# pku-lab-1806-llm/lab-1806-vec-db

Measured on AMD Instinct MI355X. Metric: queries/sec at recall@10, Gist1M d=960 (Flat brute force, L2Sqr, k=10), higher is better.
Workload: dtype f32 (int8 lower-bound filter pass); 1 GPU; flat_knn_gist1m; rows=1000000, dim=960, k=10, dist=L2Sqr, parallelism=single GPU, steps_in_flight=1, queries_per_corpus_pass=128

## Files before the change

lab_1806_vec_db_amd/csrc/api.hip:

```cpp
#include <algorithm>
#include <cmath>
#include <cstring>

#include "ctx.hpp"
#include "pq_hnsw.hpp"
#include "remove_plan.hpp"

using namespace vdb;

static thread_local std::string g_last_error;
void vdb::set_last_error(const std::string &m) { g_last_error = m; }
void vdb::require_gpu() {
    int cnt = 0;
    hipError_t e = hipGetDeviceCount(&cnt);
    if (e != hipSuccess || cnt <= 0)
        throw Error(VDB_ERR_NOGPU, std::string("no usable HIP device (libvdbhip has no CPU fallback): ") +
                                       hipGetErrorString(e));
}

static void require_merge_ids_fit(const Index &ix) {
    VDB_REQUIRE(ix.id_offset <= (1ull << 32) && ix.n <= (1ull << 32) - ix.id_offset, "shard merge: global row ids must fit 32 bits");
}

void vdb::merge_topk_dev(Index &ix, const void *d_dists, const void *d_ids, const void *d_counts, uint64_t stride_d,
// ... 616 lines not shown
        throw;
    }
    ix.prof_collect(*ws);
    VDB_API_END
}

int vdb_flat_knn_filtered_device(vdb_index *idx, const void *d_queries, uint64_t nq, uint64_t dim, uint64_t k, const vdb_mask *mask, void *d_out_idx,
                                 void *d_out_dist, void *d_out_count, void *stream) {
    VDB_API_BEGIN
    VDB_REQUIRE(idx, "null index");
    Index &ix = idx->ix;
    check_query_args(ix, d_queries, nq, dim, d_out_idx, d_out_dist);
    VDB_REQUIRE(nq == 0 || d_out_count, "null out_count");
    VDB_REQUIRE(nq <= 32768, "at most 32768 queries per device call");
    filtered_check(ix, mask);
    if (nq == 0) return VDB_OK;
    ix.use_device();
    WsLease ws(ix);
    VDB_SYNC(static_cast<hipStream_t>(stream));
    try {
        ix.flat_knn_masked_device(*ws, static_cast<const float *>(d_queries), nq, k, mask->m, static_cast<uint64_t *>(d_out_idx),
                                  static_cast<float *>(d_out_dist), static_cast<uint64_t *>(d_out_count));
    } catch (...) {
        (void)hipStreamSynchronize(ws->stream);
        ix.prof_collect(*ws);
        throw;
    }
    ix.prof_collect(*ws);
    VDB_API_END
}

static std::vector<const RowMask *> filtered_multi_check(const Index &ix, uint64_t nq, const vdb_mask *const *masks, uint64_t n_masks,
                                                         const uint32_t *mask_of) {
    VDB_REQUIRE(!ix.elem_u8, "filtered k-NN needs f32 rows: a VecSet<u8> index serves the filtered range search only");
    VDB_REQUIRE(n_masks == 0 || masks, "null masks");
    VDB_REQUIRE(nq == 0 || mask_of, "null mask_of");
    VDB_REQUIRE(n_masks < (1ull << 32), "too many masks");
    std::vector<const RowMask *> rm(n_masks);
    for (uint64_t g = 0; g < n_masks; g++) {
        VDB_REQUIRE(masks[g], "null mask");
        ix.check_mask(masks[g]->m);
        rm[g] = &masks[g]->m;
    }
    for (uint64_t q = 0; q < nq; q++)
        VDB_REQUIRE(mask_of[q] < n_masks, "mask_of[" + std::to_string(q) + "] = " + std::to_string(mask_of[q]) + ": the call has " +
                                              std::to_string(n_masks) + " masks");
    return rm;
}

int vdb_flat_knn_filtered_multi(vdb_index *idx, const float *queries, uint64_t nq, uint64_t dim, uint64_t k, const vdb_mask *const *masks,
                                uint64_t n_masks, const uint32_t *mask_of, uint64_t *out_idx, float *out_dist, uint64_t *out_count) {
    VDB_API_BEGIN
    VDB_REQUIRE(idx, "null index");
    Index &ix = idx->ix;
    check_query_args(ix, queries, nq, dim, out_idx, out_dist);
    const std::vector<const RowMask *> rm = filtered_multi_check(ix, nq, masks, n_masks, mask_of);
    ix.filtered_multi_calls++;
    if (nq == 0) return VDB_OK;
    ix.use_device();
    WsLease ws(ix);
    hipStream_t s = ws->stream;
    constexpr uint64_t CHUNK = 16384;
    const uint64_t kk = std::max<uint64_t>(k, 1), ch = std::min(nq, CHUNK);
    const size_t off_d = ch * kk * sizeof(uint64_t), off_c = (off_d + ch * kk * sizeof(float) + 7) & ~size_t(7);
    ws->q.reserve(ch * dim * sizeof(float));
    ws->out_idx.reserve(off_c + ch * sizeof(uint64_t));
    char *d_out = ws->out_idx.as<char>();
    try {
        for (uint64_t q0 = 0; q0 < nq; q0 += CHUNK) {
            const uint64_t nb = std::min<uint64_t>(CHUNK, nq - q0);
            VDB_HIP(hipMemcpyAsync(ws->q.p, queries + q0 * dim, nb * dim * sizeof(float), hipMemcpyHostToDevice, s));
            ix.flat_knn_masked_multi_device(*ws, ws->q.as<float>(), nb, k, rm.data(), n_masks, mask_of + q0, reinterpret_cast<uint64_t *>(d_out),
                                            reinterpret_cast<float *>(d_out + off_d), reinterpret_cast<uint64_t *>(d_out + off_c));
            if (k) {
                VDB_HIP(hipMemcpyAsync(out_idx + q0 * k, d_out, nb * k * sizeof(uint64_t), hipMemcpyDeviceToHost, s));
                VDB_HIP(hipMemcpyAsync(out_dist + q0 * k, d_out + off_d, nb * k * sizeof(float), hipMemcpyDeviceToHost, s));
            }
            if (out_count) VDB_HIP(hipMemcpyAsync(out_count + q0, d_out + off_c, nb * sizeof(uint64_t), hipMemcpyDeviceToHost, s));
            VDB_SYNC(s);
        }
    } catch (...) {
        (void)hipStreamSynchronize(s);
        ix.prof_collect(*ws);
        throw;
    }
    ix.prof_collect(*ws);
    VDB_API_END
}

int vdb_flat_knn_filtered_multi_device(vdb_index *idx, const void *d_queries, uint64_t nq, uint64_t dim, uint64_t k, const vdb_mask *const *masks,
                                       uint64_t n_masks, const uint32_t *mask_of, void *d_out_idx, void *d_out_dist, void *d_out_count, void *stream) {
    VDB_API_BEGIN
    VDB_REQUIRE(idx, "null index");
    Index &ix = idx->ix;
    check_query_args(ix, d_queries, nq, dim, d_out_idx, d_out_dist);
    VDB_REQUIRE(nq == 0 || d_out_count, "null out_count");
    VDB_REQUIRE(nq <= 32768, "at most 32768 queries per device call");
    const std::vector<const RowMask *> rm = filtered_multi_check(ix, nq, masks, n_masks, mask_of);
    ix.filtered_multi_calls++;
    if (nq == 0) return VDB_OK;
    ix.use_device();
    WsLease ws(ix);
    VDB_SYNC(static_cast<hipStream_t>(stream));
    try {
        ix.flat_knn_masked_multi_device(*ws, static_cast<const float *>(d_queries), nq, k, rm.data(), n_masks, mask_of, static_cast<uint64_t *>(d_out_idx),
                                        static_cast<float *>(d_out_dist), static_cast<uint64_t *>(d_out_count));
    } catch (...) {
        (void)hipStreamSynchronize(ws->stream);
        ix.prof_collect(*ws);
        throw;
    }
    ix.prof_collect(*ws);
    VDB_API_END
}

int vdb_flat_range_filtered(vdb_index *idx, const float *queries, uint64_t nq, uint64_t dim, const float *radius, uint64_t limit, const vdb_mask *mask,
                            vdb_range **out) {
    VDB_API_BEGIN
    VDB_REQUIRE(idx, "null index");
    Index &ix = idx->ix;
    range_check(ix, queries, nq, dim, radius, out);
    VDB_REQUIRE(mask, "null mask");
    ix.check_mask(mask->m);
    ix.use_device();
    std::unique_ptr<vdb_range> res(new vdb_range);
    WsLease ws(ix);
    const float *d_q = nullptr, *d_r = nullptr;
    if (nq) {
        const size_t qb = nq * dim * sizeof(float), qb_pad = (qb + 255) & ~size_t(255);
        ws->q.reserve(qb_pad + nq * sizeof(float));
        VDB_HIP(hipMemcpyAsync(ws->q.p, queries, qb, hipMemcpyHostToDevice, ws->stream));
        VDB_HIP(hipMemcpyAsync(ws->q.as<char>() + qb_pad, radius, nq * sizeof(float), hipMemcpyHostToDevice, ws->stream));
        d_q = ws->q.as<float>();
        d_r = reinterpret_cast<const float *>(ws->q.as<char>() + qb_pad);
    }
    try {
        ix.flat_range_device(*ws, d_q, nq, d_r, limit, res->r, &mask->m);
    } catch (...) {
        (void)hipStreamSynchronize(ws->stream);
        ix.prof_collect(*ws);
        throw;
    }
    ix.prof_collect(*ws);
    *out = res.release();
    VDB_API_END
}

int vdb_flat_shortlist_keys(vdb_index *idx, const float *queries, uint64_t nq, uint64_t dim, int tier, float *out_keys,
                            float *out_qsq, float *out_qerr, float *out_dx4) {
    VDB_API_BEGIN
    VDB_REQUIRE(idx && queries && out_keys, "null argument");
    Index &ix = idx->ix;
    VDB_REQUIRE(dim == ix.dim, "query dimension mismatch");
    VDB_REQUIRE(tier >= 0 && tier <= 2, "tier must be 0 (fp16 operands), 1 (split-bf16 operands) or 2 (8-bit operands, lower-bound keys)");
    ix.use_device();
    WsLease ws(ix);
    ws->q.reserve(nq * ix.dim * sizeof(float));
    VDB_HIP(hipMemcpyAsync(ws->q.p, queries, nq * ix.dim * sizeof(float), hipMemcpyHostToDevice, ws->stream));
    ix.flat_debug_keys(*ws, ws->q.as<float>(), nq, tier, out_keys, out_qsq, out_qerr, out_dx4);
    VDB_API_END
}

int vdb_flat_set_mode(vdb_index *idx, int mode) {
    VDB_API_BEGIN
    VDB_REQUIRE(idx, "null index");
    VDB_REQUIRE(mode >= 0 && mode <= 2, "mode must be 0, 1 or 2");
    idx->ix.flat_mode = mode;
    VDB_API_END
}
int vdb_set_param(vdb_index *idx, const char *name, int64_t value) {
    VDB_API_BEGIN
    VDB_REQUIRE(idx && name, "null argument");
    std::string n(name);
    if (n == "mfma_variant")
        mfma_set_variant((int)value);
    else if (n == "flat_share")
        mfma_set_share((int)value);
    else if (n == "flat_gemm")
        idx->ix.flat_gemm_mode = (int)value;
    else if (n == "hnsw_dma")
        hnsw_set_dma((int)value);
    else if (n == "hnsw_half")
        hnsw_set_half((int)value);
    else if (n == "ivf_half")
        ivf_set_half((int)value);
    else if (n == "ivf_q8")
        ivf_set_q8((int)value);
    else if (n == "hnsw_build_gpu")
        hnsw_set_build_gpu((int)value);
    else if (n == "hnsw_pool_cap")
        hnsw_set_pool_cap((int)value);
    else if (n == "pq_adc_fast")
        pq_set_adc_fast((int)value);
    else if (n == "pq_sample16")
        pq_set_adc16_sample((int)value);
    else if (n == "pq_adc16")
        pq_set_adc16((int)value);
    else if (n == "pq_adc8_sliced")
        pq_set_adc8_sliced((int)value);
    else if (n == "flat_sample_thin")
        mfma_set_sample_thin((int)value);
    else if (n == "flat_gemm_tw")
        gemm_set_tw((int)value);
    else if (n == "flat_gemm_nt")
        gemm_set_nt((int)value);
    else if (n == "flat_gemm_zigzag")
        gemm_set_zigzag((int)value);
    else if (n == "flat_gemm_block_rows") {
        VDB_REQUIRE(value >= 0, "flat_gemm_block_rows must be >= 0");
        gemm_set_block_rows((uint64_t)value);
    }
    else if (n == "flat_gemm_stagger")
        gemm_set_stagger((int)value);
    else if (n == "flat_gemm_debug")
        idx->ix.flat_gemm_debug = (int)value;
    else if (n == "flat_tail")
        idx->ix.flat_tail_mode = (int)value;
    else if (n == "flat_tail_lb_nw")
        flat_tail_lb_set_nw((int)value);
    else if (n == "flat_tail_lb_walk")
        flat_tail_lb_set_walk((int)value);
    else if (n == "flat_small")
        idx->ix.flat_small_mode = (int)value;
    else if (n == "flat_small_max_rows")
        idx->ix.flat_small_max_rows = (uint64_t)value;
    else if (n == "flat_half")
        idx->ix.flat_half_mode = (int)value;
    else if (n == "flat_i8")
        idx->ix.flat_i8_mode = (int)value;
    else if (n == "flat_i8_rows") {
        VDB_REQUIRE(value >= 64 && value <= 8192 && value % 64 == 0, "flat_i8_rows must be a multiple of 64 in [64, 8192]");
        idx->ix.flat_i8_kprime = (uint32_t)value;
    }
    else if (n == "flat_range_max_results") {
        VDB_REQUIRE(value >= 0, "flat_range_max_results must be >= 0");
        idx->ix.range_max_results = (uint64_t)value;
    }
    else if (n == "flat_filtered_direct_max") {
        VDB_REQUIRE(value >= 0, "flat_filtered_direct_max must be >= 0");
        idx->ix.flat_filtered_direct_max = (uint64_t)value;
    }
    else if (n == "debug_alloc_fail_over")
        devbuf_fail_over() = (size_t)value;
    else if (n == "flat_i8_unit_min")
        idx->ix.flat_i8_unit_min = (int)value;
    else if (n == "flat_i8_full")
        idx->ix.flat_i8_full = (int)value;
    else if (n == "flat_i8_refine") {
        idx->ix.flat_i8_refine = (int)value;
        idx->ix.i8_refine_on = 0;
        idx->ix.i8_refine_calls = 0;
    }
    else if (n == "flat_i8_second")
        idx->ix.flat_i8_second = (int)value;
    else if (n == "flat_i8_stats") {
        idx->ix.flat_i8_stats = (int)value;
        for (auto &h : idx->ix.i8_rounds_hist) h = 0;
        idx->ix.i8_hits_sum = 0;
        idx->ix.i8_hits_max = 0;
        idx->ix.i8_stat_queries = 0;
    }
    else if (n == "flat_i8_hits") {
        VDB_REQUIRE(value >= 256 && value <= 4096, "flat_i8_hits must be in [256, 4096]");
        idx->ix.flat_i8_hits = (uint32_t)value;
    }
    else if (n == "flat_gemm8_sample_res")
        gemm8_set_sample_res((int)value);
    else if (n == "flat_gemm8_nt")
        gemm8_set_nt((int)value);
    else if (n == "flat_gemm8_kc")
        gemm8_set_kc((int)value);
    else if (n == "flat_gemm8_burst")
        gemm8_set_burst((int)value);
    else if (n == "flat_gemm8_res")
        gemm8_set_res((int)value);
    else if (n == "flat_gemm8_coop")
        gemm8_set_coop((int)value);
    else if (n == "flat_gemm8_grid")
        gemm8_set_grid((int)value);
    else if (n == "flat_gemm8_epi")
        gemm8_set_epi((int)value);
    else if (n == "flat_gemm_coop")
        gemm_set_coop((int)value);
    else if (n == "flat_half_kmul") {
        VDB_REQUIRE(value >= 1 && value <= 64, "flat_half_kmul must be in [1, 64]");
        idx->ix.flat_half_kmul = (uint32_t)value;
    }
    else
        throw Error(VDB_ERR_INVALID, "unknown parameter " + n);
    VDB_API_END
}
int vdb_index_prepare(vdb_index *idx, int all_tiers) {
    VDB_API_BEGIN
    VDB_REQUIRE(idx, "null index");
    require_gpu();
    idx->ix.prepare_flat(all_tiers != 0);
    VDB_API_END
}
int vdb_flat_fallback_count(const vdb_index *idx, uint64_t *out) {
    VDB_API_BEGIN
    VDB_REQUIRE(idx && out, "null argument");
    *out = idx->ix.fallback_count.load();
    VDB_API_END
}

int vdb_get_stat(const vdb_index *idx, const char *name, uint64_t *out) {
    VDB_API_BEGIN
    VDB_REQUIRE(idx && name && out, "null argument");
    std::string n(name);
    if (n == "flat_fallback")
        *out = idx->ix.fallback_count.load();
    else if (n == "flat_half_queries")
        *out = idx->ix.half_queries.load();
    else if (n == "flat_half_redo")
        *out = idx->ix.half_redo.load();
    else if (n == "flat_half_valid")
        *out = idx->ix.half_m.valid ? 1 : 0;
    else if (n == "flat_gemm_coop_sets")
        *out = gemm_last_coop();
    else if (n == "flat_gemm8_coop_sets")
        *out = gemm8_last_coop();
    else if (n == "flat_i8_queries")
        *out = idx->ix.i8_queries.load();
    else if (n == "flat_i8_redo")
        *out = idx->ix.i8_redo.load();
    else if (n == "flat_i8_valid")
        *out = idx->ix.i8_m.valid ? 1 : 0;
    else if (n == "flat_range_queries")
        *out = idx->ix.range_queries.load();
    else if (n == "flat_range_i8_queries")
        *out = idx->ix.range_i8_queries.load();
    else if (n == "flat_range_scan_queries")
        *out = idx->ix.range_scan_queries.load();
    else if (n == "flat_range_hits")
        *out = idx->ix.range_hits.load();
    else if (n == "flat_range_hits_max")
        *out = idx->ix.range_hits_max.load();
    else if (n == "flat_range_results")
        *out = idx->ix.range_results.load();
    else if (n == "flat_filtered_queries")
        *out = idx->ix.filtered_queries.load();
    else if (n == "flat_filtered_direct_queries")
        *out = idx->ix.filtered_direct_queries.load();
    else if (n == "flat_filtered_i8_queries")
        *out = idx->ix.filtered_i8_queries.load();
    else if (n == "flat_filtered_fallback_queries")
        *out = idx->ix.filtered_fallback_queries.load();
    else if (n == "flat_filtered_multi_calls")
        *out = idx->ix.filtered_multi_calls.load();
    else if (n == "flat_filtered_grouped_queries")
        *out = idx->ix.filtered_grouped_queries.load();
    else if (n.rfind("flat_i8_rounds_", 0) == 0 && n.size() == 16 && n[15] >= '0' && n[15] <= '8')
        *out = idx->ix.i8_rounds_hist[n[15] - '0'].load();
    else if (n == "mirror_alloc_failures")
        *out = idx->ix.mirror_alloc_failures.load();
    else if (n == "flat_i8_second_queries")
        *out = idx->ix.i8_second_queries.load();
    else if (n == "flat_i8_second_redo")
        *out = idx->ix.i8_second_redo.load();
    else if (n == "flat_i8_hits_sum")
        *out = idx->ix.i8_hits_sum.load();
    else if (n == "flat_i8_hits_max")
        *out = idx->ix.i8_hits_max.load();
    else if (n == "flat_i8_stat_queries")
        *out = idx->ix.i8_stat_queries.load();
    else if (n == "flat_i8_rows_walked")
        *out = idx->ix.i8_rows_walked.load();
    else if (n == "flat_bf16_mirror")
        *out = idx->ix.tiled_built ? 1 : 0;
    else if (n == "hnsw_heap_walk_queries")
        *out = idx->ix.hnsw.heap_walk_queries.load();
    else if (n == "hnsw_half_dropped")
        *out = idx->ix.hnsw.last_half_dropped.load();
    else if (n == "ivf_last_offers")
        *out = idx->ix.ivf.last_offers.load();
    else if (n == "ivf_last_rows_fetched_q8")
        *out = idx->ix.ivf.last_rows_fetched_q8.load();
    else if (n == "ivf_last_kept_q8")
        *out = idx->ix.ivf.last_kept_q8.load();
    else if (n == "ivf_last_kept")
        *out = idx->ix.ivf.last_kept.load();
    else if (n == "pq_adc16_queries")
        *out = idx->ix.pq.adc16_queries.load();
    else if (n == "pq_adc16_redo")
        *out = idx->ix.pq.adc16_redo.load();
    else if (n == "flat_i8_refine_queries")
        *out = idx->ix.i8_refine_queries.load();
    else if (n == "flat_i8_refine_on")
        *out = (uint64_t)idx->ix.i8_refine_on.load();
    else if (n == "pq_q8_overflow")
        *out = idx->ix.pq.q8_overflow.load();
    else if (n == "pq_q8_short")
        *out = idx->ix.pq.q8_short.load();
    else if (n == "pq_q8_hits_sum")
        *out = idx->ix.pq.q8_hits_sum.load();
    else if (n == "pq_q8_hits_max")
        *out = idx->ix.pq.q8_hits_max.load();
    else if (n == "hbm_bytes_per_row")
        *out = idx->ix.hbm_bytes_per_row();
    else
        throw Error(VDB_ERR_INVALID, "unknown statistic " + n);
    VDB_API_END
}

int vdb_pq_attach(vdb_index *idx, uint64_t n_bits, uint64_t m, const float *centroids, const uint8_t *codes) {
    VDB_API_BEGIN
    VDB_REQUIRE(idx && centroids, "null argument");
    pq_attach(idx->ix, n_bits, m, centroids, codes);
    VDB_API_END
}
int vdb_pq_build(vdb_index *idx, uint64_t n_bits, uint64_t m, uint64_t train_n, uint64_t max_iter, float tol,
                 uint64_t seed) {
    VDB_API_BEGIN
    VDB_REQUIRE(idx, "null index");
    pq_build(idx->ix, n_bits, m, train_n, max_iter, tol, seed);
    VDB_API_END
}
int vdb_pq_clear(vdb_index *idx) {
    VDB_API_BEGIN
    VDB_REQUIRE(idx, "null index");
    pq_clear(idx->ix);
    VDB_API_END
}
int vdb_pq_has(const vdb_index *idx, int *out) {
    VDB_API_BEGIN
    VDB_REQUIRE(idx && out, "null argument");
    *out = idx->ix.pq.present ? 1 : 0;
    VDB_API_END
}
int vdb_pq_info(const vdb_index *idx, uint64_t *n_bits, uint64_t *m, uint64_t *enc_dim) {
    VDB_API_BEGIN
    VDB_REQUIRE(idx, "null index");
    VDB_REQUIRE(idx->ix.pq.present, "no PQ table");
    if (n_bits) *n_bits = idx->ix.pq.n_bits;
    if (m) *m = idx->ix.pq.m;
    if (enc_dim) *enc_dim = idx->ix.pq.enc_dim;
    VDB_API_END
}
int vdb_pq_export(const vdb_index *idx, float *centroids, uint8_t *codes) {
    VDB_API_BEGIN
    VDB_REQUIRE(idx, "null index");
    const Index &ix = idx->ix;
    VDB_REQUIRE(ix.pq.present, "no PQ table");
    if (centroids) std::memcpy(centroids, ix.pq.h_centroids.data(), ix.pq.h_centroids.size() * sizeof(float));
    if (codes && ix.n) {
        ix.use_device();
        VDB_HIP(hipMemcpy(codes, ix.pq.d_codes.p, ix.n * ix.pq.enc_dim, hipMemcpyDeviceToHost));
    }
    VDB_API_END
}

static void flat_pq_dev(Index &ix, Workspace &ws, const float *d_q, uint64_t nq, uint64_t k, uint64_t ef,
                        uint64_t *d_idx, float *d_dist, uint64_t *d_cnt) {
    flat_knn_pq_device(ix, ws, d_q, nq, k, ef, d_idx, d_dist, d_cnt);
}
int vdb_flat_knn_pq(vdb_index *idx, const float *queries, uint64_t nq, uint64_t dim, uint64_t k, uint64_t ef,
                    uint64_t *out_idx, float *out_dist, uint64_t *out_count) {
    VDB_API_BEGIN
    VDB_REQUIRE(idx, "null index");
    check_query_args(idx->ix, queries, nq, dim, out_idx, out_dist);
    VDB_REQUIRE(idx->ix.pq.present, "knn_pq needs a PQ table (vdb_pq_build / vdb_pq_attach)");
    host_search(idx->ix, queries, nq, k, ef, out_idx, out_dist, out_count, flat_pq_dev);
    VDB_API_END
}

int vdb_flat_knn_pq_device(vdb_index *idx, const void *d_queries, uint64_t nq, uint64_t dim, uint64_t k, uint64_t ef,
                           void *d_out_idx, void *d_out_dist, void *d_out_count, void *stream) {
    VDB_API_BEGIN
    VDB_REQUIRE(idx, "null index");
    VDB_REQUIRE(idx->ix.pq.present, "knn_pq needs a PQ table (vdb_pq_build / vdb_pq_attach)");
    device_search(idx->ix, d_queries, nq, dim, k, ef, d_out_idx, d_out_dist, d_out_count, stream, flat_pq_dev);
    VDB_API_END
}

// ... 480 lines not shown
```

lab_1806_vec_db_amd/csrc/index.hip:

```cpp
#include "index.hpp"
#include "multi_plan.hpp"
#include "remove_plan.hpp"

#include <algorithm>
#include <cmath>
#include <cstring>

namespace vdb {

Index::Index(int dev, uint64_t d, int ds, bool u8) : device(dev), dim(d), dist(ds), elem_u8(u8) {
#ifndef VDB_HOST_SANITIZER_BUILD
    use_device();
    hipDeviceProp_t prop;
    VDB_HIP(hipGetDeviceProperties(&prop, dev));
    num_cu = prop.multiProcessorCount > 0 ? prop.multiProcessorCount : 256;
    std::string arch = prop.gcnArchName;
    if (arch.rfind("gfx950", 0) != 0)
        throw Error(4, "libvdbhip is built for gfx950 (MI355X) only; device reports " + arch);
#endif
}

std::unique_ptr<Workspace> Index::acquire_ws() {
    use_device();
    {
// ... 402 lines not shown
            auto &e = prof[p.name];
            e.ms += ms;
            e.launches += 1;
            e.bytes += p.bytes;
        }
    }
    ws.pending.clear();
    ws.ev_used = 0;
}

void Index::scan_rows(uint64_t nrows, uint32_t d, const float *Q, uint32_t nq, int metric, const float *xsq, const float *qsq,
                      float *out, uint64_t ld, bool use_lds, hipStream_t s) const {
    if (elem_u8)
        launch_scan_exact_u8(d_rows.as<uint8_t>(), nrows, d, Q, nq, metric, xsq, qsq, out, ld, s);
    else
        launch_scan_exact(d_rows.as<float>(), nrows, d, Q, nq, metric, xsq, qsq, out, ld, use_lds, s);
}
void Index::rerank_rows(uint32_t d, const float *Q, uint32_t nq, int metric, const float *xsq, const float *qsq, const uint64_t *cand,
                        uint64_t *out, uint32_t ncand, uint32_t ldc, hipStream_t s) const {
    if (elem_u8)
        launch_rerank_u8(d_rows.as<uint8_t>(), d, Q, nq, metric, xsq, qsq, cand, out, ncand, ldc, s);
    else
        launch_rerank(d_rows.as<float>(), d, Q, nq, metric, xsq, qsq, cand, out, ncand, ldc, s);
}

void Index::flat_exact_device(Workspace &ws, const float *d_q, const float *d_qsq, uint64_t nq, uint32_t ksel,
                              uint64_t k, uint64_t *d_idx, float *d_dist, uint64_t *d_cnt) {
    hipStream_t s = ws.stream;
    const int metric = dist == 0 ? MET_L2_DIRECT : MET_COSINE;
    const uint64_t ld = (n + 63) & ~63ull;
    const uint32_t nl = topk_num_lists(n);
    const uint32_t cap = topk_capacity(ksel);
    constexpr uint32_t BQ = 8;
    ws.dense.reserve(size_t(BQ) * ld * sizeof(float));
    ws.lists.reserve(size_t(BQ) * nl * cap * sizeof(uint64_t));
    ws.keys_c.reserve(size_t(BQ) * cap * sizeof(uint64_t));
    if (n <= 8192 && nq >= 32) {
        constexpr uint64_t QCH = 4096;
        const uint64_t qch = std::min<uint64_t>(nq, QCH);
        ws.keys_a.reserve(qch * ld * sizeof(uint64_t));
        ws.keys_b.reserve(qch * ld * sizeof(uint64_t));
        ws.keys_c.reserve(qch * cap * sizeof(uint64_t));
        for (uint64_t q0 = 0; q0 < nq; q0 += qch) {
            const uint32_t nb = (uint32_t)std::min<uint64_t>(qch, nq - q0);
            launch_iota_keys(ws.keys_a.as<uint64_t>(), nb, (uint32_t)n, (uint32_t)ld, s);
            prof_begin(ws, "flat_exact", double(n) * dim * sizeof(float));
            rerank_rows((uint32_t)dim, d_q + q0 * dim, nb, metric, d_sq.as<float>(),
                          d_qsq ? d_qsq + q0 : nullptr, ws.keys_a.as<uint64_t>(), ws.keys_b.as<uint64_t>(), (uint32_t)n,
                          (uint32_t)ld, s);
            prof_end(ws);
            launch_topk_merge(ws.keys_b.as<uint64_t>(), 1, (uint32_t)ld, nb, ksel, ws.keys_c.as<uint64_t>(), s);
            launch_finalize(ws.keys_c.as<uint64_t>(), cap, nb, ksel, (uint32_t)k, id_offset, d_idx + q0 * k, d_dist + q0 * k,
                            d_cnt + q0, s);
        }
        return;
    }
    const bool use_lds = n >= 4096;
    for (uint64_t q0 = 0; q0 < nq; q0 += BQ) {
        uint32_t nb = (uint32_t)std::min<uint64_t>(BQ, nq - q0);
        prof_begin(ws, "flat_exact", double(n) * dim * sizeof(float));
        scan_rows(n, (uint32_t)dim, d_q + q0 * dim, nb, metric, d_sq.as<float>(),
                          d_qsq ? d_qsq + q0 : nullptr, ws.dense.as<float>(), ld, use_lds, s);
        prof_end(ws);
        launch_topk_dense(ws.dense.as<float>(), ld, n, nb, ksel, ws.lists.as<uint64_t>(), s);
        launch_topk_merge(ws.lists.as<uint64_t>(), nl, cap, nb, ksel, ws.keys_c.as<uint64_t>(), s);
        launch_finalize(ws.keys_c.as<uint64_t>(), cap, nb, ksel, (uint32_t)k, id_offset, d_idx + q0 * k, d_dist + q0 * k,
                        d_cnt + q0, s);
    }
}

void Index::flat_sorted_device(Workspace &ws, const float *d_q, uint64_t nq, uint64_t ksel, uint64_t k, uint64_t *d_idx,
                               float *d_dist, uint64_t *d_cnt) {
    hipStream_t s = ws.stream;
    VDB_REQUIRE(k < (1ull << 31), "flat knn: k too large");
    const int metric = dist == 0 ? MET_L2_DIRECT : MET_COSINE;
    const uint64_t ld = (n + 63) & ~63ull;
    constexpr uint32_t BQ = 8;
    size_t tb = sort_pairs_temp_bytes(n);
    ws.qsq.reserve(nq * sizeof(float));
    launch_row_sqnorm(d_q, nq, (uint32_t)dim, ws.qsq.as<float>(), s);
    ws.dense.reserve(size_t(BQ) * ld * sizeof(float));
    ws.keys_a.reserve(n * sizeof(uint64_t));
    ws.keys_b.reserve(n * sizeof(uint64_t));
    ws.lists.reserve(tb + 256);
    if (k > ksel) {
        VDB_HIP(hipMemsetAsync(d_idx, 0, nq * k * sizeof(uint64_t), s));
        VDB_HIP(hipMemsetAsync(d_dist, 0, nq * k * sizeof(float), s));
    }
    for (uint64_t q0 = 0; q0 < nq; q0 += BQ) {
        uint32_t nb = (uint32_t)std::min<uint64_t>(BQ, nq - q0);
        scan_rows(n, (uint32_t)dim, d_q + q0 * dim, nb, metric, d_sq.as<float>(),
                          ws.qsq.as<float>() + q0, ws.dense.as<float>(), ld, n >= 4096, s);
        for (uint32_t b = 0; b < nb; b++) {
            launch_sort_pairs(ws.dense.as<float>() + b * ld, n, ws.keys_a.as<uint64_t>(), ws.keys_b.as<uint64_t>(),
                              ws.lists.p, tb, s);
            launch_finalize(ws.keys_b.as<uint64_t>(), (uint32_t)n, 1, (uint32_t)ksel, (uint32_t)k, id_offset,
                            d_idx + (q0 + b) * k, d_dist + (q0 + b) * k, d_cnt + q0 + b, s);
        }
    }
}

bool Index::flat_small_applies(uint64_t nq, uint64_t k) const {
    if (flat_small_mode == 1 || elem_u8 || n == 0 || !flat_small_supported(n, (uint32_t)dim, nq, k)) return false;
    if (flat_small_mode == 2) return true;
    if (flat_mode != 0) return false;
    if (n <= flat_small_max_rows) return nq < 32;
    return mfma_supported((uint32_t)dim) ? double(n) * (0.9 * double(nq) - 0.3) < 75000.0 : nq < 32 && n <= (1u << 17);
}
void Index::flat_small_device(Workspace &ws, const float *q, uint64_t nq, uint64_t k, uint64_t *o_idx, float *o_dist, uint64_t *o_cnt) {
    hipStream_t s = ws.stream;
    const uint32_t ksel = (uint32_t)std::min<uint64_t>(k, n);
    ws.small_part.reserve(flat_small_part_keys(n, nq, ksel, num_cu) * sizeof(uint64_t));
    if (ws.small_cnt.cap < 64 * sizeof(uint32_t)) {
        ws.small_cnt.reserve(64 * sizeof(uint32_t));
        VDB_HIP(hipMemsetAsync(ws.small_cnt.p, 0, 64 * sizeof(uint32_t), s));
    }
    FlatSmallArgs a{};
    a.X = d_rows.as<float>();
    a.n = n;
    a.dim = (uint32_t)dim;
    a.Q = q;
    a.metric = dist == 0 ? MET_L2_DIRECT : MET_COSINE;
    a.xsq = d_sq.as<float>();
    a.part = ws.small_part.as<uint64_t>();
    a.counter = ws.small_cnt.as<uint32_t>();
    a.ksel = ksel;
    a.kstride = (uint32_t)k;
    a.id_offset = id_offset;
    a.out_idx = o_idx;
    a.out_dist = o_dist;
    a.out_count = o_cnt;
    prof_begin(ws, "flat_small", double(nq) * double(n) * dim * sizeof(float));
    launch_flat_small(a, (uint32_t)nq, num_cu, s);
    prof_end(ws);
}

constexpr uint64_t QCH = 1024;

template <class F>
void Index::corpus_pass(Workspace &ws, const char *name, double bytes, F launch) {
    {
        std::lock_guard<std::mutex> g(pass_mu);
        if (pass_ev_valid) VDB_HIP(hipStreamWaitEvent(ws.stream, pass_ev, 0));
    }
    prof_begin(ws, name, bytes);
    launch();
    prof_end(ws);
    std::lock_guard<std::mutex> g(pass_mu);
    if (!pass_ev) VDB_HIP(hipEventCreateWithFlags(&pass_ev, hipEventDisableTiming));
    VDB_HIP(hipEventRecord(pass_ev, ws.stream));
    pass_ev_valid = true;
}

I8Queries Index::i8_query_prep(Workspace &ws, const float *Q, uint64_t nb) {
    I8Queries qp;
    const uint64_t gq = gemm_group();
    qp.ngroups = (nb + gq - 1) / gq;
    qp.nq_pad = qp.ngroups * gq;
    const size_t sync_words = std::max<size_t>(128, mfma_sync_words(uint32_t(qp.nq_pad / mfma_batch((uint32_t)dim)), num_cu));
    ws.qsq.reserve(qp.nq_pad * sizeof(float));
    ws.qfrag_g.reserve(qp.nq_pad * size_t(mfma_dim_pad((uint32_t)dim)) * sizeof(float));
    ws.qaux.reserve(3 * qp.nq_pad * sizeof(float));
    ws.misc.reserve(qp.nq_pad * (sizeof(float) + sizeof(uint32_t)) + sync_words * sizeof(uint32_t));
    qp.d_tau = ws.misc.as<float>();
    qp.d_hits = reinterpret_cast<uint32_t *>(qp.d_tau + qp.nq_pad);
    qp.d_qscale = ws.qaux.as<float>();
    qp.d_qoff = qp.d_qscale + qp.nq_pad;
    launch_query_prep_i8(Q, (uint32_t)nb, (uint32_t)qp.nq_pad, (uint32_t)dim, d_mu_i8.as<float>(), i8_l1, i8_l2, ws.qsq.as<float>(), qp.d_qscale,
                         qp.d_qoff, qp.d_hits, ws.qfrag_g.p, ws.stream, dist == 1 ? 1 : 0);
    return qp;
}

TauSample Index::i8_sample_plan() const {
    TauSample sp;
    sp.s_rank = 64;
    mfma_sample_plan(n, 64u, &sp.s_step, &sp.s_rank, flat_i8_hits);
    const uint64_t units = gemm8_sample_units(n, sp.s_step);
    sp.unit_min = flat_i8_unit_min != 1 && units >= (flat_i8_unit_min == 2 ? 2ull : 16ull) * sp.s_rank;
    sp.set_keys(sp.unit_min ? units : gemm8_sample_rows(n, sp.s_step));
    return sp;
}

void Index::i8_sample(Workspace &ws, const I8Queries &qp, const float *rowc, const TauSample &sp) {
    launch_flat_gemm8_sample(d_tiled_i8.p, n, (uint32_t)dim, ws.qfrag_g.p, qp.d_qscale, (uint32_t)qp.ngroups, rowc, sp.s_step, ws.dense.as<float>(),
                             sp.ld_s, num_cu, ws.stream, sp.unit_min ? 1 : 0);
}

void Index::select_tau(Workspace &ws, const TauSample &sp, uint64_t nq_pad, uint64_t nq, float *d_tau) {
    hipStream_t s = ws.stream;
    if (sp.n_s <= select_tau_max_n()) {
        launch_select_tau(ws.dense.as<float>(), sp.ld_s, (uint32_t)sp.n_s, (uint32_t)nq_pad, (uint32_t)nq, sp.s_rank, d_tau, s);
        return;
    }
    launch_topk_dense(ws.dense.as<float>(), sp.ld_s, sp.n_s, (uint32_t)nq_pad, sp.s_rank, ws.lists.as<uint64_t>(), s);
    launch_topk_merge(ws.lists.as<uint64_t>(), sp.nl_s, sp.cap_s, (uint32_t)nq_pad, sp.s_rank, ws.keys_a.as<uint64_t>(), s);
    launch_extract_tau(ws.keys_a.as<uint64_t>(), sp.cap_s, (uint32_t)nq_pad, sp.s_rank, d_tau, s);
    if (nq_pad > nq) VDB_HIP(hipMemsetD32Async(reinterpret_cast<hipDeviceptr_t>(d_tau + nq), (int)0xFF800000u, nq_pad - nq, s));
}

void Index::i8_filter(Workspace &ws, const I8Queries &qp, const float *rowc, const char *name, uint32_t hits_expected) {
    corpus_pass(ws, name, double(qp.ngroups) * double(n) * dim, [&] {
        launch_flat_gemm8_filter(d_tiled_i8.p, n, (uint32_t)dim, ws.qfrag_g.p, qp.d_qscale, (uint32_t)qp.ngroups, rowc, qp.d_tau, ws.lists.as<uint64_t>(),
                                 qp.d_hits, FLAT_CAND_CAP, flat_gemm_debug, num_cu, ws.stream, hits_expected);
    });
}

FlatTailArgs Index::flat_tail_args(const Workspace &ws, const uint32_t *d_hits, const float *d_tau, const SplitErr &se) const {
    FlatTailArgs t{};
    t.cand = ws.lists.as<uint64_t>();
    t.cap = FLAT_CAND_CAP;
    t.cnt = d_hits;
    t.X = d_rows.as<float>();
    t.dim = (uint32_t)dim;
    t.cosine = dist == 1 ? 1 : 0;
    t.metric = t.cosine ? MET_COSINE : MET_L2_DIRECT;
    t.xsq = d_sq.as<float>();
    t.qsq = ws.qsq.as<float>();
    t.n_rows = n;
    t.xsq_max = xsq_max;
    t.xsq_min_pos = xsq_min_pos;
    t.se = se;
    t.id_offset = id_offset;
    t.tau = d_tau;
    return t;
}

bool Index::i8_side_tier(Workspace &ws) {
    return flat_mode != 1 && (flat_mode == 2 || n >= 16384) && flat_gemm_mode != 1 && i8_mirror_applicable() && ensure_i8(ws);
}

struct RedoSet {
    const uint64_t nr, k;
    DevBuf rx, rq, ri, rd, rc;
    RedoSet(const std::vector<uint64_t> &rows, const float *d_q, uint64_t dim, uint64_t k_, hipStream_t s) : nr(rows.size()), k(k_) {
        rx.reserve(nr * sizeof(uint64_t));
        rq.reserve(nr * dim * sizeof(float));
        ri.reserve(nr * k * sizeof(uint64_t));
        rd.reserve(nr * k * sizeof(float));
        rc.reserve(nr * sizeof(uint64_t));
        VDB_HIP(hipMemcpyAsync(rx.p, rows.data(), nr * sizeof(uint64_t), hipMemcpyHostToDevice, s));
        launch_gather_rows_f32(d_q, rx.as<uint64_t>(), nr, (uint32_t)dim, rq.as<float>(), s);
        VDB_HIP(hipMemsetAsync(ri.p, 0, nr * k * sizeof(uint64_t), s));
        VDB_HIP(hipMemsetAsync(rd.p, 0, nr * k * sizeof(float), s));
    }
    void scatter(uint64_t *d_idx, float *d_dist, uint64_t *d_cnt, hipStream_t s) {
        launch_scatter_results(ri.as<uint64_t>(), rd.as<float>(), rc.as<uint64_t>(), rx.as<uint64_t>(), nr, (uint32_t)k, d_idx, d_dist, d_cnt, s);
        VDB_SYNC(s);
    }
};

uint64_t Index::flat_knn_device(Workspace &ws, const float *d_q, uint64_t nq, uint64_t k, uint64_t *d_idx,
                                float *d_dist, uint64_t *d_cnt, bool allow_half, uint32_t kprime_min, bool allow_i8, const float *d_dk_hint) {
    FlatPending p;
    flat_knn_enqueue(ws, d_q, nq, k, d_idx, d_dist, d_cnt, allow_half, kprime_min, p, allow_i8, d_dk_hint);
    return flat_knn_finish(ws, p);
}

void Index::flat_knn_enqueue(Workspace &ws, const float *d_q, uint64_t nq, uint64_t k, uint64_t *d_idx, float *d_dist,
                             uint64_t *d_cnt, bool allow_half, uint32_t kprime_min, FlatPending &p, bool allow_i8, const float *d_dk_hint) {
    hipStream_t s = ws.stream;
    p = FlatPending{};
    if (nq == 0) return;
    if (k == 0 || n == 0) {
        VDB_HIP(hipMemsetAsync(d_cnt, 0, nq * sizeof(uint64_t), s));
        return;
    }
    if (flat_small_applies(nq, k)) {
        flat_small_device(ws, d_q, nq, k, d_idx, d_dist, d_cnt);
        return;
    }
    const uint64_t ksel64 = std::min<uint64_t>(k, n);
    if (ksel64 > 1024) {
        flat_sorted_device(ws, d_q, nq, ksel64, k, d_idx, d_dist, d_cnt);
        return;
    }
    const uint32_t ksel = (uint32_t)ksel64;
    if (k > ksel) {
        VDB_HIP(hipMemsetAsync(d_idx, 0, nq * k * sizeof(uint64_t), s));
        VDB_HIP(hipMemsetAsync(d_dist, 0, nq * k * sizeof(float), s));
    }
    ws.qsq.reserve(nq * sizeof(float));

    uint32_t kprime = std::max<uint32_t>(32, 2 * ksel);
    if (kprime_min > kprime && kprime_min <= 1024 && n > kprime_min) kprime = kprime_min;
    const int cosine = dist == 1 ? 1 : 0;
    bool mfma = mfma_supported((uint32_t)dim) && kprime <= 1024 && n > kprime &&
                (flat_mode == 2 || (flat_mode == 0 && n >= 16384));
    if (flat_mode == 1) mfma = false;
    if (!mfma) {
        launch_row_sqnorm(d_q, nq, (uint32_t)dim, ws.qsq.as<float>(), s);
        flat_exact_device(ws, d_q, ws.qsq.as<float>(), nq, ksel, k, d_idx, d_dist, d_cnt);
        return;
    }

    const uint64_t bq = mfma_batch((uint32_t)dim);
    const uint32_t kprime_h = std::max<uint32_t>(64, flat_half_kmul * ksel);
    const uint64_t hq = half_queries.load(), hr = half_redo.load();
    const bool i8_first = allow_i8 && allow_half && kprime_min == 0 && flat_gemm_mode != 1 && (d_dk_hint ? i8_m.valid.load() : i8_applicable(ksel));
    const bool i8 = i8_first && ensure_i8(ws);
    const bool half_wanted = !i8 && allow_half && flat_half_mode != 1 && kprime_h <= 1024 && n > kprime_h &&
                             (flat_half_mode == 2 || hq < 1024 || hr * 8 <= hq);
    const bool half_ok = half_wanted && ensure_half(ws);
    const bool gemm = i8 || flat_gemm_mode == 2 || (flat_gemm_mode == 0 && (nq > 64 || half_ok));
    const bool half = !i8 && half_ok && gemm;
    if (half) kprime = kprime_h;
    const bool i8_second = i8 && d_dk_hint != nullptr;
    if (i8) kprime = i8_second ? FLAT_CAND_CAP : flat_i8_kprime;
    if (!half && !i8) launch_row_sqnorm(d_q, nq, (uint32_t)dim, ws.qsq.as<float>(), s);
    if (!half && !i8 && !ensure_tiled(ws)) {
        flat_exact_device(ws, d_q, ws.qsq.as<float>(), nq, ksel, k, d_idx, d_dist, d_cnt);
        return;
    }
    const uint32_t capp = topk_capacity(i8 ? 64u : kprime);
    const uint32_t capk = topk_capacity(ksel);
    const uint64_t gq = gemm_group();
    const uint64_t ngroups = gemm ? (nq + gq - 1) / gq : 0;
    const uint64_t nq_pad = gemm ? ngroups * gq : (nq + bq - 1) / bq * bq;
    const uint64_t nbatch = nq_pad / bq;
    TauSample sp;
    if (i8) {
        sp = i8_sample_plan();
    } else {
        sp.s_rank = kprime;
        mfma_sample_plan(n, kprime, &sp.s_step, &sp.s_rank);
        sp.set_keys(gemm ? gemm_sample_rows(n, sp.s_step) : mfma_sample_rows(n, sp.s_step));
    }
    const size_t qf = mfma_qfrag_floats((uint32_t)dim);
    ws.qfrag.reserve(nbatch * qf * sizeof(float));
    ws.dense.reserve(nq_pad * sp.ld_s * sizeof(float));
    ws.lists.reserve(std::max<size_t>(nq_pad * sp.nl_s * capp, nq_pad * size_t(FLAT_CAND_CAP)) * sizeof(uint64_t));
    ws.keys_a.reserve(nq_pad * capp * sizeof(uint64_t));
    ws.keys_b.reserve(nq_pad * capp * sizeof(uint64_t));
    ws.keys_c.reserve(nq_pad * capk * sizeof(uint64_t));
    const size_t sync_words = mfma_sync_words((uint32_t)nbatch, num_cu);
    I8Queries qp;
    if (i8) {
        qp = i8_query_prep(ws, d_q, nq);
    } else {
        ws.misc.reserve(nq_pad * (sizeof(float) + sizeof(uint32_t)) + sync_words * sizeof(uint32_t));
        qp.d_tau = ws.misc.as<float>();
        qp.d_hits = reinterpret_cast<uint32_t *>(qp.d_tau + nq_pad);
    }
    float *const d_tau = qp.d_tau;
    uint32_t *const d_hits = qp.d_hits;
    if (!gemm) launch_mfma_pack_queries(d_q, (uint32_t)nq, (uint32_t)nq_pad, (uint32_t)dim, ws.qfrag.as<float>(), s);
    const float *xt = half ? d_tiled_h.as<float>() : d_tiled.as<float>();
    float *d_qmul = nullptr, *d_qerr = nullptr;
    if (gemm && !i8) {
        ws.qfrag_g.reserve(nq_pad * size_t(mfma_dim_pad((uint32_t)dim)) * sizeof(float));
        if (half) {
            ws.qaux.reserve(3 * nq_pad * sizeof(float));
            float *d_qscale = ws.qaux.as<float>();
            d_qmul = d_qscale + nq_pad;
            d_qerr = d_qmul + nq_pad;
            launch_query_prep_h(d_q, (uint32_t)nq, (uint32_t)nq_pad, (uint32_t)dim, half_sx(), ws.qsq.as<float>(), d_qscale, d_qmul,
                                d_qerr, d_hits, ws.qfrag_g.p, s);
        } else {
            launch_mfma_pack_queries_nh(d_q, (uint32_t)nq, (uint32_t)nq_pad, (uint32_t)dim, 8, ws.qfrag_g.as<float>(), s);
        }
    }
    if (i8_second) {
        launch_i8_tau_from_dk(d_dk_hint, (uint32_t)nq, (uint32_t)nq_pad, qp.d_qoff, ws.qsq.as<float>(), xsq_max, i8_mu_norm, (uint32_t)dim, cosine,
                              d_tau, s);
    } else {
        if (i8)
            i8_sample(ws, qp, d_rowc_i8.as<float>(), sp);
        else if (gemm)
            launch_flat_gemm_sample(xt, n, (uint32_t)dim, ws.qfrag_g.as<float>(), d_qmul, (uint32_t)ngroups,
                                    d_sq.as<float>(), cosine, sp.s_step, ws.dense.as<float>(), sp.ld_s, num_cu, s);
        else
            launch_flat_mfma_sample(d_tiled.as<float>(), n, (uint32_t)dim, ws.qfrag.as<float>(), (uint32_t)nbatch,
                                    d_sq.as<float>(), cosine, sp.s_step, ws.dense.as<float>(), sp.ld_s, num_cu, s);
        select_tau(ws, sp, nq_pad, nq, d_tau);
    }
    uint64_t *d_cand = ws.lists.as<uint64_t>();
    if (i8) {
        i8_filter(ws, qp, d_rowc_i8.as<float>(), "flat_i8", i8_second ? FLAT_CAND_CAP : std::max<uint32_t>(64u, sp.s_step * sp.s_rank));
    } else {
        if (!half) VDB_HIP(hipMemsetAsync(d_hits, 0, (nq_pad + sync_words) * sizeof(uint32_t), s));
        const uint64_t hbm_passes = gemm ? ngroups : (nbatch + mfma_share() - 1) / mfma_share();
        corpus_pass(ws, half ? "flat_half" : "flat_mfma", double(hbm_passes) * double(n) * dim * (half ? sizeof(uint16_t) : sizeof(float)), [&] {
            if (gemm)
                launch_flat_gemm_filter(xt, n, (uint32_t)dim, ws.qfrag_g.as<float>(), d_qmul, (uint32_t)ngroups,
                                        d_sq.as<float>(), cosine, d_tau, d_cand, d_hits, FLAT_CAND_CAP, flat_gemm_debug, num_cu, s);
            else
                launch_flat_mfma_filter(d_tiled.as<float>(), n, (uint32_t)dim, ws.qfrag.as<float>(), (uint32_t)nbatch,
                                        d_sq.as<float>(), cosine, d_tau, d_cand, d_hits, FLAT_CAND_CAP, d_hits + nq_pad, num_cu, s);
        });
    }
    SplitErr se;
    if (half) {
        se.qerr = d_qerr;
        se.dx_abs = half_dx_abs;
        se.dx_rel = half_dx_rel;
    }
    if (i8) {
        se.qoff = qp.d_qoff;
        se.mu_norm = i8_mu_norm;
    }
    if (i8 || (flat_tail_mode != 1 && !elem_u8 && flat_tail64_supported((uint32_t)dim, kprime, ksel))) {
        FlatTailArgs t = flat_tail_args(ws, d_hits, d_tau, se);
        t.kprime = kprime;
        t.ksel = ksel;
        t.kstride = (uint32_t)k;
        t.Q = d_q;
        bool refine = false;
        if (i8 && !i8_second && nq >= 64 && flat_i8_refine != 1) {
            bool on = flat_i8_refine == 2;
            if (flat_i8_refine == 0 && i8_refine_on.load() != 0) on = (i8_refine_calls.fetch_add(1) % 32u) != 31u;
            refine = on && ensure_rows_h(ws);
        }
        const size_t st_off = (nq + 15) & ~size_t(15);
        const bool want_stats = i8 && flat_i8_stats;
        t.flags = static_cast<uint8_t *>(ws.pinned(want_stats ? st_off + nq * sizeof(uint32_t) : nq));
        if (want_stats) t.qstat = reinterpret_cast<uint32_t *>(t.flags + st_off);
        p.stats = want_stats;
        p.refined = refine;
        if (refine) {
            launch_flat_refine_half(d_rows_h.as<uint16_t>(), (uint32_t)dim, half_sx(), half_dx_abs, half_dx_rel, cosine, d_q, d_sq.as<float>(),
                                    ws.qsq.as<float>(), qp.d_qoff, d_cand, FLAT_CAND_CAP, d_hits, (uint32_t)nq, FLAT_CAND_CAP, s);
            i8_refine_queries += nq;
        }
        t.out_idx = d_idx;
        t.out_dist = d_dist;
        t.out_count = d_cnt;
        if (i8 && i8_second && nq <= 96 && flat_i8_full != 1) {
            ws.keys_b.reserve(nq * size_t(FLAT_CAND_CAP) * sizeof(uint64_t));
            launch_flat_full_lb(t, (uint32_t)nq, ws.keys_b.as<uint64_t>(), ws.keys_c.as<uint64_t>(), s);
        } else if (i8)
            launch_flat_tail_lb(t, (uint32_t)nq, s);
        else
            launch_flat_tail64(t, (uint32_t)nq, s);
    } else {
        launch_topk_merge_counted(d_cand, FLAT_CAND_CAP, d_hits, (uint32_t)nq, kprime, ws.keys_a.as<uint64_t>(), s);
        rerank_rows((uint32_t)dim, d_q, (uint32_t)nq, cosine ? MET_COSINE : MET_L2_DIRECT, d_sq.as<float>(),
                      ws.qsq.as<float>(), ws.keys_a.as<uint64_t>(), ws.keys_b.as<uint64_t>(), kprime, capp, s);
        launch_topk_merge(ws.keys_b.as<uint64_t>(), 1, capp, (uint32_t)nq, ksel, ws.keys_c.as<uint64_t>(), s);
        launch_flat_finish(ws.keys_c.as<uint64_t>(), capk, ws.keys_a.as<uint64_t>(), capp, (uint32_t)nq, ksel, (uint32_t)k, kprime,
                           n, ws.qsq.as<float>(), xsq_max, xsq_min_pos, cosine, (uint32_t)dim, se, d_hits, FLAT_CAND_CAP, id_offset,
                           static_cast<uint8_t *>(ws.pinned(nq)), d_idx, d_dist, d_cnt, s);
    }
    p.active = true;
    p.half = half;
    p.i8 = i8;
    p.i8_second = i8_second;
    p.kprime = kprime;
    p.ksel = ksel;
    p.nq = nq;
    p.k = k;
    p.d_q = d_q;
    p.d_idx = d_idx;
    p.d_dist = d_dist;
    p.d_cnt = d_cnt;
}

uint64_t Index::flat_knn_finish(Workspace &ws, FlatPending &p) {
    hipStream_t s = ws.stream;
    if (!p.active) return 0;
    p.active = false;
    const uint64_t nq = p.nq, k = p.k;
    const uint8_t *flags = static_cast<const uint8_t *>(ws.pinned(nq));
    VDB_SYNC(s);
    std::vector<uint64_t> redo;
    for (uint64_t q = 0; q < nq; q++)
        if (flags[q] & 1u) redo.push_back(q);
    if (p.half) {
        half_queries += nq;
        half_redo += redo.size();
    }
    if (p.i8 && p.i8_second) {
        i8_second_queries += nq;
        i8_second_redo += redo.size();
    }
    const bool try_second = p.i8 && !p.i8_second && flat_i8_second != 1 && !redo.empty();
    if (p.i8 && !p.i8_second) {
        i8_queries += nq;
        if (!try_second) i8_redo += redo.size();
        if (flat_i8_refine == 0 && nq >= 64) {
            uint64_t rs = 0;
            for (uint64_t q = 0; q < nq; q++) rs += std::min<uint32_t>(flags[q] >> 1, 32u);
            const double mean_rounds = double(rs) / double(nq);
            if (!p.refined) {
                const int was = i8_refine_on.load();
                const int now = was ? (mean_rounds >= 4.0 ? 1 : 0) : (mean_rounds >= 6.0 ? 1 : 0);
                if (now != was) {
                    i8_refine_on = now;
                    i8_refine_calls = 0;
                }
            }
        }
        if (p.stats) {
            const uint32_t *qs = reinterpret_cast<const uint32_t *>(flags + ((nq + 15) & ~size_t(15)));
            uint64_t hs = 0, hm = 0;
            for (uint64_t q = 0; q < nq; q++) {
                const uint32_t r = qs[q] & 0xFFu, h = qs[q] >> 8;
                i8_rounds_hist[r < 8 ? r : 8] += 1;
                hs += h;
                hm = std::max<uint64_t>(hm, h);
            }
            i8_hits_sum += hs;
            i8_stat_queries += nq;
            uint64_t cur = i8_hits_max.load();
            while (hm > cur && !i8_hits_max.compare_exchange_weak(cur, hm)) {
            }
        }
    }
    if (redo.empty()) return 0;
    if (!p.half && !p.i8) fallback_count += redo.size();
    const uint64_t nr = redo.size();
    RedoSet r(redo, p.d_q, dim, k, s);
    DevBuf rqs, rdk;
    rqs.reserve(nr * sizeof(float));
    launch_gather_rows_f32(ws.qsq.as<float>(), r.rx.as<uint64_t>(), nr, 1, rqs.as<float>(), s);
    if (try_second) {
        rdk.reserve(nr * sizeof(float));
        launch_gather_dk(p.d_dist, p.d_cnt, r.rx.as<uint64_t>(), nr, (uint32_t)k, p.ksel, rdk.as<float>(), s);
    }
    VDB_SYNC(s);
    uint64_t *ri = r.ri.as<uint64_t>(), *rc = r.rc.as<uint64_t>();
// ... 125 lines not shown
            launch_range_scan_select(ws.dense.as<float>(), ld, n, R, nb, blk.as<uint32_t>(), p_cnt, s);
            VDB_SYNC(s);
            uint64_t add = 0, max_tot = 0, max_take = 0;
            for (uint32_t j = 0; j < nb; j++) {
                const uint64_t q = scan[g0 + j], t = limit ? std::min<uint64_t>(p_cnt[j], limit) : p_cnt[j];
                h_cnt[q] = t;
                h_off[q] = pool_used + add;
                p_off[j] = pool_used + add;
                p_take[j] = (uint32_t)t;
                add += t;
                max_tot = std::max<uint64_t>(max_tot, p_cnt[j]);
                max_take = std::max(max_take, t);
            }
            if (add == 0) continue;
            pool_room(add);
            const uint64_t ldo = (max_tot + 63) & ~63ull;
            const size_t tb = sort_rows_temp_bytes(nb, ldo);
            ws.keys_a.reserve(size_t(nb) * ldo * sizeof(uint64_t));
            ws.keys_b.reserve(size_t(nb) * ldo * sizeof(uint64_t));
            ws.lists.reserve(tb);
            VDB_HIP(hipMemsetAsync(ws.keys_a.p, 0xFF, size_t(nb) * ldo * sizeof(uint64_t), s));
            launch_range_compact(ws.dense.as<float>(), ld, n, R, nb, blk.as<uint32_t>(), ws.keys_a.as<uint64_t>(), ldo, s);
            launch_sort_rows(ws.keys_a.as<uint64_t>(), ws.keys_b.as<uint64_t>(), nb, ldo, ws.lists.p, tb, s);
            launch_range_append(ws.keys_b.as<uint64_t>(), ldo, p_off, p_take, nb, max_take, pool.as<uint64_t>(), s);
            pool_used += add;
            VDB_SYNC(s);
        }
        VDB_SYNC(s);
    }
    uint64_t total = 0, max_take = 0;
    for (uint64_t q = 0; q < nq; q++) {
        out.lims[q] = total;
        total += h_cnt[q];
        max_take = std::max(max_take, h_cnt[q]);
    }
    out.lims[nq] = total;
    range_results += total;
    if (total == 0) return;
    out.idx.reserve(total * sizeof(uint64_t));
    out.dist.reserve(total * sizeof(float));
    DevBuf meta;
    meta.reserve((2 * nq + 1) * sizeof(uint64_t));
    VDB_HIP(hipMemcpyAsync(meta.p, h_off.data(), nq * sizeof(uint64_t), hipMemcpyHostToDevice, s));
    VDB_HIP(hipMemcpyAsync(meta.as<uint64_t>() + nq, out.lims.data(), (nq + 1) * sizeof(uint64_t), hipMemcpyHostToDevice, s));
    launch_range_gather(pool.as<uint64_t>(), meta.as<uint64_t>(), meta.as<uint64_t>() + nq, nq, max_take, id_offset, out.idx.as<uint64_t>(),
                        out.dist.as<float>(), s);
    VDB_SYNC(s);
}

void Index::check_mask(const RowMask &mask) const {
    if (mask.owner != this) throw Error(1, "mask: made for another index");
    if (mask.gen != write_gen.load() || mask.n_rows != n)
        throw Error(3, "mask: stale -- rows were added to or removed from the index after the mask was made; make a new one");
}

const float *Index::masked_rowc(Workspace &ws, const RowMask &mask) {
    std::lock_guard<std::mutex> g(mask.mu);
    if (mask.rowc_of == d_rowc_i8.p && mask.d_rowc.p) return mask.d_rowc.as<float>();
    const uint64_t rows_pad = mirror_tiles(n) * 16;
    mask.d_rowc.reserve(rows_pad * 2 * sizeof(float));
    launch_mask_rowc(d_rowc_i8.as<float>(), mask.d_bits.as<uint64_t>(), n, rows_pad, mask.d_rowc.as<float>(), ws.stream);
    VDB_SYNC(ws.stream);
    mask.rowc_of = d_rowc_i8.p;
    return mask.d_rowc.as<float>();
}

void Index::flat_masked_direct(Workspace &ws, const float *d_q, uint64_t nq, uint64_t k, const RowMask &mask, uint64_t *d_idx, float *d_dist,
                               uint64_t *d_cnt) {
    hipStream_t s = ws.stream;
    const uint64_t m = mask.m;
    if (nq == 0 || k == 0 || m == 0) return;
    VDB_REQUIRE(k < (1ull << 31), "flat knn: k too large");
    const int metric = dist == 0 ? MET_L2_DIRECT : MET_COSINE;
    const uint64_t ksel = std::min<uint64_t>(k, m), ld = (m + 63) & ~63ull;
    const uint32_t *ids = mask.d_ids.as<uint32_t>();
    const bool use_lds = m >= 4096;
    constexpr uint64_t BUDGET = 256ull << 20;
    auto chunk_of = [&](uint64_t row_bytes) { return std::max<uint64_t>(8, std::min<uint64_t>(BUDGET / row_bytes, 32768) & ~7ull); };
    ws.qsq.reserve(nq * sizeof(float));
    launch_row_sqnorm(d_q, nq, (uint32_t)dim, ws.qsq.as<float>(), s);
    if (ksel <= 1024) {
        const uint32_t nl = topk_num_lists(m), cap = topk_capacity((uint32_t)ksel);
        const uint64_t qch = std::min(nq, std::min(chunk_of(ld * sizeof(float)), chunk_of(uint64_t(nl) * cap * sizeof(uint64_t))));
        ws.dense.reserve(qch * ld * sizeof(float));
        ws.lists.reserve(qch * nl * cap * sizeof(uint64_t));
        ws.keys_c.reserve(qch * cap * sizeof(uint64_t));
        for (uint64_t q0 = 0; q0 < nq; q0 += qch) {
            const uint32_t nb = (uint32_t)std::min<uint64_t>(qch, nq - q0);
            prof_begin(ws, "flat_filtered_scan", double((nb + 7) / 8) * double(m) * dim * sizeof(float));
            launch_scan_gather(d_rows.as<float>(), ids, m, (uint32_t)dim, d_q + q0 * dim, nb, metric, d_sq.as<float>(), ws.qsq.as<float>() + q0,
                               ws.dense.as<float>(), ld, use_lds, s);
            prof_end(ws);
            launch_topk_dense(ws.dense.as<float>(), ld, m, nb, (uint32_t)ksel, ws.lists.as<uint64_t>(), s);
            launch_topk_merge(ws.lists.as<uint64_t>(), nl, cap, nb, (uint32_t)ksel, ws.keys_c.as<uint64_t>(), s);
            launch_filter_finalize(ws.keys_c.as<uint64_t>(), cap, nb, (uint32_t)ksel, (uint32_t)k, ids, m, id_offset, d_idx + q0 * k, d_dist + q0 * k,
                                   d_cnt + q0, s);
        }
        return;
    }
    const uint64_t qch = std::min(nq, chunk_of(ld * sizeof(uint64_t)));
    const size_t tb = sort_rows_temp_bytes(qch, ld);
    ws.dense.reserve(qch * ld * sizeof(float));
    ws.keys_a.reserve(qch * ld * sizeof(uint64_t));
    ws.keys_b.reserve(qch * ld * sizeof(uint64_t));
    ws.keys_c.reserve(qch * ksel * sizeof(uint64_t));
    ws.lists.reserve(tb);
    for (uint64_t q0 = 0; q0 < nq; q0 += qch) {
        const uint32_t nb = (uint32_t)std::min<uint64_t>(qch, nq - q0);
        prof_begin(ws, "flat_filtered_scan", double((nb + 7) / 8) * double(m) * dim * sizeof(float));
        launch_scan_gather(d_rows.as<float>(), ids, m, (uint32_t)dim, d_q + q0 * dim, nb, metric, d_sq.as<float>(), ws.qsq.as<float>() + q0,
                           ws.dense.as<float>(), ld, use_lds, s);
        prof_end(ws);
        launch_pair_keys_rows(ws.dense.as<float>(), ld, m, nb, ws.keys_a.as<uint64_t>(), ld, s);
        launch_sort_rows(ws.keys_a.as<uint64_t>(), ws.keys_b.as<uint64_t>(), nb, ld, ws.lists.p, tb, s);
        launch_copy_prefix(ws.keys_b.as<uint64_t>(), ld, ws.keys_c.as<uint64_t>(), ksel, ksel, nb, s);
        launch_filter_finalize(ws.keys_c.as<uint64_t>(), ksel, nb, (uint32_t)ksel, (uint32_t)k, ids, m, id_offset, d_idx + q0 * k, d_dist + q0 * k,
                               d_cnt + q0, s);
    }
}

void Index::flat_knn_masked_device(Workspace &ws, const float *d_q, uint64_t nq, uint64_t k, const RowMask &mask, uint64_t *d_idx, float *d_dist,
                                   uint64_t *d_cnt) {
    hipStream_t s = ws.stream;
    check_mask(mask);
    VDB_REQUIRE(!elem_u8, "filtered k-NN needs f32 rows: a VecSet<u8> index serves the filtered range search only");
    filtered_queries += nq;
    if (nq == 0) return;
    const uint64_t m = mask.m;
    const uint64_t ksel64 = std::min<uint64_t>(k, m);
    VDB_HIP(hipMemsetAsync(d_cnt, 0, nq * sizeof(uint64_t), s));
    if (k > ksel64) {
        VDB_HIP(hipMemsetAsync(d_idx, 0, nq * k * sizeof(uint64_t), s));
        VDB_HIP(hipMemsetAsync(d_dist, 0, nq * k * sizeof(float), s));
    }
    if (ksel64 == 0) {
        filtered_direct_queries += nq;
        VDB_SYNC(s);
        return;
    }
    const bool tier = m > flat_filtered_direct_max && ksel64 <= 64 && flat_tail_lb_supported((uint32_t)dim, flat_i8_kprime, (uint32_t)ksel64) &&
                      i8_side_tier(ws);
    if (!tier) {
        filtered_direct_queries += nq;
        flat_masked_direct(ws, d_q, nq, k, mask, d_idx, d_dist, d_cnt);
        VDB_SYNC(s);
        return;
    }
    const float *rowc = masked_rowc(ws, mask);
    const TauSample sp = i8_sample_plan();
    std::vector<uint64_t> redo;
    for (uint64_t q0 = 0; q0 < nq; q0 += QCH) {
        const uint64_t nb = std::min<uint64_t>(QCH, nq - q0);
        const float *Q = d_q + q0 * dim;
        const I8Queries qp = i8_query_prep(ws, Q, nb);
        ws.dense.reserve(qp.nq_pad * sp.ld_s * sizeof(float));
        ws.lists.reserve(std::max<size_t>(qp.nq_pad * size_t(sp.nl_s) * sp.cap_s, qp.nq_pad * size_t(FLAT_CAND_CAP)) * sizeof(uint64_t));
        ws.keys_a.reserve(qp.nq_pad * size_t(sp.cap_s) * sizeof(uint64_t));
        i8_sample(ws, qp, rowc, sp);
        select_tau(ws, sp, qp.nq_pad, nb, qp.d_tau);
        launch_tau_clamp(qp.d_tau, (uint32_t)qp.nq_pad, s);
        i8_filter(ws, qp, rowc, "flat_filtered_i8", std::max<uint32_t>(64u, sp.s_step * sp.s_rank));
        SplitErr se;
        se.qoff = qp.d_qoff;
        se.mu_norm = i8_mu_norm;
        FlatTailArgs t = flat_tail_args(ws, qp.d_hits, qp.d_tau, se);
        t.kprime = flat_i8_kprime;
        t.ksel = (uint32_t)ksel64;
        t.kstride = (uint32_t)k;
        t.Q = Q;
        t.flags = static_cast<uint8_t *>(ws.pinned(nb));
        t.out_idx = d_idx + q0 * k;
        t.out_dist = d_dist + q0 * k;
        t.out_count = d_cnt + q0;
        launch_flat_tail_lb(t, (uint32_t)nb, s);
        VDB_SYNC(s);
        for (uint64_t q = 0; q < nb; q++)
            if (t.flags[q] & 1u) redo.push_back(q0 + q);
    }
    filtered_i8_queries += nq;
    filtered_fallback_queries += redo.size();
    if (redo.empty()) return;
    RedoSet r(redo, d_q, dim, k, s);
    VDB_HIP(hipMemsetAsync(r.rc.p, 0, r.nr * sizeof(uint64_t), s));
    flat_masked_direct(ws, r.rq.as<float>(), r.nr, k, mask, r.ri.as<uint64_t>(), r.rd.as<float>(), r.rc.as<uint64_t>());
    r.scatter(d_idx, d_dist, d_cnt, s);
}

void Index::flat_knn_masked_multi_device(Workspace &ws, const float *d_q, uint64_t nq, uint64_t k, const RowMask *const *masks, uint64_t n_masks,
                                         const uint32_t *mask_of, uint64_t *d_idx, float *d_dist, uint64_t *d_cnt) {
    hipStream_t s = ws.stream;
    VDB_REQUIRE(!elem_u8, "filtered k-NN needs f32 rows: a VecSet<u8> index serves the filtered range search only");
    if (nq == 0) return;
    VDB_REQUIRE(nq < (1ull << 32) && k < (1ull << 31), "flat knn: too many queries or k too large");
    if (k == 0) {
        filtered_queries += nq;
        filtered_direct_queries += nq;
        VDB_HIP(hipMemsetAsync(d_cnt, 0, nq * sizeof(uint64_t), s));
        VDB_SYNC(s);
        return;
    }
    std::vector<uint64_t> m_of(n_masks);
    std::vector<uint8_t> grouped(n_masks);
    for (uint64_t g = 0; g < n_masks; g++) {
        m_of[g] = masks[g]->m;
        grouped[g] = k <= 1024 && m_of[g] <= flat_filtered_direct_max;
    }
    {
        std::vector<std::vector<uint64_t>> bucket(n_masks);
        for (uint64_t q = 0; q < nq; q++)
            if (!grouped[mask_of[q]]) bucket[mask_of[q]].push_back(q);
        for (uint64_t g = 0; g < n_masks; g++) {
            if (bucket[g].empty()) continue;
            RedoSet r(bucket[g], d_q, dim, k, s);
            VDB_HIP(hipMemsetAsync(r.rc.p, 0, r.nr * sizeof(uint64_t), s));
            flat_knn_masked_device(ws, r.rq.as<float>(), r.nr, k, *masks[g], r.ri.as<uint64_t>(), r.rd.as<float>(), r.rc.as<uint64_t>());
            r.scatter(d_idx, d_dist, d_cnt, s);
        }
    }
    const uint64_t max_m = multi_plan_max_m(m_of.data(), grouped.data(), n_masks, mask_of, nq);
    const uint64_t ksel_all = std::min<uint64_t>(k, max_m);
    const uint64_t list_bytes = ksel_all ? uint64_t(topk_num_lists(max_m)) * topk_capacity((uint32_t)ksel_all) * sizeof(uint64_t) : 64;
    constexpr uint64_t BUDGET = 256ull << 20;
    MultiPlan plan;
    multi_plan(m_of.data(), grouped.data(), n_masks, mask_of, nq, BUDGET, list_bytes, plan);
    const uint64_t ns = plan.slot_query.size();
    if (ns == 0) return;
    filtered_queries += ns;
    filtered_direct_queries += ns;
    filtered_grouped_queries += ns;
    const int metric = dist == 0 ? MET_L2_DIRECT : MET_COSINE;
    std::vector<GroupedItem> h_items(plan.items.size());
    for (size_t i = 0; i < h_items.size(); i++) {
        const MultiItem &it = plan.items[i];
        h_items[i] = GroupedItem{masks[it.mask]->d_ids.as<uint32_t>(), (uint32_t)m_of[it.mask], it.tile, it.slot, it.nb};
    }
    std::vector<const uint32_t *> h_ids(ns);
    std::vector<uint32_t> h_m(ns);
    for (uint64_t i = 0; i < ns; i++) {
        h_ids[i] = masks[plan.slot_mask[i]]->d_ids.as<uint32_t>();
        h_m[i] = (uint32_t)m_of[plan.slot_mask[i]];
    }
    static_assert(sizeof(GroupedItem) % 8 == 0, "the items follow the pointer array");
    const size_t off_items = ns * sizeof(uint32_t *), off_q = off_items + h_items.size() * sizeof(GroupedItem), off_m = off_q + ns * sizeof(uint32_t);
    ws.misc.reserve(off_m + ns * sizeof(uint32_t));
    ws.qsq.reserve(nq * sizeof(float));
    const uint64_t ld_all = (max_m + 63) & ~63ull;
    const uint64_t qch = std::min(plan.qch, ns);
    if (ksel_all) {
        ws.dense.reserve(qch * ld_all * sizeof(float));
        ws.lists.reserve(qch * list_bytes);
        ws.keys_c.reserve(qch * topk_capacity((uint32_t)ksel_all) * sizeof(uint64_t));
    }
    char *d_plan = ws.misc.as<char>();
    VDB_HIP(hipMemcpyAsync(d_plan, h_ids.data(), ns * sizeof(uint32_t *), hipMemcpyHostToDevice, s));
    if (!h_items.empty()) VDB_HIP(hipMemcpyAsync(d_plan + off_items, h_items.data(), h_items.size() * sizeof(GroupedItem), hipMemcpyHostToDevice, s));
    VDB_HIP(hipMemcpyAsync(d_plan + off_q, plan.slot_query.data(), ns * sizeof(uint32_t), hipMemcpyHostToDevice, s));
    VDB_HIP(hipMemcpyAsync(d_plan + off_m, h_m.data(), ns * sizeof(uint32_t), hipMemcpyHostToDevice, s));
    const uint32_t *const *d_slot_ids = reinterpret_cast<const uint32_t *const *>(d_plan);
    const GroupedItem *d_items = reinterpret_cast<const GroupedItem *>(d_plan + off_items);
    const uint32_t *d_slot_q = reinterpret_cast<const uint32_t *>(d_plan + off_q), *d_slot_m = reinterpret_cast<const uint32_t *>(d_plan + off_m);
    launch_row_sqnorm(d_q, nq, (uint32_t)dim, ws.qsq.as<float>(), s);
    for (const MultiChunk &c : plan.chunks) {
        const uint32_t nb = (uint32_t)c.nslots;
        const uint64_t ksel = std::min<uint64_t>(k, c.max_m);
        uint32_t cap = 0;
        if (ksel) {
            const uint32_t nl = topk_num_lists(c.max_m);
            cap = topk_capacity((uint32_t)ksel);
            VDB_HIP(hipMemsetAsync(ws.dense.p, 0xFF, uint64_t(nb) * c.ld * sizeof(float), s));
            prof_begin(ws, "flat_filtered_scan_grouped", double(c.rows) * dim * sizeof(float));
            launch_scan_gather_grouped(d_rows.as<float>(), (uint32_t)dim, d_items + c.item0, c.nitems, d_slot_q + c.slot0, d_q, metric, d_sq.as<float>(),
                                       ws.qsq.as<float>(), ws.dense.as<float>(), c.ld, s);
            prof_end(ws);
            launch_topk_dense(ws.dense.as<float>(), c.ld, c.max_m, nb, (uint32_t)ksel, ws.lists.as<uint64_t>(), s);
            launch_topk_merge(ws.lists.as<uint64_t>(), nl, cap, nb, (uint32_t)ksel, ws.keys_c.as<uint64_t>(), s);
        }
        launch_filter_finalize_grouped(ws.keys_c.as<uint64_t>(), cap, nb, (uint32_t)ksel, (uint32_t)k, d_slot_ids + c.slot0, d_slot_m + c.slot0,
                                       d_slot_q + c.slot0, id_offset, d_idx, d_dist, d_cnt, s);
    }
    VDB_SYNC(s);
}

void Index::flat_debug_keys(Workspace &ws, const float *d_q, uint64_t nq, int tier, float *h_keys, float *h_qsq, float *h_qerr,
                            float *h_dx) {
    hipStream_t s = ws.stream;
    VDB_REQUIRE(nq >= 1 && nq <= 1024 && n >= 1, "debug keys: 1..1024 queries on a non-empty index");
    VDB_REQUIRE(mfma_supported((uint32_t)dim), "debug keys: the dimension has no MFMA shortlist path");
    const int cosine = dist == 1 ? 1 : 0;
    const uint64_t gq = gemm_group(), ngroups = (nq + gq - 1) / gq, nq_pad = ngroups * gq;
    if (tier == 2) {
        VDB_REQUIRE(!elem_u8 && (dim & 3) == 0 && gemm8_supported((uint32_t)dim), "debug keys: the index has no 8-bit pass");
        VDB_REQUIRE(ensure_i8(ws), "debug keys: the 8-bit mirror could not be allocated");
        TauSample sp;
        sp.set_keys(gemm8_sample_rows(n, 1));
        const I8Queries qp = i8_query_prep(ws, d_q, nq);
        ws.dense.reserve(qp.nq_pad * sp.ld_s * sizeof(float));
        i8_sample(ws, qp, d_rowc_i8.as<float>(), sp);
        VDB_HIP(hipMemcpy2DAsync(h_keys, n * sizeof(float), ws.dense.p, sp.ld_s * sizeof(float), n * sizeof(float), nq, hipMemcpyDeviceToHost, s));
        if (h_qsq) VDB_HIP(hipMemcpyAsync(h_qsq, ws.qsq.p, nq * sizeof(float), hipMemcpyDeviceToHost, s));
        if (h_qerr) VDB_HIP(hipMemcpyAsync(h_qerr, qp.d_qoff, nq * sizeof(float), hipMemcpyDeviceToHost, s));
        VDB_SYNC(s);
        if (h_dx) {
            h_dx[0] = i8_l1;
            h_dx[1] = i8_l2;
            h_dx[2] = i8_mu_norm;
            h_dx[3] = 0.0f;
        }
        return;
    }
    const bool half = tier == 0;
    VDB_REQUIRE(!half || ensure_half(ws), "debug keys: the index holds no fp16 mirror");
    if (!half) VDB_REQUIRE(ensure_tiled(ws), "debug keys: the split-bf16 mirror could not be allocated");
    const uint64_t n_s = gemm_sample_rows(n, 1), ld = (n_s + 63) & ~63ull;
    ws.qsq.reserve(nq_pad * sizeof(float));
    ws.qfrag_g.reserve(nq_pad * size_t(mfma_dim_pad((uint32_t)dim)) * sizeof(float));
    ws.dense.reserve(nq_pad * ld * sizeof(float));
    ws.qaux.reserve(3 * nq_pad * sizeof(float));
    ws.misc.reserve((nq_pad + 128) * sizeof(uint32_t));
    float *d_qscale = ws.qaux.as<float>(), *d_qmul = d_qscale + nq_pad, *d_qerr = d_qmul + nq_pad;
    if (half) {
        launch_query_prep_h(d_q, (uint32_t)nq, (uint32_t)nq_pad, (uint32_t)dim, half_sx(), ws.qsq.as<float>(), d_qscale, d_qmul, d_qerr,
                            ws.misc.as<uint32_t>(), nullptr, s);
        launch_pack_queries_h(d_q, (uint32_t)nq, (uint32_t)nq_pad, (uint32_t)dim, 8, d_qscale, ws.qfrag_g.p, s);
    } else {
        launch_row_sqnorm(d_q, nq, (uint32_t)dim, ws.qsq.as<float>(), s);
        launch_mfma_pack_queries_nh(d_q, (uint32_t)nq, (uint32_t)nq_pad, (uint32_t)dim, 8, ws.qfrag_g.as<float>(), s);
    }
    launch_flat_gemm_sample(half ? d_tiled_h.as<float>() : d_tiled.as<float>(), n, (uint32_t)dim, ws.qfrag_g.as<float>(),
                            half ? d_qmul : nullptr, (uint32_t)ngroups, d_sq.as<float>(), cosine, 1, ws.dense.as<float>(), ld, num_cu, s);
    VDB_HIP(hipMemcpy2DAsync(h_keys, n * sizeof(float), ws.dense.p, ld * sizeof(float), n * sizeof(float), nq, hipMemcpyDeviceToHost, s));
    if (h_qsq) VDB_HIP(hipMemcpyAsync(h_qsq, ws.qsq.p, nq * sizeof(float), hipMemcpyDeviceToHost, s));
    if (h_qerr) {
        if (half)
            VDB_HIP(hipMemcpyAsync(h_qerr, d_qerr, nq * sizeof(float), hipMemcpyDeviceToHost, s));
        else
            std::memset(h_qerr, 0, nq * sizeof(float));
    }
    VDB_SYNC(s);
    if (h_dx) {
        h_dx[0] = half ? half_dx_abs : 0.0f;
        h_dx[1] = half ? half_dx_rel : 0.0f;
        h_dx[2] = xsq_max;
        h_dx[3] = xsq_min_pos;
    }
}

}
```

lab_1806_vec_db_amd/csrc/index.hpp:

```cpp
#pragma once
#include <algorithm>
#include <atomic>
#include <cmath>
#include <cstdlib>
#include <functional>
#include <map>
#include <memory>
#include <mutex>
#include <string>
#include <vector>

#include "common.hpp"
#include "kernels.hpp"

namespace vdb {

inline bool devbuf_efence() {
    static const bool on = [] {
        const char *e = std::getenv("VDB_EFENCE");
        return e && e[0] == '1';
    }();
    return on;
}
inline std::atomic<size_t> &devbuf_fail_over() {
// ... 152 lines not shown
    std::atomic<uint64_t> heap_walk_queries{0};
};

struct FlatPending {
    bool active = false;
    bool half = false;
    bool i8 = false;
    bool i8_second = false;
    bool stats = false;
    bool refined = false;
    uint32_t kprime = 0, ksel = 0;
    uint64_t nq = 0, k = 0;
    const float *d_q = nullptr;
    uint64_t *d_idx = nullptr;
    float *d_dist = nullptr;
    uint64_t *d_cnt = nullptr;
};

struct I8Queries {
    uint64_t ngroups = 0, nq_pad = 0;
    float *d_tau = nullptr, *d_qscale = nullptr, *d_qoff = nullptr;
    uint32_t *d_hits = nullptr;
};

struct TauSample {
    uint32_t s_step = 1, s_rank = 0;
    bool unit_min = false;
    uint64_t n_s = 0, ld_s = 0;
    uint32_t nl_s = 0, cap_s = 0;
    void set_keys(uint64_t keys) {
        n_s = keys;
        ld_s = (keys + 63) & ~63ull;
        nl_s = topk_num_lists(keys);
        cap_s = topk_capacity(s_rank);
    }
};

struct RangeResult {
    int device = 0;
    uint64_t nq = 0;
    std::vector<uint64_t> lims;
    DevBuf idx, dist;
};

inline uint64_t mirror_tiles(uint64_t rows) { return ((rows + 15) / 16 + 11) / 12 * 12; }

struct RowMirror {
    std::mutex mu;
    std::atomic<bool> valid{false};
    std::atomic<uint64_t> rows{0};
    uint64_t failed_n = ~0ull;
    std::atomic<uint64_t> &failures;
    std::vector<DevBuf *> bufs;
    RowMirror(std::atomic<uint64_t> &f, std::initializer_list<DevBuf *> b) : failures(f), bufs(b) {}
    bool covers(uint64_t n) const { return valid && rows == n; }
    void set(uint64_t n) {
        rows = n;
        valid = true;
    }
    void invalidate() {
        valid = false;
        rows = 0;
    }
    bool attempt(const std::function<void()> &build);
    bool ensure(uint64_t n, const std::function<bool()> &current, const std::function<void()> &build);
};

struct Index;
struct RowMask {
    const Index *owner = nullptr;
    int device = 0;
    uint64_t gen = 0;
    uint64_t n_rows = 0;
    uint64_t m = 0;
    DevBuf d_bits;
    DevBuf d_ids;
    mutable std::mutex mu;
    mutable DevBuf d_rowc;
    mutable const void *rowc_of = nullptr;
};
struct IVFState {
    bool present = false;
    uint64_t k = 0, default_n_probes = 4;
    std::shared_ptr<Index> cent;
    std::vector<uint64_t> assign;
    std::vector<uint32_t> offsets;
    std::vector<uint32_t> sizes_desc;
    DevBuf d_offsets, d_members;
    std::atomic<uint64_t> last_rows_fetched_q8{0};
    std::atomic<uint64_t> last_kept_q8{0};
    std::atomic<uint32_t> q8_overflows{0};
    std::atomic<uint64_t> last_offers{0}, last_kept{0};
    std::atomic<uint32_t> half_overflows{0};
};

struct Index {
    int device = 0;
    int num_cu = 256;
    uint64_t dim = 0;
    int dist = 0;
    uint64_t n = 0;
    uint64_t id_offset = 0;
    bool elem_u8 = false;
    size_t elem_size() const { return elem_u8 ? 1 : sizeof(float); }
    const float *rows_f32_view(DevBuf &scratch, uint64_t r0, uint64_t r1, hipStream_t s) const;
    static constexpr uint64_t TILE_CHUNK = 12 * 64;
    size_t tile_chunk_bytes() const { return TILE_CHUNK * 16 * dim * sizeof(float); }
    template <class F>
    void for_tile_chunks(Workspace &ws, uint64_t t_begin, uint64_t t_end, uint64_t n_rows, F fn) const {
        if (!elem_u8) {
            fn(d_rows.as<float>(), t_begin, t_end, std::min(t_begin * 16, n_rows), n_rows);
            return;
        }
        constexpr uint64_t CH = TILE_CHUNK;
        ws.dense.reserve(tile_chunk_bytes());
        for (uint64_t t = t_begin; t < t_end; t += CH) {
            const uint64_t tb = std::min(t_end, t + CH), ra = std::min(t * 16, n_rows), rb = std::min(tb * 16, n_rows);
            fn(rows_f32_view(ws.dense, ra, rb, ws.stream), t, tb, ra, rb);
        }
    }
    DevBuf d_rows, d_sq;
    std::atomic<uint64_t> mirror_alloc_failures{0};
    DevBuf d_tiled;
    RowMirror tiled_m{mirror_alloc_failures, {&d_tiled}};
    const std::atomic<bool> &tiled_built = tiled_m.valid;
    bool ensure_tiled(Workspace &ws);
    void prepare_flat(bool all_tiers);
    uint64_t hbm_bytes_per_row() const;
    DevBuf d_tiled_h, d_half_err;
    int half_exp = 0;
    float half_dx_abs = 0.0f, half_dx_rel = 0.0f;
    int flat_half_mode = 0;
    uint32_t flat_half_kmul = 4;
    std::atomic<uint64_t> half_queries{0}, half_redo{0};
    void half_refresh(Workspace &ws, uint64_t n_old, uint64_t n_new);
    RowMirror half_m{mirror_alloc_failures, {&d_tiled_h}};
    bool i8_defers_half() const;
    bool ensure_half(Workspace &ws);
    float half_sx() const { return std::ldexp(1.0f, 13 - half_exp); }
    DevBuf d_tiled_i8, d_rowc_i8, d_mu_i8;
    RowMirror i8_m{mirror_alloc_failures, {&d_tiled_i8, &d_rowc_i8}};
    uint64_t i8_mu_rows = 0;
    float i8_l1 = 0.0f, i8_l2 = 0.0f, i8_mu_norm = 0.0f;
    int flat_i8_mode = 0;
    uint32_t flat_i8_kprime = 2048;
    int flat_i8_full = 0;
    int flat_i8_refine = 0;
    std::atomic<int> i8_refine_on{0};
    std::atomic<uint32_t> i8_refine_calls{0};
    std::atomic<uint64_t> i8_refine_queries{0};
    int flat_i8_unit_min = 0;
    int flat_i8_second = 0;
    std::atomic<uint64_t> i8_second_queries{0}, i8_second_redo{0};
    uint32_t flat_i8_hits = 1024;
    std::atomic<uint64_t> i8_queries{0}, i8_redo{0};
    int flat_i8_stats = 0;
    std::atomic<uint64_t> i8_rounds_hist[9] = {};
    std::atomic<uint64_t> i8_hits_sum{0}, i8_hits_max{0}, i8_stat_queries{0};
    std::atomic<uint64_t> i8_rows_walked{0};
    bool i8_applicable(uint32_t ksel) const;
    bool i8_mirror_applicable() const;
    bool ensure_i8(Workspace &ws);
    void build_i8(Workspace &ws);
    DevBuf d_rows_h;
    RowMirror rows_h_m{mirror_alloc_failures, {&d_rows_h}};
    int rows_h_exp = 0;
    bool ensure_rows_h(Workspace &ws);
    DevBuf d_rows_q8, d_q8_scale, d_q8_err;
    RowMirror rows_q8_m{mirror_alloc_failures, {&d_rows_q8, &d_q8_scale, &d_q8_err}};
    bool ensure_rows_q8(Workspace &ws);
    std::vector<float> h_sq;
    float xsq_max = 0.0f;
    float xsq_min_pos = 3.4e38f;
    mutable std::vector<float> h_rows;
    mutable bool host_valid = true;
    mutable std::mutex host_mu;
    int flat_mode = 0;
    int flat_gemm_mode = 0;
    int flat_gemm_debug = 0;
    int flat_tail_mode = 0;
    int flat_small_mode = 0;
    uint64_t flat_small_max_rows = 16384;
    bool flat_small_applies(uint64_t nq, uint64_t k) const;
    void flat_small_device(Workspace &ws, const float *q, uint64_t nq, uint64_t k, uint64_t *o_idx, float *o_dist, uint64_t *o_cnt);
    std::atomic<uint64_t> fallback_count{0};
    PQState pq;
    HNSWState hnsw;
    IVFState ivf;

    std::mutex ws_mu;
    std::vector<std::unique_ptr<Workspace>> ws_free;
    std::mutex pass_mu;
    hipEvent_t pass_ev = nullptr;
    bool pass_ev_valid = false;
    bool prof_on = false;
    std::mutex prof_mu;
    std::map<std::string, ProfEntry> prof;

    Index(int dev, uint64_t d, int ds, bool u8 = false);
    ~Index() {
        if (pass_ev) (void)hipEventDestroy(pass_ev);
    }
    void use_device() const {
#ifndef VDB_HOST_SANITIZER_BUILD
        VDB_HIP(hipSetDevice(device));
#endif
    }
    std::unique_ptr<Workspace> acquire_ws();
    void release_ws(std::unique_ptr<Workspace> ws);
    const float *host_rows() const;

    void add_rows(const void *rows, uint64_t count, bool on_device);
    void swap_remove(uint64_t i);
    void remove_rows(const uint64_t *rows, uint64_t m, std::vector<uint64_t> &dst, std::vector<uint64_t> &src);

    void prof_begin(Workspace &ws, const char *name, double bytes);
    void prof_end(Workspace &ws);
    void prof_collect(Workspace &ws);

    uint64_t flat_knn_device(Workspace &ws, const float *d_q, uint64_t nq, uint64_t k, uint64_t *d_idx, float *d_dist,
                         uint64_t *d_cnt, bool allow_half = true, uint32_t kprime_min = 0, bool allow_i8 = true,
                         const float *d_dk_hint = nullptr);
    void flat_knn_enqueue(Workspace &ws, const float *d_q, uint64_t nq, uint64_t k, uint64_t *d_idx, float *d_dist, uint64_t *d_cnt,
                          bool allow_half, uint32_t kprime_min, FlatPending &p, bool allow_i8 = true, const float *d_dk_hint = nullptr);
    uint64_t flat_knn_finish(Workspace &ws, FlatPending &p);
    template <class F>
    void corpus_pass(Workspace &ws, const char *name, double bytes, F launch);
    I8Queries i8_query_prep(Workspace &ws, const float *Q, uint64_t nb);
    TauSample i8_sample_plan() const;
    void i8_sample(Workspace &ws, const I8Queries &qp, const float *rowc, const TauSample &sp);
    void select_tau(Workspace &ws, const TauSample &sp, uint64_t nq_pad, uint64_t nq, float *d_tau);
    void i8_filter(Workspace &ws, const I8Queries &qp, const float *rowc, const char *name, uint32_t hits_expected);
    FlatTailArgs flat_tail_args(const Workspace &ws, const uint32_t *d_hits, const float *d_tau, const SplitErr &se) const;
    bool i8_side_tier(Workspace &ws);
    void flat_sorted_device(Workspace &ws, const float *d_q, uint64_t nq, uint64_t ksel, uint64_t k, uint64_t *d_idx,
                            float *d_dist, uint64_t *d_cnt);
    void scan_rows(uint64_t nrows, uint32_t d, const float *Q, uint32_t nq, int metric, const float *xsq, const float *qsq, float *out,
                   uint64_t ld, bool use_lds, hipStream_t s) const;
    void rerank_rows(uint32_t d, const float *Q, uint32_t nq, int metric, const float *xsq, const float *qsq, const uint64_t *cand,
                     uint64_t *out, uint32_t ncand, uint32_t ldc, hipStream_t s) const;
    void flat_debug_keys(Workspace &ws, const float *d_q, uint64_t nq, int tier, float *h_keys, float *h_qsq, float *h_qerr,
                         float *h_dx );
    void flat_exact_device(Workspace &ws, const float *d_q, const float *d_qsq, uint64_t nq, uint32_t ksel,
                           uint64_t k, uint64_t *d_idx, float *d_dist, uint64_t *d_cnt);
    void flat_range_device(Workspace &ws, const float *d_q, uint64_t nq, const float *d_radius, uint64_t limit, RangeResult &out,
                           const RowMask *mask = nullptr);
    void flat_knn_masked_device(Workspace &ws, const float *d_q, uint64_t nq, uint64_t k, const RowMask &mask, uint64_t *d_idx, float *d_dist,
                                uint64_t *d_cnt);
    void flat_masked_direct(Workspace &ws, const float *d_q, uint64_t nq, uint64_t k, const RowMask &mask, uint64_t *d_idx, float *d_dist,
                            uint64_t *d_cnt);
    void flat_knn_masked_multi_device(Workspace &ws, const float *d_q, uint64_t nq, uint64_t k, const RowMask *const *masks, uint64_t n_masks,
                                      const uint32_t *mask_of, uint64_t *d_idx, float *d_dist, uint64_t *d_cnt);
    void check_mask(const RowMask &mask) const;
    const float *masked_rowc(Workspace &ws, const RowMask &mask);
    std::atomic<uint64_t> write_gen{0};
    uint64_t flat_filtered_direct_max = 8192;
    std::atomic<uint64_t> filtered_queries{0}, filtered_direct_queries{0}, filtered_i8_queries{0}, filtered_fallback_queries{0};
    std::atomic<uint64_t> filtered_multi_calls{0}, filtered_grouped_queries{0};
    uint64_t range_max_results = 0;
    std::atomic<uint64_t> range_queries{0}, range_i8_queries{0}, range_scan_queries{0}, range_hits{0}, range_results{0};
    std::atomic<uint64_t> range_hits_max{0};
};

struct WsLease {
    Index &ix;
    std::unique_ptr<Workspace> ws;
    explicit WsLease(Index &i) : ix(i), ws(i.acquire_ws()) {}
    ~WsLease() { ix.release_ws(std::move(ws)); }
    Workspace &operator*() { return *ws; }
    Workspace *operator->() { return ws.get(); }
};

}
```

lab_1806_vec_db_amd/csrc/k_gemm8.hip:

```cpp
#include <atomic>
#include <type_traits>

#include "common.hpp"
#include "kernels.hpp"

namespace vdb {

typedef int i32x4 __attribute__((ext_vector_type(4)));
typedef float f32x2 __attribute__((ext_vector_type(2)));

constexpr uint32_t G8_NH = 8;
constexpr uint32_t G8_BQ = 16 * G8_NH;
constexpr uint32_t G8_WGBUF = 3072;
constexpr uint32_t G8_WGBUF_RES = 1536;
constexpr uint32_t G8_STAGE = 64;
constexpr uint32_t G8_TW = 3;

struct Gemm8Args {
    const uint4 *XT;
    const uint4 *qfrag;
    const float *qscale;
    const float2 *rowc;
    uint64_t n;
    uint32_t KB, n_units, ngroups;
    uint32_t unit_step;
    float *out;
    uint32_t unit_min;
    uint64_t ld;
    const float *tau;
    uint64_t *cand;
    uint32_t *cnt;
    uint32_t cap;
    uint32_t nt;
    uint32_t debug;
    uint32_t coop;
    uint32_t coop_block;
    uint32_t hits_expected;
    uint32_t *sync;
};

enum { G8_FILTER = 0, G8_SAMPLE = 1 };
#ifndef G8_ABLATE
#define G8_ABLATE 0
#endif

template <int KC, int MODE, bool XNT, bool BURST, bool RES, int EPI>
__global__ __launch_bounds__(512, 1) void k_flat_gemm8(Gemm8Args a) {
    constexpr int TW = G8_TW, NT = 512, NW = 8, NH = G8_NH, R = KC;
    constexpr uint32_t CHUNK = KC * NH * 64;
    constexpr int QST = CHUNK / NT;
    static_assert(CHUNK % NT == 0 && QST == KC, "one staged uint4 per thread and k-block");
    static_assert(!(RES && BURST), "the resident form stages nothing");
    constexpr uint32_t WGBUF = RES ? G8_WGBUF_RES : G8_WGBUF;
    extern __shared__ __attribute__((aligned(16))) uint4 smem8[];
    uint64_t *hit_key = reinterpret_cast<uint64_t *>(smem8 + (RES ? (a.KB / KC) * CHUNK : 2 * CHUNK));
    uint32_t *hit_q = reinterpret_cast<uint32_t *>(hit_key + WGBUF);
    uint32_t *hit_n = hit_q + WGBUF;
    float *tau_s = reinterpret_cast<float *>(hit_n + 4 + 2 * G8_BQ);
    float *qs_s = tau_s + G8_BQ;
    float *c_s = qs_s + G8_BQ;
    float *m_s = c_s + 8 * 64;
    float *stage_s = m_s + 8 * 64;

    const uint32_t lane = threadIdx.x & 63, wave = __builtin_amdgcn_readfirstlane(threadIdx.x >> 6);
    const uint32_t nwaves = gridDim.x * NW, gw = blockIdx.x * NW + wave;
    const uint32_t KB = a.KB, nchunk = KB / KC;
    const uint64_t n = a.n;

    const uint32_t S0 = a.n_units / nwaves, rem = a.n_units - S0 * nwaves;
    const uint32_t rem_wg = (rem + NW - 1) / NW;
    const uint32_t rw = S0 == 0 ? 0u : rem_wg;
    const uint32_t coopS = (RES && MODE == G8_FILTER) ? a.coop : 0u;
    const bool coop = coopS > 1;
    const uint32_t c_li = blockIdx.x >> 3, c_member = coop ? c_li % coopS : 0u, c_slices = coop ? (gridDim.x >> 3) / coopS : 1u;
    const uint32_t c_stride = c_slices * 64u, c_base0 = ((coop ? c_li / coopS : 0u) * 8u) * 8u + (blockIdx.x & 7u), c_base = c_base0 + wave * 8u;
    const uint32_t c_steps = c_base < a.n_units ? (a.n_units - c_base + c_stride - 1) / c_stride : 0u;
    const uint32_t c_steps_max = c_base0 < a.n_units ? (a.n_units - c_base0 + c_stride - 1) / c_stride : 0u;
    auto adv = [&](uint32_t slot) -> uint32_t {
        if (coop) return slot;
        return slot >= rw ? slot - rw : slot + gridDim.x - rw;
    };
    auto steps_of = [&](uint32_t slot) -> uint32_t {
        if (coop) return c_steps;
        if (rem == 0) return S0;
        if (S0 == 0) return 1;
        return S0 + (slot < rem_wg ? 1u : 0u);
    };
    auto unit_of = [&](uint32_t slot, uint32_t st) -> uint32_t {
        if (coop) return c_base + st * c_stride;
        return st < S0 ? st * nwaves + gw : S0 * nwaves + slot * NW + wave;
    };
    auto unit_ptr = [&](uint32_t u) -> const char * {
        if (u >= a.n_units) u = a.n_units - 1;
        return reinterpret_cast<const char *>(a.XT) + uint64_t(u) * a.unit_step * TW * KB * 1024;
    };
    if (coop && a.sync) {
        if (threadIdx.x == 0) {
            uint32_t *ctr = a.sync + (blockIdx.x & 7u) * 16u + c_li / coopS;
            __hip_atomic_fetch_add(ctr, 1u, __ATOMIC_RELAXED, __HIP_MEMORY_SCOPE_AGENT);
            const unsigned long long t0 = __builtin_readcyclecounter();
            while (__hip_atomic_load(ctr, __ATOMIC_RELAXED, __HIP_MEMORY_SCOPE_AGENT) < coopS && __builtin_readcyclecounter() - t0 < 250000ull)
                __builtin_amdgcn_s_sleep(16);
        }
        __syncthreads();
    }
    uint32_t slot_cur = blockIdx.x, slot_nxt = adv(slot_cur);
    const char *cp_cur = unit_ptr(unit_of(slot_cur, 0)),
               *cp_nxt = unit_ptr(1 < steps_of(slot_cur) ? unit_of(slot_cur, 1) : unit_of(slot_nxt, 0));
    uint32_t voff[TW];
#pragma unroll
    for (int t = 0; t < TW; t++) voff[t] = lane * 16 + t * KB * 1024;
    uint4 ring[R][TW];
    auto fetch_at = [&](uint4(&dst)[TW], const char *base, uint32_t kb) {
        const char *sb = base + kb * 1024;
#pragma unroll
        for (int t = 0; t < TW; t++) {
            if constexpr (XNT) {
                typedef uint32_t u32x4 __attribute__((ext_vector_type(4)));
                dst[t] = __builtin_bit_cast(uint4, __builtin_nontemporal_load(reinterpret_cast<const u32x4 *>(sb + voff[t])));
            } else {
                dst[t] = *reinterpret_cast<const uint4 *>(sb + voff[t]);
            }
        }
    };
#pragma unroll
    for (int p = 0; p < R; p++) {
        fetch_at(ring[p], cp_cur, p);
        __builtin_amdgcn_sched_barrier(0);
    }

    if constexpr (!RES) {
        const uint4 *src = a.qfrag + (MODE == G8_SAMPLE ? uint64_t(blockIdx.y) * nchunk * CHUNK : 0);
#pragma unroll
        for (int j = 0; j < QST; j++) smem8[j * NT + threadIdx.x] = src[j * NT + threadIdx.x];
    }
    uint32_t buf = 0;
    if constexpr (!RES) __syncthreads();

    const uint32_t g_begin = MODE == G8_SAMPLE ? blockIdx.y : 0, g_end = MODE == G8_SAMPLE ? blockIdx.y + 1 : a.ngroups;
    uint32_t stage_n = 0;
    for (uint32_t grp = g_begin + c_member; grp < g_end; grp += coop ? coopS : 1u) {
        const uint4 *qgrp = a.qfrag + uint64_t(grp) * nchunk * CHUNK;
        if constexpr (RES) {
            for (uint32_t c = 0; c < nchunk; c++) {
                uint4 t[QST];
#pragma unroll
                for (int j = 0; j < QST; j++) t[j] = qgrp[(c * QST + j) * NT + threadIdx.x];
#pragma unroll
                for (int j = 0; j < QST; j++) smem8[(c * QST + j) * NT + threadIdx.x] = t[j];
            }
        }
        if (MODE == G8_FILTER && threadIdx.x < 1 + 2 * G8_BQ) hit_n[threadIdx.x] = 0;
        if (MODE == G8_FILTER && threadIdx.x < G8_BQ) tau_s[threadIdx.x] = (a.debug & 1) ? -INFINITY : a.tau[grp * G8_BQ + threadIdx.x];
        if (threadIdx.x < G8_BQ) qs_s[threadIdx.x] = a.qscale[grp * G8_BQ + threadIdx.x];
        if constexpr (RES) __syncthreads();
        i32x4 qr0 = {0, 0, 0, 0}, qr1 = qr0, qr2 = qr0, qr3 = qr0;
        if constexpr (RES) {
            const uint4 *q0p = smem8 + lane;
            qr0 = __builtin_bit_cast(i32x4, q0p[0]);
            qr1 = __builtin_bit_cast(i32x4, q0p[64]);
            qr2 = __builtin_bit_cast(i32x4, q0p[128]);
        }
        auto drain = [&](const uint32_t lane) {
            float4 *stage_k = reinterpret_cast<float4 *>(stage_s) + wave * G8_STAGE;
            uint32_t *stage_r = reinterpret_cast<uint32_t *>(reinterpret_cast<float4 *>(stage_s) + 8 * G8_STAGE) + wave * G8_STAGE;
            uint32_t *stage_q = stage_r + 8 * G8_STAGE;
            const uint32_t cnt = stage_n < G8_STAGE ? stage_n : G8_STAGE;
            for (uint32_t i = lane; i < cnt; i += 64) {
                const float4 kv = stage_k[i];
                const uint2 mt = make_uint2(stage_r[i], stage_q[i]);
                const float tq = tau_s[mt.y];
                const bool p0 = kv.x <= tq && mt.x + 0 < n, p1 = kv.y <= tq && mt.x + 1 < n;
                const bool p2 = kv.z <= tq && mt.x + 2 < n, p3 = kv.w <= tq && mt.x + 3 < n;
                const uint32_t mine = uint32_t(p0) + uint32_t(p1) + uint32_t(p2) + uint32_t(p3);
                if (mine) {
                    uint32_t pos = atomicAdd(hit_n, mine);
#ifdef G8_NOSPILL
#define G8_SPILL(KEY, E) atomicAdd(&a.cnt[grp * G8_BQ + mt.y], a.cap + 1);
#else
#define G8_SPILL(KEY, E)                                                                  \
    const uint32_t gslot = atomicAdd(&a.cnt[grp * G8_BQ + mt.y], 1u);                     \
    if (gslot < a.cap) a.cand[(uint64_t(grp) * G8_BQ + mt.y) * a.cap + gslot] = pair_key(KEY, mt.x + E);
#endif
#define VDB_PARK8(P, KEY, E)                                                                          \
    if (P) {                                                                                          \
        if (pos < WGBUF) {                                                                            \
            hit_key[pos] = pair_key(KEY, mt.x + E);                                                   \
            hit_q[pos] = mt.y;                                                                        \
        } else {                                                                                      \
            G8_SPILL(KEY, E)                                                                          \
        }                                                                                             \
        pos++;                                                                                        \
    }
                    if constexpr (EPI == 0) {
#pragma clang loop unroll(disable)
                        for (uint32_t e = 0; e < 4; e++) {
                            const bool pe = e == 0 ? p0 : (e == 1 ? p1 : (e == 2 ? p2 : p3));
                            const float ke = e == 0 ? kv.x : (e == 1 ? kv.y : (e == 2 ? kv.z : kv.w));
                            VDB_PARK8(pe, ke, e)
                        }
                    } else {
                        VDB_PARK8(p0, kv.x, 0)
                        VDB_PARK8(p1, kv.y, 1)
                        VDB_PARK8(p2, kv.z, 2)
                        VDB_PARK8(p3, kv.w, 3)
                    }
#undef VDB_PARK8
#undef G8_SPILL
                }
            }
            stage_n = 0;
        };
        const uint32_t steps = steps_of(slot_cur);
        const uint32_t steps_all = coop ? c_steps_max : steps;
        const uint32_t blk = RES && a.coop_block ? a.coop_block : 0xFFFFFFFFu;
        for (uint32_t b0 = 0;;) {
        const uint32_t b1 = blk >= steps_all - b0 ? steps_all : b0 + blk;
        const uint32_t st_end = b1 < steps ? b1 : steps;
        for (uint32_t st = b0; st < st_end; st++) {
            const uint32_t u_raw = unit_of(slot_cur, st);
            const uint32_t u = u_raw < a.n_units ? u_raw : a.n_units - 1;
            i32x4 acc[TW][NH];
#pragma unroll
            for (int t = 0; t < TW; t++)
#pragma unroll
                for (int h = 0; h < NH; h++) acc[t][h] = (i32x4){0, 0, 0, 0};
            const char *rc_base = reinterpret_cast<const char *>(a.rowc + uint64_t(__builtin_amdgcn_readfirstlane(u)) * a.unit_step * (16 * TW));
            uint32_t rc_off = (lane < 16 * TW ? lane : 0) * 8;
            asm volatile("" : "+v"(rc_off));
            for (uint32_t c = 0; c < nchunk; c++) {
                const uint4 *nxt = (c + 1 < nchunk ? qgrp + uint64_t(c + 1) * CHUNK
                                    : (st + 1 < steps ? qgrp : (grp + 1 < a.ngroups ? qgrp + uint64_t(nchunk) * CHUNK : a.qfrag)));
                const uint32_t tid16 = threadIdx.x * 16;
                uint4 *qdst = smem8 + (buf ^ 1) * CHUNK + threadIdx.x;
                const uint4 *qcur = smem8 + (RES ? c : buf) * CHUNK + lane;
                const bool last_c = c + 1 == nchunk;
                i32x4 q_n = {0, 0, 0, 0};
                if constexpr (!RES) q_n = __builtin_bit_cast(i32x4, qcur[0]);
                const uint4 *qnx = smem8 + (last_c ? 0u : (c + 1) * CHUNK) + lane;
                float2 rc_stage = make_float2(0.0f, 0.0f);
                uint4 qs0, qs1, qs2, qs3, qs4;
                auto stage_ref = [&](auto P) -> uint4 & {
                    constexpr int p = decltype(P)::value;
                    if constexpr (p == 0) return qs0;
                    else if constexpr (p == 1) return qs1;
                    else if constexpr (p == 2) return qs2;
                    else if constexpr (p == 3) return qs3;
                    else return qs4;
                };
                auto stage_load = [&](auto P) {
                    constexpr int p = decltype(P)::value;
                    stage_ref(P) = *reinterpret_cast<const uint4 *>(reinterpret_cast<const char *>(nxt + p * NT) + tid16);
                };
                auto kblock = [&](auto P) {
                    constexpr int p = decltype(P)::value;
                    if constexpr (!BURST && !RES) {
                        stage_load(P);
                        if (p == 0) rc_stage = *reinterpret_cast<const float2 *>(rc_base + rc_off);
                    }
                    if constexpr (RES) {
                        if (p == 0) rc_stage = *reinterpret_cast<const float2 *>(rc_base + rc_off);
                    }
                    __builtin_amdgcn_sched_barrier(0);
                    i32x4 xv[TW];
#pragma unroll
                    for (int t = 0; t < TW; t++) xv[t] = __builtin_bit_cast(i32x4, ring[p][t]);
#pragma unroll
                    for (int h = 0; h < NH; h++) {
                        i32x4 qv;
                        if constexpr (RES) {
                            const int sidx = p * NH + h, f = sidx + 3;
                            qv = (sidx & 3) == 0 ? qr0 : ((sidx & 3) == 1 ? qr1 : ((sidx & 3) == 2 ? qr2 : qr3));
                            const i32x4 ld = __builtin_bit_cast(i32x4, f < KC * NH ? qcur[f * 64] : qnx[(f - KC * NH) * 64]);
                            if ((f & 3) == 0) qr0 = ld;
                            else if ((f & 3) == 1) qr1 = ld;
                            else if ((f & 3) == 2) qr2 = ld;
                            else qr3 = ld;
                        } else {
                            qv = q_n;
                            if (!(p == KC - 1 && h == NH - 1)) {
                                const int pn = h + 1 < NH ? p : p + 1, hn = h + 1 < NH ? h + 1 : 0;
                                q_n = __builtin_bit_cast(i32x4, qcur[(pn * NH + hn) * 64]);
                            }
                        }
                        __builtin_amdgcn_sched_barrier(0);
                        if ((G8_ABLATE & 2) && h > 0) {
                            acc[0][h][0] += qv[0];
                        } else {
#pragma unroll
                            for (int t = 0; t < TW; t++) acc[t][h] = __builtin_amdgcn_mfma_i32_16x16x64_i8(xv[t], qv, acc[t][h], 0, 0, 0);
                        }
                        __builtin_amdgcn_sched_barrier(0);
                    }
                    fetch_at(ring[p], last_c ? cp_nxt : cp_cur, last_c ? uint32_t(p) : (c + 1) * KC + p);
                    __builtin_amdgcn_sched_barrier(0);
                    if constexpr (!BURST && !RES) {
                        qdst[p * NT] = stage_ref(P);
                        if (p == 0) {
                            c_s[wave * 64 + lane] = rc_stage.x;
                            m_s[wave * 64 + lane] = rc_stage.y;
                        }
                        __builtin_amdgcn_sched_barrier(0);
                    }
                };
                using I0 = std::integral_constant<int, 0>;
                using I1 = std::integral_constant<int, 1>;
                using I2 = std::integral_constant<int, 2>;
// ... 39 lines not shown
                else
                    un = 1 < steps_of(slot_nxt) ? unit_of(slot_nxt, 1) : unit_of(adv(slot_nxt), 0);
                cp_nxt = unit_ptr(un);
            }
            const uint64_t row0 = uint64_t(u_raw) * a.unit_step * (16 * TW);
            if constexpr (EPI == 1) stage_n = 0;
            uint32_t lane_e = __builtin_amdgcn_mbcnt_hi(~0u, __builtin_amdgcn_mbcnt_lo(~0u, 0u));
            asm volatile("" : "+v"(lane_e));
            const uint32_t r = lane_e & 15, g4 = lane_e >> 4, lane = lane_e;
            float4 *stage_k = reinterpret_cast<float4 *>(stage_s) + wave * G8_STAGE;
            uint32_t *stage_r = reinterpret_cast<uint32_t *>(reinterpret_cast<float4 *>(stage_s) + 8 * G8_STAGE) + wave * G8_STAGE;
            uint32_t *stage_q = stage_r + 8 * G8_STAGE;
            float tauv[NH], qsv[NH];
#pragma unroll
            for (int h = 0; h < NH; h++) {
                tauv[h] = MODE == G8_FILTER ? tau_s[h * 16 + r] : 0.0f;
                qsv[h] = qs_s[h * 16 + r];
            }
            float umin[NH];
#pragma unroll
            for (int h = 0; h < NH; h++) umin[h] = INFINITY;
#pragma unroll
            for (int t = 0; t < TW; t++) {
                const float4 c4 = *reinterpret_cast<const float4 *>(&c_s[wave * 64 + t * 16 + 4 * g4]);
                const float4 m4 = *reinterpret_cast<const float4 *>(&m_s[wave * 64 + t * 16 + 4 * g4]);
                const uint32_t rb32 = uint32_t(row0) + t * 16 + 4 * g4;
#pragma unroll
                for (int h = 0; h < NH; h++) {
                    if ((G8_ABLATE & 1) && (t > 0 || h > 0)) {
                        if (acc[t][h][0] + acc[t][h][1] + acc[t][h][2] + acc[t][h][3] == 12345) atomicAdd(hit_n, 1u);
                        continue;
                    }
                    const float tau_h = tauv[h], sq = qsv[h];
                    float k0, k1, k2, k3;
                    if constexpr (EPI == 1) {
                        const f32x2 c01 = {c4.x, c4.y}, c23 = {c4.z, c4.w}, m01 = {m4.x, m4.y}, m23 = {m4.z, m4.w};
                        const f32x2 sq2 = {sq, sq};
                        f32x2 p01 = {float(acc[t][h][0]), float(acc[t][h][1])}, p23 = {float(acc[t][h][2]), float(acc[t][h][3])};
                        p01 *= sq2;
                        p23 *= sq2;
                        const f32x2 k01 = __builtin_elementwise_fma(p01, m01, c01), k23 = __builtin_elementwise_fma(p23, m23, c23);
                        k0 = k01.x, k1 = k01.y, k2 = k23.x, k3 = k23.y;
                    } else {
                        float p0 = float(acc[t][h][0]) * sq, p1 = float(acc[t][h][1]) * sq, p2 = float(acc[t][h][2]) * sq, p3 = float(acc[t][h][3]) * sq;
                        asm volatile("" : "+v"(p0), "+v"(p1), "+v"(p2), "+v"(p3));
                        k0 = __builtin_fmaf(p0, m4.x, c4.x), k1 = __builtin_fmaf(p1, m4.y, c4.y);
                        k2 = __builtin_fmaf(p2, m4.z, c4.z), k3 = __builtin_fmaf(p3, m4.w, c4.w);
                        asm volatile("" : "+v"(k0), "+v"(k1), "+v"(k2), "+v"(k3));
                    }
                    if (MODE == G8_SAMPLE && a.unit_min) {
                        float mn;
                        asm("v_min3_f32 %0, %1, %2, %3" : "=v"(mn) : "v"(rb32 + 0 < n ? k0 : INFINITY), "v"(rb32 + 1 < n ? k1 : INFINITY),
                            "v"(rb32 + 2 < n ? k2 : INFINITY));
                        asm("v_min3_f32 %0, %1, %2, %3" : "=v"(umin[h]) : "v"(mn), "v"(rb32 + 3 < n ? k3 : INFINITY), "v"(umin[h]));
                        continue;
                    }
                    if (MODE == G8_SAMPLE) {
                        if (u_raw < a.n_units) {
                            float4 kv;
                            kv.x = rb32 + 0 < n ? k0 : INFINITY;
                            kv.y = rb32 + 1 < n ? k1 : INFINITY;
                            kv.z = rb32 + 2 < n ? k2 : INFINITY;
                            kv.w = rb32 + 3 < n ? k3 : INFINITY;
                            const uint64_t col = uint64_t(u_raw) * (16 * TW) + t * 16 + 4 * g4;
                            *reinterpret_cast<float4 *>(a.out + (uint64_t(grp) * G8_BQ + h * 16 + r) * a.ld + col) = kv;
                        }
                        continue;
                    }
                    float kmin3, kmin;
                    asm("v_min3_f32 %0, %1, %2, %3" : "=v"(kmin3) : "v"(k0), "v"(k1), "v"(k2));
                    asm("v_min_f32 %0, %1, %2" : "=v"(kmin) : "v"(kmin3), "v"(k3));
                    const bool pass = kmin <= tau_h;
                    const uint64_t pm = __ballot(pass);
                    if (pm) {
                        const uint32_t np = __builtin_popcountll(pm);
                        if (stage_n + np > G8_STAGE) drain(lane);
                        if (pass) {
                            const uint32_t slot = stage_n + __builtin_amdgcn_mbcnt_hi(uint32_t(pm >> 32), __builtin_amdgcn_mbcnt_lo(uint32_t(pm), 0u));
                            stage_k[slot] = make_float4(k0, k1, k2, k3);
                            stage_r[slot] = rb32;
                            stage_q[slot] = h * 16 + r;
                        }
                        stage_n += np;
                    }
                }
            }
            if (MODE == G8_SAMPLE && a.unit_min && u_raw < a.n_units) {
#pragma unroll
                for (int h = 0; h < NH; h++) {
                    float m = umin[h];
                    m = fminf(m, __shfl_xor(m, 16));
                    m = fminf(m, __shfl_xor(m, 32));
                    if (g4 == 0) a.out[(uint64_t(grp) * G8_BQ + h * 16 + r) * a.ld + u_raw] = m;
                }
            }
            if (EPI == 1 && MODE == G8_FILTER && stage_n) drain(lane);
        }
        if (EPI == 0 && MODE == G8_FILTER && stage_n) drain(__builtin_amdgcn_mbcnt_hi(~0u, __builtin_amdgcn_mbcnt_lo(~0u, 0u)));
        __syncthreads();
        if (MODE == G8_FILTER) {
            uint32_t total = hit_n[0];
            if (total > WGBUF) total = WGBUF;
            constexpr uint32_t NJ = (WGBUF + NT - 1) / NT;
            uint32_t rank[NJ];
#pragma unroll
            for (uint32_t j = 0; j < NJ; j++) {
                uint32_t i = j * NT + threadIdx.x;
                rank[j] = i < total ? atomicAdd(&hit_n[1 + hit_q[i]], 1u) : 0u;
            }
            __syncthreads();
            if (threadIdx.x < G8_BQ && hit_n[1 + threadIdx.x] > 0)
                hit_n[1 + G8_BQ + threadIdx.x] = atomicAdd(&a.cnt[grp * G8_BQ + threadIdx.x], hit_n[1 + threadIdx.x]);
            __syncthreads();
#pragma unroll
            for (uint32_t j = 0; j < NJ; j++) {
                uint32_t i = j * NT + threadIdx.x;
                if (i < total) {
                    uint32_t q = hit_q[i];
                    uint32_t slot = hit_n[1 + G8_BQ + q] + rank[j];
                    if (slot < a.cap) a.cand[(uint64_t(grp) * G8_BQ + q) * a.cap + slot] = hit_key[i];
                }
            }
            __syncthreads();
            if (blk != 0xFFFFFFFFu) {
                if (threadIdx.x < 1 + 2 * G8_BQ) hit_n[threadIdx.x] = 0;
                __syncthreads();
            }
        }
        b0 = b1;
        if (b0 >= steps_all) break;
        }
        slot_cur = slot_nxt;
        slot_nxt = adv(slot_nxt);
    }
}

static std::atomic<int> g_gemm8_nt{0};
void gemm8_set_nt(int v) { g_gemm8_nt = v; }

bool gemm8_supported(uint32_t dim) {
    const uint32_t pad = mfma_dim_pad(dim);
    const uint32_t kb = pad / 64;
    return kb >= 2 && pad <= 2048 && (kb % 5 == 0 || kb % 3 == 0 || kb % 2 == 0);
}

static size_t gemm8_res_lds(uint32_t KB) {
    return size_t(KB) * G8_NH * 64 * sizeof(uint4) + size_t(G8_WGBUF_RES) * 12 + (4 + 4 * G8_BQ + 2 * 8 * 64) * 4 + size_t(8) * G8_STAGE * 24 + 16;
}
static std::atomic<int> g_gemm8_epi{0};
void gemm8_set_epi(int v) {
    VDB_REQUIRE(v == 0 || v == 1, "flat_gemm8_epi: 0 (scalar arithmetic, carried stage) or 1 (packed arithmetic, one drain per unit)");
    g_gemm8_epi = v;
}
template <int KC, int MODE, bool XNT, bool BURST, bool RES, int EPI>
static void flat_gemm8_launch2(const Gemm8Args &a0, int num_cu, hipStream_t s) {
    Gemm8Args a = a0;
    const uint64_t n_tiles = (a.n + 15) / 16;
    const uint32_t units_all = (uint32_t)((n_tiles + G8_TW - 1) / G8_TW);
    uint32_t grid;
    if (MODE == G8_SAMPLE) {
        a.n_units = (units_all + a.unit_step - 1) / a.unit_step;
        grid = (a.n_units + 7) / 8;
    } else {
        a.unit_step = 1;
        a.n_units = units_all;
        grid = (uint32_t)num_cu;
        const uint32_t need = (a.n_units + 7) / 8;
        if (need < grid) grid = need;
    }
    if (grid == 0 || a.ngroups == 0) return;
    const size_t lds = RES ? gemm8_res_lds(a.KB)
                           : size_t(2) * KC * G8_NH * 64 * sizeof(uint4) + size_t(G8_WGBUF) * 12 + (4 + 4 * G8_BQ + 2 * 8 * 64) * 4 +
                                 size_t(8) * G8_STAGE * 24 + 16;
    func_max_lds(reinterpret_cast<const void *>(&k_flat_gemm8<KC, MODE, XNT, BURST, RES, EPI>), int(160 * 1024));
    hipLaunchKernelGGL((k_flat_gemm8<KC, MODE, XNT, BURST, RES, EPI>), dim3(grid, MODE == G8_SAMPLE ? a.ngroups : 1), dim3(512), lds, s, a);
    VDB_HIP(hipGetLastError());
}
template <int KC, int MODE, bool XNT, bool BURST, bool RES>
static void flat_gemm8_launch1(const Gemm8Args &a, int num_cu, hipStream_t s) {
    if (g_gemm8_epi == 1)
        flat_gemm8_launch2<KC, MODE, XNT, BURST, RES, 1>(a, num_cu, s);
    else
        flat_gemm8_launch2<KC, MODE, XNT, BURST, RES, 0>(a, num_cu, s);
}
static std::atomic<int> g_gemm8_kc{0};
void gemm8_set_kc(int v) { g_gemm8_kc = v; }
static std::atomic<int> g_gemm8_burst{0};
void gemm8_set_burst(int v) { g_gemm8_burst = v; }
static std::atomic<int> g_gemm8_res{0};
void gemm8_set_res(int v) { g_gemm8_res = v; }

static std::atomic<int> g_gemm8_sample_res{0};
void gemm8_set_sample_res(int v) { g_gemm8_sample_res = v; }

static std::atomic<int> g_gemm8_coop{0};
void gemm8_set_coop(int v) { g_gemm8_coop = v; }
static std::atomic<int> g_gemm8_grid{0};
void gemm8_set_grid(int v) {
    VDB_REQUIRE(v == 0 || (v >= 32 && v <= 256 && v % 32 == 0), "flat_gemm8_grid: 0, or a multiple of 32 up to 256");
    g_gemm8_grid = v;
}
static std::atomic<uint32_t> g_gemm8_last_coop{0};
uint32_t gemm8_last_coop() { return g_gemm8_last_coop; }

template <int KC, int MODE>
static void flat_gemm8_launch(const Gemm8Args &a0, int num_cu, hipStream_t s) {
    Gemm8Args a = a0;
    const bool nt = MODE == G8_FILTER && a.nt;
    if (g_gemm8_res != 1 && !(MODE == G8_SAMPLE && g_gemm8_sample_res == 1) && gemm8_res_lds(a.KB) <= size_t(160) * 1024) {
        if (MODE == G8_FILTER && g_gemm8_coop != 1 && num_cu == 256) {
            const uint32_t S = a.ngroups % 8 == 0 ? 8u : (a.ngroups % 4 == 0 ? 4u : (a.ngroups % 2 == 0 ? 2u : 1u));
            const uint64_t units = ((a.n + 15) / 16 + G8_TW - 1) / G8_TW;
            if (S > 1 && units >= 2048) {
                a.coop = S;
                g_gemm8_last_coop = S;
                const double per_unit = 8.0 * 48.0 * 128.0 * double(a.hits_expected ? a.hits_expected : 1024u) / double(a.n);
                const double b = double(G8_WGBUF_RES) * 0.8 / per_unit;
                a.coop_block = b < 1.0 ? 1u : (b > 4096.0 ? 4096u : uint32_t(b));
                const int grid = g_gemm8_grid ? (int)g_gemm8_grid : num_cu;
                VDB_REQUIRE((grid / 8) % S == 0, "flat_gemm8_grid: the sets do not divide the workgroups of an XCD (sets of 8 need a multiple of 64)");
                flat_gemm8_launch1<KC, MODE, false, false, true>(a, grid, s);
                return;
            }
        }
        if (MODE == G8_FILTER) g_gemm8_last_coop = 0;
        if (MODE == G8_FILTER && a.hits_expected > 2048) {
            const double per_unit = 8.0 * 48.0 * 128.0 * double(a.hits_expected) / double(a.n);
            const double b = double(G8_WGBUF_RES) * 0.55 / per_unit;
            a.coop_block = b < 1.0 ? 1u : (b > 4096.0 ? 4096u : uint32_t(b));
        }
        if (nt)
            flat_gemm8_launch1<KC, MODE, true, false, true>(a, num_cu, s);
        else
            flat_gemm8_launch1<KC, MODE, false, false, true>(a, num_cu, s);
        return;
    }
    const int bm = g_gemm8_burst;
    const bool burst = KC <= 3 && bm != 1;
    if (nt) {
        if (burst) {
            if constexpr (KC <= 3) flat_gemm8_launch1<KC, MODE, true, true, false>(a, num_cu, s);
        } else {
            flat_gemm8_launch1<KC, MODE, true, false, false>(a, num_cu, s);
        }
    } else {
        if (burst) {
            if constexpr (KC <= 3) flat_gemm8_launch1<KC, MODE, false, true, false>(a, num_cu, s);
        } else {
            flat_gemm8_launch1<KC, MODE, false, false, false>(a, num_cu, s);
        }
    }
}
template <int MODE>
static void flat_gemm8_dispatch(const Gemm8Args &a, int num_cu, hipStream_t s) {
    const int want = g_gemm8_kc;
    int kc = 0;
    if (want == 5 || want == 3 || want == 2)
        if (a.KB % uint32_t(want) == 0) kc = want;
    const bool res = g_gemm8_res != 1 && !(MODE == G8_SAMPLE && g_gemm8_sample_res == 1) && gemm8_res_lds(a.KB) <= size_t(160) * 1024;
    if (kc == 0) kc = res ? (a.KB % 5 == 0 ? 5 : (a.KB % 3 == 0 ? 3 : 2)) : (a.KB % 3 == 0 ? 3 : (a.KB % 5 == 0 ? 5 : 2));
    VDB_REQUIRE(a.KB % uint32_t(kc) == 0, "flat_gemm8: k-block count must be divisible by 5, 3 or 2");
    if (kc == 5)
        flat_gemm8_launch<5, MODE>(a, num_cu, s);
    else if (kc == 3)
        flat_gemm8_launch<3, MODE>(a, num_cu, s);
    else
        flat_gemm8_launch<2, MODE>(a, num_cu, s);
}

static Gemm8Args gemm8_args(const void *XT, uint64_t n, uint32_t dim, const void *qfrag, const float *qscale, uint32_t ngroups,
                            const float *rowc) {
    VDB_REQUIRE(n < (1ull << 32), "flat_gemm8: too many rows for one shard");
    VDB_REQUIRE(gemm8_supported(dim), "flat_gemm8: unsupported dimension");
    Gemm8Args a{};
    a.XT = reinterpret_cast<const uint4 *>(XT);
    a.qfrag = reinterpret_cast<const uint4 *>(qfrag);
    a.qscale = qscale;
    a.rowc = reinterpret_cast<const float2 *>(rowc);
    a.n = n;
    a.KB = mfma_dim_pad(dim) / 64;
    a.ngroups = ngroups;
    a.unit_step = 1;
    return a;
}

void launch_flat_gemm8_filter(const void *XT, uint64_t n, uint32_t dim, const void *qfrag, const float *qscale, uint32_t ngroups,
                              const float *rowc, const float *tau, uint64_t *cand, uint32_t *cnt, uint32_t cap, int debug, int num_cu,
                              hipStream_t s, uint32_t hits_expected) {
    if (n == 0 || ngroups == 0) return;
    Gemm8Args a = gemm8_args(XT, n, dim, qfrag, qscale, ngroups, rowc);
    a.debug = (uint32_t)debug;
    a.tau = tau;
    a.cand = cand;
    a.cnt = cnt;
    a.sync = cnt + uint64_t(ngroups) * G8_BQ;
    a.cap = cap;
    a.hits_expected = hits_expected;
    const double mirror_bytes = double((n + 15) / 16 * 16) * mfma_dim_pad(dim);
    a.nt = g_gemm8_nt == 2 || (g_gemm8_nt == 0 && mirror_bytes > 384.0 * 1024 * 1024) ? 1u : 0u;
    flat_gemm8_dispatch<G8_FILTER>(a, num_cu, s);
}

uint64_t gemm8_sample_rows(uint64_t n, uint32_t unit_step) {
    const uint64_t units = ((n + 15) / 16 + G8_TW - 1) / G8_TW;
    return (units + unit_step - 1) / unit_step * (16 * G8_TW);
}
uint64_t gemm8_sample_units(uint64_t n, uint32_t unit_step) {
    const uint64_t units = ((n + 15) / 16 + G8_TW - 1) / G8_TW;
    return (units + unit_step - 1) / unit_step;
}
void launch_flat_gemm8_sample(const void *XT, uint64_t n, uint32_t dim, const void *qfrag, const float *qscale, uint32_t ngroups,
                              const float *rowc, uint32_t unit_step, float *out, uint64_t ld, int num_cu, hipStream_t s, int unit_min) {
    if (n == 0 || ngroups == 0) return;
    VDB_REQUIRE(unit_step >= 1 && (ld & 3) == 0 && ld >= (unit_min ? gemm8_sample_units(n, unit_step) : gemm8_sample_rows(n, unit_step)),
                "flat_gemm8: ld must cover the sample");
    VDB_REQUIRE(ngroups <= 65535, "flat_gemm8: too many query groups");
    Gemm8Args a = gemm8_args(XT, n, dim, qfrag, qscale, ngroups, rowc);
    a.unit_step = unit_step;
    a.out = out;
    a.ld = ld;
    a.unit_min = unit_min ? 1u : 0u;
    flat_gemm8_dispatch<G8_SAMPLE>(a, num_cu, s);
}

}
```

lab_1806_vec_db_amd/csrc/k_i8.hip:

```cpp
#include "common.hpp"
#include "kernels.hpp"

namespace vdb {

constexpr float I8_U = 5.9604645e-8f;

__global__ __launch_bounds__(256) void k_col_sum(const float *__restrict__ X, uint64_t n, uint32_t dim, uint64_t stride,
                                                 uint64_t n_s, float *__restrict__ part, const float *__restrict__ xsq) {
    const uint32_t col = blockIdx.x * 64 + (threadIdx.x & 63), sub = threadIdx.x >> 6;
    const uint64_t per = (n_s + gridDim.y - 1) / gridDim.y;
    const uint64_t a = uint64_t(blockIdx.y) * per, b = a + per < n_s ? a + per : n_s;
    float acc = 0.0f;
    if (col < dim)
        for (uint64_t i = a + sub; i < b; i += 4) {
            float v = X[(i * stride) * dim + col];
            if (xsq) {
                const float ns = xsq[i * stride];
                v = (ns >= 1e-30f && ns <= 1e30f) ? v / sqrtf(ns) : 0.0f;
            }
            acc += (v - v == 0.0f) ? v : 0.0f;
        }
    __shared__ float sh[256];
    sh[threadIdx.x] = acc;
    __syncthreads();
    if (sub == 0 && col < dim) part[uint64_t(blockIdx.y) * dim + col] = (sh[threadIdx.x] + sh[threadIdx.x + 64]) + (sh[threadIdx.x + 128] + sh[threadIdx.x + 192]);
}
__global__ void k_col_mean(const float *__restrict__ part, uint32_t chunks, uint32_t dim, float inv_rows, float *__restrict__ mu) {
    const uint32_t col = blockIdx.x * blockDim.x + threadIdx.x;
    if (col >= dim) return;
    float acc = 0.0f;
    for (uint32_t c = 0; c < chunks; c++) acc += part[uint64_t(c) * dim + col];
    mu[col] = acc * inv_rows;
}
void launch_i8_col_mean(const float *X, uint64_t n, uint32_t dim, float *part, float *mu, hipStream_t s, const float *xsq_cos) {
    const uint64_t n_s = n < 16384 ? n : 16384, stride = n / n_s;
    hipLaunchKernelGGL(k_col_sum, dim3((dim + 63) / 64, I8_MEAN_CHUNKS), dim3(256), 0, s, X, n, dim, stride, n_s, part, xsq_cos);
    hipLaunchKernelGGL(k_col_mean, dim3((dim + 63) / 64), dim3(64), 0, s, part, I8_MEAN_CHUNKS, dim, 1.0f / float(n_s), mu);
}

struct I8Row {
    float s;
    float xs;
    float e2;
    float i2;
    bool bad;
};
template <bool COS>
__device__ __forceinline__ float i8_centre(float a, float m, double inv) {
    if constexpr (COS)
        return float(double(a) * inv - double(m));
    else
        return a - m;
}
__device__ __forceinline__ double i8_sumsq64(const float *__restrict__ v, uint32_t dim, uint32_t sub) {
    double acc = 0.0;
    const float4 *v4 = reinterpret_cast<const float4 *>(v);
    for (uint32_t j = sub; j < dim / 4; j += 16) {
        const float4 a = v4[j];
        acc += double(a.x) * double(a.x) + double(a.y) * double(a.y);
        acc += double(a.z) * double(a.z) + double(a.w) * double(a.w);
    }
#pragma unroll
    for (int o = 8; o > 0; o >>= 1) acc += __shfl_xor(acc, o);
    return acc;
}
template <bool COS>
__device__ __forceinline__ void i8_pass1(const float *__restrict__ v, const float *__restrict__ mu, uint32_t dim, uint32_t sub, double inv,
                                         float &mx, float &xs, bool &bad) {
    mx = 0.0f;
    xs = 0.0f;
    bad = false;
    const float4 *v4 = reinterpret_cast<const float4 *>(v), *m4 = reinterpret_cast<const float4 *>(mu);
    for (uint32_t j = sub; j < dim / 4; j += 16) {
        const float4 a = v4[j], m = m4[j];
        const float c[4] = {i8_centre<COS>(a.x, m.x, inv), i8_centre<COS>(a.y, m.y, inv), i8_centre<COS>(a.z, m.z, inv), i8_centre<COS>(a.w, m.w, inv)};
#pragma unroll
        for (int e = 0; e < 4; e++) {
            mx = fmaxf(mx, fabsf(c[e]));
            xs += c[e] * c[e];
            bad |= !(c[e] - c[e] == 0.0f);
        }
    }
#pragma unroll
    for (int o = 8; o > 0; o >>= 1) {
        mx = fmaxf(mx, __shfl_xor(mx, o));
        xs += __shfl_xor(xs, o);
        bad |= __shfl_xor((int)bad, o) != 0;
    }
}
template <bool COS>
__device__ __forceinline__ uint4 i8_piece(const float *__restrict__ v, const float *__restrict__ mu, uint32_t dim, uint32_t c0, float s,
                                          float inv, double inv_n, bool zero, float &e2, float &i2) {
    uint32_t w[4] = {0u, 0u, 0u, 0u};
    if (zero || c0 >= dim) return make_uint4(0u, 0u, 0u, 0u);
#pragma unroll
    for (int k = 0; k < 4; k++) {
        if (c0 + 4 * k >= dim) break;
        const float4 a = *reinterpret_cast<const float4 *>(v + c0 + 4 * k), m = *reinterpret_cast<const float4 *>(mu + c0 + 4 * k);
        const float c[4] = {i8_centre<COS>(a.x, m.x, inv_n), i8_centre<COS>(a.y, m.y, inv_n), i8_centre<COS>(a.z, m.z, inv_n),
                            i8_centre<COS>(a.w, m.w, inv_n)};
#pragma unroll
        for (int e = 0; e < 4; e++) {
            float q = rintf(c[e] * inv);
            q = fminf(fmaxf(q, -127.0f), 127.0f);
            const float d = c[e] - q * s;
            e2 += d * d;
            i2 += q * q;
            w[k] |= (uint32_t(int(q)) & 0xffu) << (8 * e);
        }
    }
    return make_uint4(w[0], w[1], w[2], w[3]);
}
__device__ __forceinline__ float i8_scale(float mx, bool bad) { return (mx >= 1e-30f && mx <= 1e30f && !bad) ? mx / 127.0f : 1.0f; }

template <bool COS>
__global__ __launch_bounds__(256) void k_tile_rows_i8(const float *__restrict__ X, uint64_t n, uint32_t dim, uint64_t tile0,
                                                      const float *__restrict__ mu, float il1, float il2, uint4 *__restrict__ T,
                                                      float2 *__restrict__ rowc, float *__restrict__ stats, uint64_t stride,
                                                      const float *__restrict__ xsq, const uint32_t *__restrict__ tiles) {
    const uint32_t KB = ((dim + 63) & ~63u) / 64;
    const uint32_t grp = threadIdx.x >> 4, sub = threadIdx.x & 15;
    const uint64_t tile = tiles ? uint64_t(tiles[blockIdx.x]) : tile0 + blockIdx.x;
    const uint64_t row = stats ? (uint64_t(blockIdx.x) * 16 + grp) * stride : tile * 16 + grp;
    const bool live = row < n;
    const float *v = X + (live ? row : 0) * dim;
    double inv_n = 0.0;
    bool odd = false;
    if constexpr (COS) {
        const double s64 = i8_sumsq64(v, dim, sub);
        const float ns = xsq[live ? row : 0];
        inv_n = (s64 > 0.0 && s64 < 1e300) ? 1.0 / sqrt(s64) : 0.0;
        odd = !(s64 == 0.0 && ns == 0.0) && !(ns >= 1e-30f && ns <= 1e30f);
    }
    float mx, xs;
    bool bad;
    i8_pass1<COS>(v, mu, dim, sub, inv_n, mx, xs, bad);
    const float s = i8_scale(mx, bad), inv = 1.0f / s;
    const bool zero = !live || bad || odd || !(mx >= 1e-30f && mx <= 1e30f);
    float e2 = 0.0f, i2 = 0.0f;
    for (uint32_t pp = sub; pp < KB * 4; pp += 16) {
        const uint4 w = i8_piece<COS>(v, mu, dim, pp * 16, s, inv, inv_n, zero, e2, i2);
        if (T) T[(tile * KB + (pp >> 2)) * 64 + 16 * (pp & 3) + grp] = w;
    }
#pragma unroll
    for (int o = 8; o > 0; o >>= 1) {
        e2 += __shfl_xor(e2, o);
        i2 += __shfl_xor(i2, o);
    }
    if (zero && live && !bad) e2 = xs;
    if (sub != 0) return;
    if (stats) {
        stats[2 * (uint64_t(blockIdx.x) * 16 + grp)] = (live && !bad && !odd) ? e2 : 0.0f;
        stats[2 * (uint64_t(blockIdx.x) * 16 + grp) + 1] = (live && !bad && !odd) ? xs : 0.0f;
        return;
    }
    float2 out;
    if (!live) {
        out = make_float2(INFINITY, 0.0f);
    } else if (bad) {
        out = make_float2(__uint_as_float(0x7fc00000u), 0.0f);
    } else if (odd) {
        out = make_float2(-3.4028234664e38f, 0.0f);
    } else {
        const float du = 2.0f * float(dim + 8) * I8_U;
        const float xs_lo = xs * (1.0f - du);
        const float dxn = sqrtf(e2) * 1.001f + 4.0f * I8_U * sqrtf(xs) + (COS ? 1e-12f : 0.0f);
        const float xt2 = (s * s) * i2 * 1.001f;
        float c = xs_lo - dxn * dxn * il1 - xt2 * il2;
        c -= 8.0f * I8_U * (xs + dxn * dxn * il1 + xt2 * il2);
        out = make_float2(c, zero ? 0.0f : -2.0f * s);
    }
    rowc[row] = out;
}
void launch_tile_rows_i8(const float *X, uint64_t n, uint32_t dim, uint64_t tile0, uint64_t tile1, const float *mu, float l1, float l2,
                         void *T, float *rowc, hipStream_t s, const float *xsq_cos) {
    if (tile1 <= tile0) return;
    if (xsq_cos)
        hipLaunchKernelGGL(k_tile_rows_i8<true>, dim3((unsigned)(tile1 - tile0)), dim3(256), 0, s, X, n, dim, tile0, mu, 1.0f / l1, 1.0f / l2,
                           reinterpret_cast<uint4 *>(T), reinterpret_cast<float2 *>(rowc), (float *)nullptr, uint64_t(1), xsq_cos, (const uint32_t *)nullptr);
    else
        hipLaunchKernelGGL(k_tile_rows_i8<false>, dim3((unsigned)(tile1 - tile0)), dim3(256), 0, s, X, n, dim, tile0, mu, 1.0f / l1, 1.0f / l2,
                           reinterpret_cast<uint4 *>(T), reinterpret_cast<float2 *>(rowc), (float *)nullptr, uint64_t(1), (const float *)nullptr, (const uint32_t *)nullptr);
}
void launch_tile_rows_i8_list(const float *X, uint64_t n, uint32_t dim, const uint32_t *tiles, uint64_t n_tiles, const float *mu, float l1,
                              float l2, void *T, float *rowc, hipStream_t s, const float *xsq_cos) {
    if (n_tiles == 0) return;
    if (xsq_cos)
        hipLaunchKernelGGL(k_tile_rows_i8<true>, dim3((unsigned)n_tiles), dim3(256), 0, s, X, n, dim, uint64_t(0), mu, 1.0f / l1, 1.0f / l2,
                           reinterpret_cast<uint4 *>(T), reinterpret_cast<float2 *>(rowc), (float *)nullptr, uint64_t(1), xsq_cos, tiles);
    else
        hipLaunchKernelGGL(k_tile_rows_i8<false>, dim3((unsigned)n_tiles), dim3(256), 0, s, X, n, dim, uint64_t(0), mu, 1.0f / l1, 1.0f / l2,
                           reinterpret_cast<uint4 *>(T), reinterpret_cast<float2 *>(rowc), (float *)nullptr, uint64_t(1), (const float *)nullptr,
                           tiles);
}
void launch_i8_row_stats(const float *X, uint64_t n, uint32_t dim, const float *mu, uint64_t n_s, uint64_t stride, float *stats,
                         hipStream_t s, const float *xsq_cos) {
    if (n_s == 0) return;
    if (xsq_cos)
        hipLaunchKernelGGL(k_tile_rows_i8<true>, dim3((unsigned)((n_s + 15) / 16)), dim3(256), 0, s, X, n, dim, uint64_t(0), mu, 1.0f, 1.0f,
                           (uint4 *)nullptr, (float2 *)nullptr, stats, stride, xsq_cos, (const uint32_t *)nullptr);
    else
        hipLaunchKernelGGL(k_tile_rows_i8<false>, dim3((unsigned)((n_s + 15) / 16)), dim3(256), 0, s, X, n, dim, uint64_t(0), mu, 1.0f, 1.0f,
                           (uint4 *)nullptr, (float2 *)nullptr, stats, stride, (const float *)nullptr, (const uint32_t *)nullptr);
}

template <bool COS>
__global__ __launch_bounds__(512) void k_query_prep_i8(const float *__restrict__ Q, uint32_t nq, uint32_t nq_pad, uint32_t dim,
                                                       const float *__restrict__ mu, float l1, float l2, float *__restrict__ qsq,
                                                       float *__restrict__ qscale, float *__restrict__ qoff,
                                                       uint32_t *__restrict__ hits, uint4 *__restrict__ qfrag) {
    extern __shared__ float qp8_smem[];
    const uint32_t lane = threadIdx.x & 63, wave = threadIdx.x >> 6;
    if (blockIdx.x == 0 && threadIdx.x < 128) hits[nq_pad + threadIdx.x] = 0;
    const uint32_t q = blockIdx.x * 4 + (wave & 3);
    if (q >= nq_pad) return;
    constexpr uint32_t NH = 8;
    const uint32_t KB = ((dim + 63) & ~63u) / 64;
    uint4 *dst = qfrag + uint64_t(q / (16 * NH)) * KB * NH * 64;
    const uint32_t h = (q % (16 * NH)) / 16, r = q & 15;
    if (q >= nq) {
        if (wave >= 4) return;
        for (uint32_t pp = lane; pp < KB * 4; pp += 64) dst[((pp >> 2) * NH + h) * 64 + 16 * (pp & 3) + r] = make_uint4(0u, 0u, 0u, 0u);
        if (lane == 0) {
            qscale[q] = 0.0f;
            qoff[q] = 0.0f;
            hits[q] = 0;
        }
        return;
    }
    const float *qv = Q + size_t(q) * dim;
    float *sq = qp8_smem + size_t(wave) * dim;
    for (uint32_t j = lane; j < dim; j += 64) sq[j] = qv[j];
    if (wave >= 4) {
        if (lane != 0) return;
        float qs = 0.0f;
        const float4 *s4 = reinterpret_cast<const float4 *>(sq);
        const uint32_t nv = dim / 4;
        uint32_t i = 0;
        for (; i + 8 <= nv; i += 8) {
            float4 t[8];
#pragma unroll
            for (int u = 0; u < 8; u++) t[u] = s4[i + u];
#pragma unroll
            for (int u = 0; u < 8; u++) {
                const float p0 = t[u].x * t[u].x, p1 = t[u].y * t[u].y, p2 = t[u].z * t[u].z, p3 = t[u].w * t[u].w;
                qs = qs + p0;
                qs = qs + p1;
                qs = qs + p2;
                qs = qs + p3;
            }
        }
        for (uint32_t j = i * 4; j < dim; j++) qs = qs + sq[j] * sq[j];
        qsq[q] = qs;
        return;
    }
    float mx, xs;
    bool bad;
    double inv_n = 0.0;
    bool odd = false;
    if constexpr (COS) {
        const double s64 = i8_sumsq64(sq, dim, lane & 15);
        odd = !(s64 >= 1e-29 && s64 <= 1e29);
        inv_n = odd ? 0.0 : 1.0 / sqrt(s64);
    }
    i8_pass1<COS>(sq, mu, dim, lane & 15, inv_n, mx, xs, bad);
    bad |= odd;
    const float s = i8_scale(mx, bad), inv = 1.0f / s;
    const bool zero = bad || !(mx >= 1e-30f && mx <= 1e30f);
    float e2 = 0.0f, i2 = 0.0f;
    for (uint32_t pp = lane; pp < KB * 4; pp += 64)
        dst[((pp >> 2) * NH + h) * 64 + 16 * (pp & 3) + r] = i8_piece<COS>(sq, mu, dim, pp * 16, s, inv, inv_n, zero, e2, i2);
#pragma unroll
    for (int o = 32; o > 0; o >>= 1) e2 += __shfl_xor(e2, o);
    if (zero && !bad) e2 = xs;
    if (lane == 0) {
        float off;
        if (bad) {
            off = __uint_as_float(0x7fc00000u);
        } else {
            const float du = 2.0f * float(dim + 8) * I8_U;
            const float dqn = sqrtf(e2) * 1.001f + 4.0f * I8_U * sqrtf(xs) + (COS ? 1e-12f : 0.0f);
            const float w1 = 1.0f - l1;
            off = (w1 >= 0.0f ? xs * (1.0f - du) : xs * (1.0f + du)) * w1 - l2 * dqn * dqn;
            off -= 8.0f * I8_U * (xs * fabsf(w1) + l2 * dqn * dqn);
        }
        qscale[q] = (zero || bad) ? 0.0f : s;
        qoff[q] = off;
        hits[q] = 0;
    }
}
void launch_query_prep_i8(const float *Q, uint32_t nq, uint32_t nq_pad, uint32_t dim, const float *mu, float l1, float l2, float *qsq,
                          float *qscale, float *qoff, uint32_t *hits, void *qfrag, hipStream_t s, int cosine) {
    if (nq_pad == 0) return;
    if (size_t(8) * dim * sizeof(float) > size_t(48) * 1024) {
        func_max_lds(reinterpret_cast<const void *>(&k_query_prep_i8<true>), int(64 * 1024));
        func_max_lds(reinterpret_cast<const void *>(&k_query_prep_i8<false>), int(64 * 1024));
    }
    if (cosine)
        hipLaunchKernelGGL(k_query_prep_i8<true>, dim3((nq_pad + 3) / 4), dim3(512), size_t(8) * dim * sizeof(float), s, Q, nq, nq_pad, dim, mu,
                           l1, l2, qsq, qscale, qoff, hits, reinterpret_cast<uint4 *>(qfrag));
    else
        hipLaunchKernelGGL(k_query_prep_i8<false>, dim3((nq_pad + 3) / 4), dim3(512), size_t(8) * dim * sizeof(float), s, Q, nq, nq_pad, dim, mu,
                           l1, l2, qsq, qscale, qoff, hits, reinterpret_cast<uint4 *>(qfrag));
}

}
```

lab_1806_vec_db_amd/csrc/kernels.hpp:

```cpp
#pragma once
#include <hip/hip_runtime.h>

#include <cstdint>

namespace vdb {

enum Metric : int {
    MET_L2_DIRECT = 0,
    MET_COSINE = 1,
    MET_L2_CACHED = 2,
};

void launch_row_sqnorm(const float *X, uint64_t n, uint32_t dim, float *sq, hipStream_t s);
void launch_scan_exact(const float *X, uint64_t n, uint32_t dim, const float *Q, uint32_t nq, int metric,
                       const float *xsq, const float *qsq, float *out, uint64_t ld, bool use_lds, hipStream_t s);
void launch_rerank(const float *X, uint32_t dim, const float *Q, uint32_t nq, int metric, const float *xsq,
                   const float *qsq, const uint64_t *cand, uint64_t *out, uint32_t ncand, uint32_t ldc,
                   hipStream_t s, const uint32_t *cnt = nullptr);
void launch_finalize(const uint64_t *keys, uint32_t ldk, uint32_t nq, uint32_t ksel, uint32_t kstride,
                     uint64_t id_offset, uint64_t *out_idx, float *out_dist, uint64_t *out_count, hipStream_t s);
void launch_iota_keys(uint64_t *rows, uint32_t nq, uint32_t n, uint32_t ld, hipStream_t s);
struct SplitErr {
    const float *qerr = nullptr;
    float dx_abs = 0.0f, dx_rel = 0.0f;
// ... 17 lines not shown
    int metric;
    const float *xsq, *qsq;
    uint64_t n_rows;
    float xsq_max, xsq_min_pos;
    int cosine;
    SplitErr se;
    uint64_t id_offset;
    uint8_t *flags;
    uint64_t *out_idx;
    float *out_dist;
    uint64_t *out_count;
    unsigned long long *stamps = nullptr;
    const float *tau = nullptr;
    uint32_t *qstat = nullptr;
};
bool flat_tail_lb_supported(uint32_t dim, uint32_t kprime, uint32_t ksel);
void launch_flat_tail_lb(const FlatTailArgs &a, uint32_t nq, hipStream_t s);
void launch_flat_full_lb(const FlatTailArgs &a, uint32_t nq, uint64_t *exact_keys, uint64_t *topk, hipStream_t s);
void flat_tail_lb_set_nw(int v);
void flat_tail_lb_set_walk(int v);
bool flat_tail64_supported(uint32_t dim, uint32_t kprime, uint32_t ksel);
void launch_flat_tail64(const FlatTailArgs &a, uint32_t nq, hipStream_t s);
struct FlatSmallArgs {
    const float *X;
    uint64_t n;
    uint32_t dim;
    const float *Q;
    int metric;
    const float *xsq;
    uint64_t *part;
    uint32_t *counter;
    uint32_t ksel, kstride;
    uint64_t id_offset;
    uint64_t *out_idx;
    float *out_dist;
    uint64_t *out_count;
};
bool flat_small_supported(uint64_t n, uint32_t dim, uint64_t nq, uint64_t k);
uint32_t flat_small_rows_per_wg(uint64_t n, int num_cu);
size_t flat_small_part_keys(uint64_t n, uint64_t nq, uint32_t ksel, int num_cu);
void launch_flat_small(const FlatSmallArgs &a, uint32_t nq, int num_cu, hipStream_t s);
void launch_certify(const uint64_t *exact_sorted, uint32_t lde, const uint64_t *approx_sorted, uint32_t lda,
                    uint32_t nq, uint32_t k, uint32_t kprime, uint64_t n_rows, const float *qsq, float xsq_max,
                    float xsq_min_pos, int cosine, uint32_t dim, uint8_t *flags, hipStream_t s);

void launch_extract_tau(const uint64_t *sorted, uint32_t ld, uint32_t nq, uint32_t kprime, float *tau, hipStream_t s);
void launch_flag_overflow(const uint32_t *cnt, uint32_t cap, uint32_t min_hits, uint32_t nq, uint8_t *flags,
                          hipStream_t s);

uint32_t topk_chunk(uint64_t n);
uint32_t topk_num_lists(uint64_t n);
void launch_select_tau(const float *keys, uint64_t ld, uint32_t n, uint32_t nq, uint32_t nq_real, uint32_t kth, float *tau,
                       hipStream_t s);
uint32_t select_tau_max_n();
uint32_t topk_capacity(uint32_t k);
void launch_topk_dense(const float *keys, uint64_t ld, uint64_t n, uint32_t nq, uint32_t k, uint64_t *lists,
                       hipStream_t s);
void launch_topk_merge(const uint64_t *lists, uint32_t nlists, uint32_t cap_in, uint32_t nq, uint32_t k,
                       uint64_t *out, hipStream_t s);

void launch_topk_merge_counted(const uint64_t *lists, uint32_t cap_in, const uint32_t *cnt, uint32_t nq, uint32_t k,
                               uint64_t *out, hipStream_t s);
void launch_merge_shards64(const float *dists, const uint64_t *ids, const uint64_t *counts, uint64_t stride_d,
                           uint64_t stride_i, uint64_t stride_c, uint32_t S, uint32_t nq, uint32_t k, uint64_t *out_idx,
                           float *out_dist, uint64_t *out_count, hipStream_t s);
void launch_pack_pairs(const float *dists, const uint64_t *ids, const uint64_t *counts, uint64_t stride_d,
                       uint64_t stride_i, uint64_t stride_c , uint32_t S, uint32_t nq, uint32_t k,
                       uint32_t cap_in, uint64_t *lists, hipStream_t s);

void launch_widen_u8(const uint8_t *in, uint64_t count, float *out, hipStream_t s);
void launch_scan_exact_u8(const uint8_t *X, uint64_t n, uint32_t dim, const float *Q, uint32_t nq, int metric, const float *xsq,
                          const float *qsq, float *out, uint64_t ld, hipStream_t s);
void launch_rerank_u8(const uint8_t *X, uint32_t dim, const float *Q, uint32_t nq, int metric, const float *xsq, const float *qsq,
                      const uint64_t *cand, uint64_t *out, uint32_t ncand, uint32_t ldc, hipStream_t s);

double stream_probe(int device, uint64_t bytes, int iters);
double stream_probe_pattern(int device, uint64_t bytes, int iters, int pattern, uint32_t row_bytes);
void mfma_probe(int device, int waves_per_simd, int iters, double *tflops, double *clock_ghz, int i8 = 0);
double latency_probe(int device, uint64_t bytes, uint32_t hops);
double fold_probe(int device, uint32_t adds);

size_t sort_pairs_temp_bytes(uint64_t n);
void launch_sort_pairs(const float *dist, uint64_t n, uint64_t *tmp_keys, uint64_t *out, void *temp, size_t temp_bytes,
                       hipStream_t s);

size_t sort_rows_temp_bytes(uint64_t nq, uint64_t ld);
void launch_sort_rows(const uint64_t *in, uint64_t *out, uint64_t nq, uint64_t ld, void *temp, size_t temp_bytes, hipStream_t s);
void launch_pair_keys_rows(const float *dist, uint64_t ldd, uint64_t n, uint32_t nq, uint64_t *keys, uint64_t ldk, hipStream_t s);
void launch_copy_prefix(const uint64_t *in, uint64_t ld_in, uint64_t *out, uint64_t ld_out, uint64_t count, uint32_t nq, hipStream_t s);
void launch_resort_big(const uint64_t *offers, uint32_t ncand, uint32_t ldc, uint32_t nq, uint32_t k, uint64_t *out, uint32_t ldo,
                       hipStream_t s);

uint32_t mfma_batch(uint32_t dim);
void launch_mfma_pack_queries(const float *Q, uint32_t nq, uint32_t nq_cover, uint32_t dim, float *qfrag, hipStream_t s);
void launch_tile_rows(const float *X, uint64_t n, uint32_t dim, uint64_t tile0, uint64_t tile1, float *T,
                      hipStream_t s);
void launch_tile_rows_list(const float *X, uint64_t n, uint32_t dim, const uint32_t *tiles, uint64_t n_tiles, float *T, hipStream_t s);
void launch_flat_mfma_sample(const float *XT, uint64_t n, uint32_t dim, const float *qfrag, uint32_t nbatch,
                             const float *xsq, int cosine, uint32_t step, float *out, uint64_t ld, int num_cu,
                             hipStream_t s);
void launch_flat_mfma_filter(const float *XT, uint64_t n, uint32_t dim, const float *qfrag, uint32_t nbatch,
                             const float *xsq, int cosine, const float *tau, uint64_t *cand, uint32_t *cnt,
                             uint32_t cap, uint32_t *sync , int num_cu, hipStream_t s);
size_t mfma_sync_words(uint32_t nbatch, int num_cu);
void launch_flat_gemm_filter(const float *XT, uint64_t n, uint32_t dim, const float *qfrag, const float *qmul, uint32_t ngroups,
                             const float *xsq, int cosine, const float *tau, uint64_t *cand, uint32_t *cnt,
                             uint32_t cap, int debug, int num_cu, hipStream_t s);
uint32_t gemm_group();
uint64_t gemm_sample_rows(uint64_t n, uint32_t unit_step);
void launch_flat_gemm_sample(const float *XT, uint64_t n, uint32_t dim, const float *qfrag, const float *qmul, uint32_t ngroups,
                             const float *xsq, int cosine, uint32_t unit_step, float *out, uint64_t ld, int num_cu,
                             hipStream_t s);
void gemm_set_tw(int v);
void gemm_set_zigzag(int v);
void gemm_set_nt(int v);
void gemm_set_block_rows(uint64_t v);
void gemm_set_stagger(int v);
bool gemm_f16_supported(uint32_t dim);
void launch_tile_rows_h(const float *X, uint64_t n, uint32_t dim, uint64_t tile0, uint64_t tile1, float sx, void *T,
                        hipStream_t s);
void launch_tile_rows_h_list(const float *X, uint64_t n, uint32_t dim, const uint32_t *tiles, uint64_t n_tiles, float sx, void *T,
                             hipStream_t s);
void launch_row_split_err(const float *X, const float *xsq, uint64_t row0, uint64_t row1, uint32_t dim, float sx,
                          uint32_t *out2 , hipStream_t s);
void launch_rows_to_half(const float *X, uint64_t count, float sx, uint16_t *H, hipStream_t s);
void launch_rows_to_q8(const float *X, uint64_t n, uint32_t dim, int8_t *Q8, float *scale, float *err, hipStream_t s);
void launch_query_prep_h(const float *Q, uint32_t nq, uint32_t nq_pad, uint32_t dim, float sx, float *qsq ,
                         float *qscale, float *qmul, float *qerr, uint32_t *hits ,
                         void *qfrag , hipStream_t s);
void launch_pack_queries_h(const float *Q, uint32_t nq, uint32_t nq_cover, uint32_t dim, uint32_t NH, const float *qscale,
                           void *qfrag, hipStream_t s);
void launch_mfma_pack_queries_nh(const float *Q, uint32_t nq, uint32_t nq_cover, uint32_t dim, uint32_t NH, float *qfrag,
                                 hipStream_t s);
constexpr uint32_t I8_MEAN_CHUNKS = 64;
bool gemm8_supported(uint32_t dim);
void gemm8_set_nt(int v);
void gemm8_set_kc(int v);
void gemm8_set_burst(int v);
uint32_t gemm8_last_coop();
uint32_t gemm_last_coop();
void gemm_set_coop(int v);
void gemm8_set_grid(int v);
void gemm8_set_epi(int v);
void gemm8_set_coop(int v);
void gemm8_set_res(int v);
void gemm8_set_sample_res(int v);
uint64_t gemm8_sample_rows(uint64_t n, uint32_t unit_step);
void launch_flat_gemm8_filter(const void *XT, uint64_t n, uint32_t dim, const void *qfrag, const float *qscale, uint32_t ngroups,
                              const float *rowc, const float *tau, uint64_t *cand, uint32_t *cnt, uint32_t cap, int debug, int num_cu,
                              hipStream_t s, uint32_t hits_expected = 0);
void launch_flat_gemm8_sample(const void *XT, uint64_t n, uint32_t dim, const void *qfrag, const float *qscale, uint32_t ngroups,
                              const float *rowc, uint32_t unit_step, float *out, uint64_t ld, int num_cu, hipStream_t s, int unit_min = 0);
uint64_t gemm8_sample_units(uint64_t n, uint32_t unit_step);
void launch_i8_col_mean(const float *X, uint64_t n, uint32_t dim, float *part , float *mu, hipStream_t s,
                        const float *xsq_cos = nullptr);
void launch_i8_row_stats(const float *X, uint64_t n, uint32_t dim, const float *mu, uint64_t n_s, uint64_t stride,
                         float *stats , hipStream_t s, const float *xsq_cos = nullptr);
void launch_tile_rows_i8(const float *X, uint64_t n, uint32_t dim, uint64_t tile0, uint64_t tile1, const float *mu, float l1, float l2,
                         void *T, float *rowc, hipStream_t s, const float *xsq_cos = nullptr);
void launch_tile_rows_i8_list(const float *X, uint64_t n, uint32_t dim, const uint32_t *tiles, uint64_t n_tiles, const float *mu, float l1,
                              float l2, void *T, float *rowc, hipStream_t s, const float *xsq_cos = nullptr);
void launch_rows_move(void *rows, uint64_t row_bytes, float *sq, const uint32_t *moves, uint64_t n_moves, int num_cu, hipStream_t s);
void launch_query_prep_i8(const float *Q, uint32_t nq, uint32_t nq_pad, uint32_t dim, const float *mu, float l1, float l2, float *qsq,
                          float *qscale, float *qoff, uint32_t *hits, void *qfrag, hipStream_t s, int cosine = 0);
void launch_gather_rows_f32(const float *src, const uint64_t *rows, uint64_t nr, uint32_t width, float *dst, hipStream_t s);
void launch_scatter_results(const uint64_t *ri, const float *rd, const uint64_t *rc, const uint64_t *rows, uint64_t nr, uint32_t k,
                            uint64_t *o_idx, float *o_dist, uint64_t *o_cnt, hipStream_t s);
void launch_gather_dk(const float *o_dist, const uint64_t *o_cnt, const uint64_t *rows, uint64_t nr, uint32_t k, uint32_t ksel, float *dk,
                      hipStream_t s);
void launch_flat_refine_half(const uint16_t *rows_h, uint32_t dim, float sx, float dx_abs, float dx_rel, int cosine, const float *Q, const float *xsq,
                             const float *qsq, const float *qoff, uint64_t *cand, uint32_t cap, const uint32_t *cnt, uint32_t nq, uint32_t max_hits,
                             hipStream_t s);
void launch_i8_tau_from_dk(const float *dk, uint32_t nq, uint32_t nq_pad, const float *qoff, const float *qsq, float xsq_max, float mu_norm,
                           uint32_t dim, int cosine, float *tau, hipStream_t s);
constexpr uint32_t RANGE_LEFT = 0xFFFFFFFFu;
void launch_range_admit(const float *radius, uint32_t nq, const float *qoff, const float *qsq, float xsq_max, float xsq_min_pos, float mu_norm,
                        uint32_t dim, int cosine, float *tau, hipStream_t s);
void launch_range_cut(uint64_t *keys, uint32_t cap, const uint32_t *cnt, const float *radius, const float *tau, uint32_t nq, uint32_t *o_cnt,
                      uint32_t *o_hits, hipStream_t s);
uint32_t range_scan_blocks(uint64_t n);
void launch_range_scan_select(const float *dist, uint64_t ld, uint64_t n, const float *radius, uint32_t nq, uint32_t *blk, uint32_t *total,
                              hipStream_t s);
void launch_range_compact(const float *dist, uint64_t ld, uint64_t n, const float *radius, uint32_t nq, const uint32_t *blk_off, uint64_t *out,
                          uint64_t ldo, hipStream_t s);
void launch_range_append(const uint64_t *keys, uint64_t ld, const uint64_t *off, const uint32_t *take, uint32_t nq, uint64_t max_take, uint64_t *pool,
                         hipStream_t s);
void launch_range_gather(const uint64_t *pool, const uint64_t *off, const uint64_t *lims, uint64_t nq, uint64_t max_take, uint64_t id_offset,
                         uint64_t *out_idx, float *out_dist, hipStream_t s);
void launch_scan_gather(const float *X, const uint32_t *ids, uint64_t m, uint32_t dim, const float *Q, uint32_t nq, int metric, const float *xsq,
                        const float *qsq, float *out, uint64_t ld, bool use_lds, hipStream_t s);
void launch_filter_finalize(const uint64_t *keys, uint64_t ldk, uint32_t nq, uint32_t ksel, uint32_t kstride, const uint32_t *ids, uint64_t m,
                            uint64_t id_offset, uint64_t *out_idx, float *out_dist, uint64_t *out_count, hipStream_t s);
struct GroupedItem {
    const uint32_t *ids;
    uint32_t m;
    uint32_t tile;
    uint32_t slot;
    uint32_t nb;
};
void launch_scan_gather_grouped(const float *X, uint32_t dim, const GroupedItem *items, uint64_t nitems, const uint32_t *slot_q, const float *Q,
                                int metric, const float *xsq, const float *qsq, float *out, uint64_t ld, hipStream_t s);
void launch_filter_finalize_grouped(const uint64_t *keys, uint64_t ldk, uint32_t nslots, uint32_t ksel, uint32_t kstride, const uint32_t *const *slot_ids,
                                    const uint32_t *slot_m, const uint32_t *slot_q, uint64_t id_offset, uint64_t *out_idx, float *out_dist,
                                    uint64_t *out_count, hipStream_t s);
void launch_mask_rowc(const float *rowc, const uint64_t *bits, uint64_t n, uint64_t rows_pad, float *out, hipStream_t s);
void launch_tau_clamp(float *tau, uint32_t nq, hipStream_t s);
void launch_mask_dense_nan(float *dist, uint64_t ld, uint64_t n, uint32_t nq, const uint64_t *bits, hipStream_t s);
void mfma_set_sample_thin(int v);
void mfma_sample_plan(uint64_t n, uint32_t kprime, uint32_t *step, uint32_t *rank, uint32_t target_floor = 1024);
uint64_t mfma_sample_rows(uint64_t n, uint32_t step);
size_t mfma_qfrag_floats(uint32_t dim);
uint32_t mfma_dim_pad(uint32_t dim);
void mfma_set_variant(int v);
void mfma_set_share(int v);
uint32_t mfma_share();
uint64_t mfma_row_pad();
bool mfma_supported(uint32_t dim);

}
```

Baseline: 1.083 million queries/s.

## Fuse int8 query preparation into the resident gemm8 threshold-sample kernel

Result: no change. 1.085 million queries/s (median of 3 runs) (+0.1%).

```diff
diff --git a/lab_1806_vec_db_amd/csrc/api.hip b/lab_1806_vec_db_amd/csrc/api.hip
--- a/lab_1806_vec_db_amd/csrc/api.hip
+++ b/lab_1806_vec_db_amd/csrc/api.hip
@@ -792,7 +792,9 @@
     VDB_REQUIRE(idx && queries && out_keys, "null argument");
     Index &ix = idx->ix;
     VDB_REQUIRE(dim == ix.dim, "query dimension mismatch");
-    VDB_REQUIRE(tier >= 0 && tier <= 2, "tier must be 0 (fp16 operands), 1 (split-bf16 operands) or 2 (8-bit operands, lower-bound keys)");
+    VDB_REQUIRE(tier >= 0 && tier <= 4,
+                "tier must be 0 (fp16 operands), 1 (split-bf16 operands), 2 (8-bit operands, lower-bound keys), 3 (the same with the query scales) or 4 "
+                "(the 8-bit pass's threshold sample)");
     ix.use_device();
     WsLease ws(ix);
     ws->q.reserve(nq * ix.dim * sizeof(float));
@@ -920,6 +922,8 @@
         gemm8_set_grid((int)value);
     else if (n == "flat_gemm8_epi")
         gemm8_set_epi((int)value);
+    else if (n == "flat_i8_prep_fused")
+        gemm8_set_prep_fused((int)value);
     else if (n == "flat_gemm_coop")
         gemm_set_coop((int)value);
     else if (n == "flat_half_kmul") {
@@ -960,6 +964,8 @@
         *out = gemm_last_coop();
     else if (n == "flat_gemm8_coop_sets")
         *out = gemm8_last_coop();
+    else if (n == "flat_i8_prep_fused_launches")
+        *out = idx->ix.i8_prep_fused_launches.load();
     else if (n == "flat_i8_queries")
         *out = idx->ix.i8_queries.load();
     else if (n == "flat_i8_redo")
diff --git a/lab_1806_vec_db_amd/csrc/i8_quant.hpp b/lab_1806_vec_db_amd/csrc/i8_quant.hpp
--- /dev/null
+++ b/lab_1806_vec_db_amd/csrc/i8_quant.hpp
@@ -0,0 +1,171 @@
+#pragma once
+#include "common.hpp"
+
+namespace vdb {
+
+constexpr float I8_U = 5.9604645e-8f;
+
+struct I8Row {
+    float s;
+    float xs;
+    float e2;
+    float i2;
+    bool bad;
+};
+template <bool COS>
+__device__ __forceinline__ float i8_centre(float a, float m, double inv) {
+    if constexpr (COS)
+        return float(double(a) * inv - double(m));
+    else
+        return a - m;
+}
+template <bool COS>
+__device__ __forceinline__ float4 i8_centre4(const float4 a, const float4 m, double inv) {
+    return make_float4(i8_centre<COS>(a.x, m.x, inv), i8_centre<COS>(a.y, m.y, inv), i8_centre<COS>(a.z, m.z, inv), i8_centre<COS>(a.w, m.w, inv));
+}
+__device__ __forceinline__ double i8_sumsq64(const float *__restrict__ v, uint32_t dim, uint32_t sub) {
+    double acc = 0.0;
+    const float4 *v4 = reinterpret_cast<const float4 *>(v);
+    for (uint32_t j = sub; j < dim / 4; j += 16) {
+        const float4 a = v4[j];
+        acc += double(a.x) * double(a.x) + double(a.y) * double(a.y);
+        acc += double(a.z) * double(a.z) + double(a.w) * double(a.w);
+    }
+#pragma unroll
+    for (int o = 8; o > 0; o >>= 1) acc += __shfl_xor(acc, o);
+    return acc;
+}
+template <class F>
+__device__ __forceinline__ void i8_pass1_c(F centred, uint32_t dim, uint32_t sub, float &mx, float &xs, bool &bad) {
+    mx = 0.0f;
+    xs = 0.0f;
+    float nf = 0.0f;
+    for (uint32_t j = sub; j < dim / 4; j += 16) {
+        const float4 c4 = centred(j);
+        const float c[4] = {c4.x, c4.y, c4.z, c4.w};
+#pragma unroll
+        for (int e = 0; e < 4; e++) {
+            mx = fmaxf(mx, fabsf(c[e]));
+            xs += c[e] * c[e];
+            nf = __builtin_fmaf(c[e], 0.0f, nf);
+        }
+    }
+    bad = !(nf == 0.0f);
+#pragma unroll
+    for (int o = 8; o > 0; o >>= 1) {
+        mx = fmaxf(mx, __shfl_xor(mx, o));
+        xs += __shfl_xor(xs, o);
+        bad |= __shfl_xor((int)bad, o) != 0;
+    }
+}
+template <bool COS>
+__device__ __forceinline__ void i8_pass1(const float *__restrict__ v, const float *__restrict__ mu, uint32_t dim, uint32_t sub, double inv,
+                                         float &mx, float &xs, bool &bad) {
+    const float4 *v4 = reinterpret_cast<const float4 *>(v), *m4 = reinterpret_cast<const float4 *>(mu);
+    i8_pass1_c([&](uint32_t j) { return i8_centre4<COS>(v4[j], m4[j], inv); }, dim, sub, mx, xs, bad);
+}
+template <class F>
+__device__ __forceinline__ uint4 i8_piece_c(F centred, uint32_t dim, uint32_t c0, float s, float inv, bool zero, float &e2, float &i2) {
+    uint32_t w[4] = {0u, 0u, 0u, 0u};
+    if (zero || c0 >= dim) return make_uint4(0u, 0u, 0u, 0u);
+#pragma unroll
+    for (int k = 0; k < 4; k++) {
+        if (c0 + 4 * k >= dim) break;
+        const float4 c4 = centred(c0 + 4 * k);
+        const float c[4] = {c4.x, c4.y, c4.z, c4.w};
+#pragma unroll
+        for (int e = 0; e < 4; e++) {
+            float q = rintf(c[e] * inv);
+            q = fminf(fmaxf(q, -127.0f), 127.0f);
+            const float d = c[e] - q * s;
+            e2 += d * d;
+            i2 += q * q;
+            w[k] |= (uint32_t(int(q)) & 0xffu) << (8 * e);
+        }
+    }
+    return make_uint4(w[0], w[1], w[2], w[3]);
+}
+template <bool COS>
+__device__ __forceinline__ uint4 i8_piece(const float *__restrict__ v, const float *__restrict__ mu, uint32_t dim, uint32_t c0, float s,
+                                          float inv, double inv_n, bool zero, float &e2, float &i2) {
+    return i8_piece_c(
+        [&](uint32_t col) {
+            return i8_centre4<COS>(*reinterpret_cast<const float4 *>(v + col), *reinterpret_cast<const float4 *>(mu + col), inv_n);
+        },
+        dim, c0, s, inv, zero, e2, i2);
+}
+__device__ __forceinline__ float i8_scale(float mx, bool bad) { return (mx >= 1e-30f && mx <= 1e30f && !bad) ? mx / 127.0f : 1.0f; }
+
+struct I8QueryHead {
+    double inv_n;
+    float s, inv;
+    float xs;
+    bool bad;
+    bool zero;
+};
+template <bool COS, bool KEEP>
+__device__ __forceinline__ I8QueryHead i8_query_head(float *v, const float *__restrict__ mu, uint32_t dim, uint32_t sub) {
+    I8QueryHead h;
+    h.inv_n = 0.0;
+    bool odd = false;
+    if constexpr (COS) {
+        const double s64 = i8_sumsq64(v, dim, sub);
+        odd = !(s64 >= 1e-29 && s64 <= 1e29);
+        h.inv_n = odd ? 0.0 : 1.0 / sqrt(s64);
+    }
+    float mx;
+    if constexpr (KEEP) {
+        float4 *v4 = reinterpret_cast<float4 *>(v);
+        const float4 *m4 = reinterpret_cast<const float4 *>(mu);
+        const double inv_n = h.inv_n;
+        i8_pass1_c(
+            [&](uint32_t j) {
+                const float4 c = i8_centre4<COS>(v4[j], m4[j], inv_n);
+                v4[j] = c;
+                return c;
+            },
+            dim, sub, mx, h.xs, h.bad);
+    } else {
+        i8_pass1<COS>(v, mu, dim, sub, h.inv_n, mx, h.xs, h.bad);
+    }
+    h.bad |= odd;
+    h.s = i8_scale(mx, h.bad);
+    h.inv = 1.0f / h.s;
+    h.zero = h.bad || !(mx >= 1e-30f && mx <= 1e30f);
+    return h;
+}
+template <bool COS>
+__device__ __forceinline__ float i8_query_off(float xs, float e2, bool zero, bool bad, uint32_t dim, float l1, float l2) {
+    if (zero && !bad) e2 = xs;
+    if (bad) return __uint_as_float(0x7fc00000u);
+    const float du = 2.0f * float(dim + 8) * I8_U;
+    const float dqn = sqrtf(e2) * 1.001f + 4.0f * I8_U * sqrtf(xs) + (COS ? 1e-12f : 0.0f);
+    const float w1 = 1.0f - l1;
+    float off = (w1 >= 0.0f ? xs * (1.0f - du) : xs * (1.0f + du)) * w1 - l2 * dqn * dqn;
+    off -= 8.0f * I8_U * (xs * fabsf(w1) + l2 * dqn * dqn);
+    return off;
+}
+__device__ __forceinline__ float i8_query_scale(float s, bool zero, bool bad) { return (zero || bad) ? 0.0f : s; }
+__device__ __forceinline__ float i8_fold_sq(const float *sq, uint32_t dim) {
+    float qs = 0.0f;
+    const float4 *s4 = reinterpret_cast<const float4 *>(sq);
+    const uint32_t nv = dim / 4;
+    uint32_t i = 0;
+    for (; i + 8 <= nv; i += 8) {
+        float4 t[8];
+#pragma unroll
+        for (int u = 0; u < 8; u++) t[u] = s4[i + u];
+#pragma unroll
+        for (int u = 0; u < 8; u++) {
+            const float p0 = t[u].x * t[u].x, p1 = t[u].y * t[u].y, p2 = t[u].z * t[u].z, p3 = t[u].w * t[u].w;
+            qs = qs + p0;
+            qs = qs + p1;
+            qs = qs + p2;
+            qs = qs + p3;
+        }
+    }
+    for (uint32_t j = i * 4; j < dim; j++) qs = qs + sq[j] * sq[j];
+    return qs;
+}
+
+}
diff --git a/lab_1806_vec_db_amd/csrc/index.hip b/lab_1806_vec_db_amd/csrc/index.hip
--- a/lab_1806_vec_db_amd/csrc/index.hip
+++ b/lab_1806_vec_db_amd/csrc/index.hip
@@ -578,7 +578,7 @@
     pass_ev_valid = true;
 }
 
-I8Queries Index::i8_query_prep(Workspace &ws, const float *Q, uint64_t nb) {
+I8Queries Index::i8_query_reserve(Workspace &ws, uint64_t nb) {
     I8Queries qp;
     const uint64_t gq = gemm_group();
     qp.ngroups = (nb + gq - 1) / gq;
@@ -592,6 +592,10 @@
     qp.d_hits = reinterpret_cast<uint32_t *>(qp.d_tau + qp.nq_pad);
     qp.d_qscale = ws.qaux.as<float>();
     qp.d_qoff = qp.d_qscale + qp.nq_pad;
+    return qp;
+}
+I8Queries Index::i8_query_prep(Workspace &ws, const float *Q, uint64_t nb) {
+    const I8Queries qp = i8_query_reserve(ws, nb);
     launch_query_prep_i8(Q, (uint32_t)nb, (uint32_t)qp.nq_pad, (uint32_t)dim, d_mu_i8.as<float>(), i8_l1, i8_l2, ws.qsq.as<float>(), qp.d_qscale,
                          qp.d_qoff, qp.d_hits, ws.qfrag_g.p, ws.stream, dist == 1 ? 1 : 0);
     return qp;
@@ -605,6 +609,20 @@
     sp.unit_min = flat_i8_unit_min != 1 && units >= (flat_i8_unit_min == 2 ? 2ull : 16ull) * sp.s_rank;
     sp.set_keys(sp.unit_min ? units : gemm8_sample_rows(n, sp.s_step));
     return sp;
+}
+
+I8Queries Index::i8_prep_and_sample(Workspace &ws, const float *Q, uint64_t nb, const float *rowc, const TauSample &sp) {
+    if (gemm8_prep_fused() != 0 || !gemm8_sample_fused_applies((uint32_t)dim)) {
+        const I8Queries qp = i8_query_prep(ws, Q, nb);
+        i8_sample(ws, qp, rowc, sp);
+        return qp;
+    }
+    const I8Queries qp = i8_query_reserve(ws, nb);
+    launch_flat_gemm8_sample_fused(d_tiled_i8.p, n, (uint32_t)dim, Q, (uint32_t)nb, d_mu_i8.as<float>(), i8_l1, i8_l2, dist == 1 ? 1 : 0, ws.qsq.as<float>(),
+                                   qp.d_qscale, qp.d_qoff, qp.d_hits, ws.qfrag_g.p, (uint32_t)qp.ngroups, rowc, sp.s_step, ws.dense.as<float>(), sp.ld_s,
+                                   num_cu, ws.stream, sp.unit_min ? 1 : 0);
+    i8_prep_fused_launches++;
+    return qp;
 }
 
 void Index::i8_sample(Workspace &ws, const I8Queries &qp, const float *rowc, const TauSample &sp) {
@@ -761,7 +779,7 @@
     const size_t sync_words = mfma_sync_words((uint32_t)nbatch, num_cu);
     I8Queries qp;
     if (i8) {
-        qp = i8_query_prep(ws, d_q, nq);
+        qp = i8_second ? i8_query_prep(ws, d_q, nq) : i8_prep_and_sample(ws, d_q, nq, d_rowc_i8.as<float>(), sp);
     } else {
         ws.misc.reserve(nq_pad * (sizeof(float) + sizeof(uint32_t)) + sync_words * sizeof(uint32_t));
         qp.d_tau = ws.misc.as<float>();
@@ -790,7 +808,7 @@
                               d_tau, s);
     } else {
         if (i8)
-            i8_sample(ws, qp, d_rowc_i8.as<float>(), sp);
+            ;
         else if (gemm)
             launch_flat_gemm_sample(xt, n, (uint32_t)dim, ws.qfrag_g.as<float>(), d_qmul, (uint32_t)ngroups,
                                     d_sq.as<float>(), cosine, sp.s_step, ws.dense.as<float>(), sp.ld_s, num_cu, s);
@@ -1222,11 +1240,11 @@
     for (uint64_t q0 = 0; q0 < nq; q0 += QCH) {
         const uint64_t nb = std::min<uint64_t>(QCH, nq - q0);
         const float *Q = d_q + q0 * dim;
-        const I8Queries qp = i8_query_prep(ws, Q, nb);
-        ws.dense.reserve(qp.nq_pad * sp.ld_s * sizeof(float));
-        ws.lists.reserve(std::max<size_t>(qp.nq_pad * size_t(sp.nl_s) * sp.cap_s, qp.nq_pad * size_t(FLAT_CAND_CAP)) * sizeof(uint64_t));
-        ws.keys_a.reserve(qp.nq_pad * size_t(sp.cap_s) * sizeof(uint64_t));
-        i8_sample(ws, qp, rowc, sp);
+        const uint64_t nb_pad = (nb + gemm_group() - 1) / gemm_group() * gemm_group();
+        ws.dense.reserve(nb_pad * sp.ld_s * sizeof(float));
+        ws.lists.reserve(std::max<size_t>(nb_pad * size_t(sp.nl_s) * sp.cap_s, nb_pad * size_t(FLAT_CAND_CAP)) * sizeof(uint64_t));
+        ws.keys_a.reserve(nb_pad * size_t(sp.cap_s) * sizeof(uint64_t));
+        const I8Queries qp = i8_prep_and_sample(ws, Q, nb, rowc, sp);
         select_tau(ws, sp, qp.nq_pad, nb, qp.d_tau);
         launch_tau_clamp(qp.d_tau, (uint32_t)qp.nq_pad, s);
         i8_filter(ws, qp, rowc, "flat_filtered_i8", std::max<uint32_t>(64u, sp.s_step * sp.s_rank));
@@ -1358,23 +1376,32 @@
     VDB_REQUIRE(mfma_supported((uint32_t)dim), "debug keys: the dimension has no MFMA shortlist path");
     const int cosine = dist == 1 ? 1 : 0;
     const uint64_t gq = gemm_group(), ngroups = (nq + gq - 1) / gq, nq_pad = ngroups * gq;
-    if (tier == 2) {
+    if (tier >= 2) {
         VDB_REQUIRE(!elem_u8 && (dim & 3) == 0 && gemm8_supported((uint32_t)dim), "debug keys: the index has no 8-bit pass");
         VDB_REQUIRE(ensure_i8(ws), "debug keys: the 8-bit mirror could not be allocated");
         TauSample sp;
-        sp.set_keys(gemm8_sample_rows(n, 1));
-        const I8Queries qp = i8_query_prep(ws, d_q, nq);
-        ws.dense.reserve(qp.nq_pad * sp.ld_s * sizeof(float));
-        i8_sample(ws, qp, d_rowc_i8.as<float>(), sp);
-        VDB_HIP(hipMemcpy2DAsync(h_keys, n * sizeof(float), ws.dense.p, sp.ld_s * sizeof(float), n * sizeof(float), nq, hipMemcpyDeviceToHost, s));
+        if (tier == 4)
+            sp = i8_sample_plan();
+        else
+            sp.set_keys(gemm8_sample_rows(n, 1));
+        ws.dense.reserve(nq_pad * sp.ld_s * sizeof(float));
+        if (tier == 4) {
+            ws.lists.reserve(nq_pad * size_t(sp.nl_s) * sp.cap_s * sizeof(uint64_t));
+            ws.keys_a.reserve(nq_pad * size_t(sp.cap_s) * sizeof(uint64_t));
+        }
+        const I8Queries qp = i8_prep_and_sample(ws, d_q, nq, d_rowc_i8.as<float>(), sp);
+        if (tier == 4) select_tau(ws, sp, qp.nq_pad, nq, qp.d_tau);
+        const uint64_t cols = tier == 4 ? std::min<uint64_t>(sp.n_s, n) : n;
+        VDB_HIP(hipMemcpy2DAsync(h_keys, n * sizeof(float), ws.dense.p, sp.ld_s * sizeof(float), cols * sizeof(float), nq, hipMemcpyDeviceToHost, s));
         if (h_qsq) VDB_HIP(hipMemcpyAsync(h_qsq, ws.qsq.p, nq * sizeof(float), hipMemcpyDeviceToHost, s));
-        if (h_qerr) VDB_HIP(hipMemcpyAsync(h_qerr, qp.d_qoff, nq * sizeof(float), hipMemcpyDeviceToHost, s));
+        if (h_qerr)
+            VDB_HIP(hipMemcpyAsync(h_qerr, tier == 4 ? qp.d_tau : (tier == 3 ? qp.d_qscale : qp.d_qoff), nq * sizeof(float), hipMemcpyDeviceToHost, s));
         VDB_SYNC(s);
         if (h_dx) {
-            h_dx[0] = i8_l1;
-            h_dx[1] = i8_l2;
-            h_dx[2] = i8_mu_norm;
-            h_dx[3] = 0.0f;
+            h_dx[0] = tier == 4 ? float(cols) : i8_l1;
+            h_dx[1] = tier == 4 ? float(sp.s_step) : i8_l2;
+            h_dx[2] = tier == 4 ? float(sp.s_rank) : i8_mu_norm;
+            h_dx[3] = tier == 4 && sp.unit_min ? 1.0f : 0.0f;
         }
         return;
     }
diff --git a/lab_1806_vec_db_amd/csrc/index.hpp b/lab_1806_vec_db_amd/csrc/index.hpp
--- a/lab_1806_vec_db_amd/csrc/index.hpp
+++ b/lab_1806_vec_db_amd/csrc/index.hpp
@@ -328,6 +328,7 @@
     int flat_i8_unit_min = 0;
     int flat_i8_second = 0;
     std::atomic<uint64_t> i8_second_queries{0}, i8_second_redo{0};
+    std::atomic<uint64_t> i8_prep_fused_launches{0};
     uint32_t flat_i8_hits = 1024;
     std::atomic<uint64_t> i8_queries{0}, i8_redo{0};
     int flat_i8_stats = 0;
@@ -403,6 +404,8 @@
     template <class F>
     void corpus_pass(Workspace &ws, const char *name, double bytes, F launch);
     I8Queries i8_query_prep(Workspace &ws, const float *Q, uint64_t nb);
+    I8Queries i8_query_reserve(Workspace &ws, uint64_t nb);
+    I8Queries i8_prep_and_sample(Workspace &ws, const float *Q, uint64_t nb, const float *rowc, const TauSample &sp);
     TauSample i8_sample_plan() const;
     void i8_sample(Workspace &ws, const I8Queries &qp, const float *rowc, const TauSample &sp);
     void select_tau(Workspace &ws, const TauSample &sp, uint64_t nq_pad, uint64_t nq, float *d_tau);
diff --git a/lab_1806_vec_db_amd/csrc/k_gemm8.hip b/lab_1806_vec_db_amd/csrc/k_gemm8.hip
--- a/lab_1806_vec_db_amd/csrc/k_gemm8.hip
+++ b/lab_1806_vec_db_amd/csrc/k_gemm8.hip
@@ -3,6 +3,7 @@
 
 #include "common.hpp"
 #include "kernels.hpp"
+#include "i8_quant.hpp"
 
 namespace vdb {
 
@@ -37,15 +38,25 @@
     uint32_t coop_block;
     uint32_t hits_expected;
     uint32_t *sync;
+    const float *Q;
+    const float *mu;
+    uint32_t nq, dim;
+    uint32_t cosine;
+    float l1, l2;
+    float *qsq_w, *qscale_w, *qoff_w;
+    uint4 *qfrag_w;
+    uint32_t *hits_w;
 };
+constexpr uint32_t G8_FOLD_WG = 4;
 
 enum { G8_FILTER = 0, G8_SAMPLE = 1 };
 #ifndef G8_ABLATE
 #define G8_ABLATE 0
 #endif
 
-template <int KC, int MODE, bool XNT, bool BURST, bool RES, int EPI>
+template <int KC, int MODE, bool XNT, bool BURST, bool RES, int EPI, int PREP = 0>
 __global__ __launch_bounds__(512, 1) void k_flat_gemm8(Gemm8Args a) {
+    static_assert(PREP == 0 || (MODE == G8_SAMPLE && RES && !XNT), "the fused form is a resident sample launch");
     constexpr int TW = G8_TW, NT = 512, NW = 8, NH = G8_NH, R = KC;
     constexpr uint32_t CHUNK = KC * NH * 64;
     constexpr int QST = CHUNK / NT;
@@ -63,7 +74,23 @@
     float *stage_s = m_s + 8 * 64;
 
     const uint32_t lane = threadIdx.x & 63, wave = __builtin_amdgcn_readfirstlane(threadIdx.x >> 6);
-    const uint32_t nwaves = gridDim.x * NW, gw = blockIdx.x * NW + wave;
+    const uint32_t nwg = PREP ? gridDim.x - G8_FOLD_WG : gridDim.x;
+    if constexpr (PREP != 0) {
+        if (blockIdx.x >= nwg) {
+            const uint32_t per = G8_BQ / G8_FOLD_WG, q0 = blockIdx.y * G8_BQ + (blockIdx.x - nwg) * per;
+            float *st = reinterpret_cast<float *>(smem8);
+            const uint32_t nv = a.dim / 4;
+            for (uint32_t i = threadIdx.x; i < per * nv; i += NT) {
+                const uint32_t q = q0 + i / nv;
+                if (q < a.nq) reinterpret_cast<float4 *>(st)[i] = reinterpret_cast<const float4 *>(a.Q)[uint64_t(q) * nv + i % nv];
+            }
+            __syncthreads();
+            const uint32_t ql = wave * (per / NW) + lane;
+            if (lane < per / NW && q0 + ql < a.nq) a.qsq_w[q0 + ql] = i8_fold_sq(st + size_t(ql) * a.dim, a.dim);
+            return;
+        }
+    }
+    const uint32_t nwaves = nwg * NW, gw = blockIdx.x * NW + wave;
     const uint32_t KB = a.KB, nchunk = KB / KC;
     const uint64_t n = a.n;
 
@@ -78,7 +105,7 @@
     const uint32_t c_steps_max = c_base0 < a.n_units ? (a.n_units - c_base0 + c_stride - 1) / c_stride : 0u;
     auto adv = [&](uint32_t slot) -> uint32_t {
         if (coop) return slot;
-        return slot >= rw ? slot - rw : slot + gridDim.x - rw;
+        return slot >= rw ? slot - rw : slot + nwg - rw;
     };
     auto steps_of = [&](uint32_t slot) -> uint32_t {
         if (coop) return c_steps;
@@ -141,7 +168,106 @@
     uint32_t stage_n = 0;
     for (uint32_t grp = g_begin + c_member; grp < g_end; grp += coop ? coopS : 1u) {
         const uint4 *qgrp = a.qfrag + uint64_t(grp) * nchunk * CHUNK;
-        if constexpr (RES) {
+        if constexpr (PREP != 0) {
+            constexpr bool COS = PREP == 2;
+            const uint32_t dim = a.dim, nv = dim / 4, dpad = KB * 64;
+            float *mu_s = reinterpret_cast<float *>(hit_key);
+            float *stg = reinterpret_cast<float *>(smem8) + wave * 4 * dpad;
+            for (uint32_t j = threadIdx.x; j < nv; j += NT) reinterpret_cast<float4 *>(mu_s)[j] = reinterpret_cast<const float4 *>(a.mu)[j];
+            const uint32_t qg0 = grp * G8_BQ + wave * 16;
+            float4 pf0, pf1, pf2, pf3, pf4, pf5, pf6, pf7, pf8, pf9, pf10, pf11, pf12, pf13, pf14, pf15;
+            uint4 im0, im1, im2, im3, im4, im5, im6, im7, im8, im9, im10, im11, im12, im13, im14, im15;
+#define G8_NAMED16(P, I)                                                                                                                      \
+    if constexpr (I == 0) return P##0; else if constexpr (I == 1) return P##1; else if constexpr (I == 2) return P##2;                        \
+    else if constexpr (I == 3) return P##3; else if constexpr (I == 4) return P##4; else if constexpr (I == 5) return P##5;                   \
+    else if constexpr (I == 6) return P##6; else if constexpr (I == 7) return P##7; else if constexpr (I == 8) return P##8;                   \
+    else if constexpr (I == 9) return P##9; else if constexpr (I == 10) return P##10; else if constexpr (I == 11) return P##11;               \
+    else if constexpr (I == 12) return P##12; else if constexpr (I == 13) return P##13; else if constexpr (I == 14) return P##14;             \
+    else return P##15;
+            auto pf = [&](auto I) -> float4 & { G8_NAMED16(pf, decltype(I)::value) };
+            auto img = [&](auto I) -> uint4 & { G8_NAMED16(im, decltype(I)::value) };
+#undef G8_NAMED16
+            auto each16 = [&](auto f) {
+#define G8_F4(B) f(std::integral_constant<int, B>{}), f(std::integral_constant<int, B + 1>{}), f(std::integral_constant<int, B + 2>{}), f(std::integral_constant<int, B + 3>{})
+                G8_F4(0), G8_F4(4), G8_F4(8), G8_F4(12);
+#undef G8_F4
+            };
+            auto prefetch = [&](uint32_t t) {
+                each16([&](auto I) {
+                    constexpr int g = decltype(I)::value >> 2, i = decltype(I)::value & 3;
+                    const uint32_t q = qg0 + 4 * t + g;
+                    const float4 *src = reinterpret_cast<const float4 *>(a.Q) + uint64_t(q < a.nq ? q : 0) * nv;
+                    pf(I) = src[lane + 64 * i < nv ? lane + 64 * i : 0];
+                });
+            };
+            prefetch(0);
+            __syncthreads();
+            const uint32_t sub = lane & 15, gl = lane >> 4;
+            float my_xs = 0.0f, my_e2 = 0.0f, my_s = 0.0f;
+            uint32_t my_flags = 0;
+            auto round = [&](auto T) {
+                constexpr int t = decltype(T)::value;
+                each16([&](auto I) {
+                    constexpr int g = decltype(I)::value >> 2, i = decltype(I)::value & 3;
+                    if (lane + 64 * i < nv) reinterpret_cast<float4 *>(stg + g * dpad)[lane + 64 * i] = pf(I);
+                });
+                if (t < 3) prefetch(t + 1);
+                __builtin_amdgcn_fence(__ATOMIC_RELEASE, "wavefront");
+                __builtin_amdgcn_wave_barrier();
+                __builtin_amdgcn_fence(__ATOMIC_ACQUIRE, "wavefront");
+                const I8QueryHead hd = i8_query_head<COS, true>(stg + gl * dpad, mu_s, dim, sub);
+                __builtin_amdgcn_fence(__ATOMIC_RELEASE, "wavefront");
+                __builtin_amdgcn_wave_barrier();
+                __builtin_amdgcn_fence(__ATOMIC_ACQUIRE, "wavefront");
+                auto one = [&](auto G) {
+                    constexpr int g = decltype(G)::value;
+                    const uint32_t ql = wave * 16 + 4 * t + g, q = grp * G8_BQ + ql;
+                    const int src = 16 * g;
+                    const float s = __int_as_float(__builtin_amdgcn_readlane(__float_as_int(hd.s), src));
+                    const float inv = __int_as_float(__builtin_amdgcn_readlane(__float_as_int(hd.inv), src));
+                    const float xs = __int_as_float(__builtin_amdgcn_readlane(__float_as_int(hd.xs), src));
+                    const bool zero = __builtin_amdgcn_readlane((int)hd.zero, src) != 0, bad = __builtin_amdgcn_readlane((int)hd.bad, src) != 0;
+                    float e2 = 0.0f, i2 = 0.0f;
+                    const float *cq = stg + g * dpad;
+                    uint4 w = i8_piece_c([&](uint32_t col) { return *reinterpret_cast<const float4 *>(cq + col); }, dim, lane * 16, s, inv, zero, e2, i2);
+#pragma unroll
+                    for (int o = 32; o > 0; o >>= 1) e2 += __shfl_xor(e2, o);
+                    if (q >= a.nq) w = make_uint4(0u, 0u, 0u, 0u);
+                    img(std::integral_constant<int, 4 * t + g>{}) = w;
+                    if (ql % nwg == blockIdx.x && lane < KB * 4)
+                        a.qfrag_w[(uint64_t(grp) * KB * NH + (lane >> 2) * NH + wave) * 64 + 16 * (lane & 3) + (4 * t + g)] = w;
+                    if (lane == 4 * t + g) {
+                        my_xs = xs;
+                        my_e2 = e2;
+                        my_s = s;
+                        my_flags = (zero ? 1u : 0u) | (bad ? 2u : 0u);
+                    }
+                };
+                one(std::integral_constant<int, 0>{});
+                one(std::integral_constant<int, 1>{});
+                one(std::integral_constant<int, 2>{});
+                one(std::integral_constant<int, 3>{});
+            };
+            round(std::integral_constant<int, 0>{});
+            round(std::integral_constant<int, 1>{});
+            round(std::integral_constant<int, 2>{});
+            round(std::integral_constant<int, 3>{});
+            if (lane < 16) {
+                const uint32_t ql = wave * 16 + lane, q = grp * G8_BQ + ql;
+                const bool zero = (my_flags & 1u) != 0, bad = (my_flags & 2u) != 0, pad = q >= a.nq;
+                const float off = pad ? 0.0f : i8_query_off<COS>(my_xs, my_e2, zero, bad, dim, a.l1, a.l2);
+                const float sc = pad ? 0.0f : i8_query_scale(my_s, zero, bad);
+                qs_s[ql] = sc;
+                if (ql % nwg == blockIdx.x) {
+                    a.qscale_w[q] = sc;
+                    a.qoff_w[q] = off;
+                    a.hits_w[q] = 0;
+                }
+            }
+            if (blockIdx.x == 0 && blockIdx.y == 0 && threadIdx.x < 128) a.hits_w[a.ngroups * G8_BQ + threadIdx.x] = 0;
+            __syncthreads();
+            if (lane < KB * 4) each16([&](auto I) { smem8[((lane >> 2) * NH + wave) * 64 + 16 * (lane & 3) + decltype(I)::value] = img(I); });
+        } else if constexpr (RES) {
             for (uint32_t c = 0; c < nchunk; c++) {
                 uint4 t[QST];
 #pragma unroll
@@ -152,7 +278,7 @@
         }
         if (MODE == G8_FILTER && threadIdx.x < 1 + 2 * G8_BQ) hit_n[threadIdx.x] = 0;
         if (MODE == G8_FILTER && threadIdx.x < G8_BQ) tau_s[threadIdx.x] = (a.debug & 1) ? -INFINITY : a.tau[grp * G8_BQ + threadIdx.x];
-        if (threadIdx.x < G8_BQ) qs_s[threadIdx.x] = a.qscale[grp * G8_BQ + threadIdx.x];
+        if (PREP == 0 && threadIdx.x < G8_BQ) qs_s[threadIdx.x] = a.qscale[grp * G8_BQ + threadIdx.x];
         if constexpr (RES) __syncthreads();
         i32x4 qr0 = {0, 0, 0, 0}, qr1 = qr0, qr2 = qr0, qr3 = qr0;
         if constexpr (RES) {
@@ -498,7 +624,13 @@
     VDB_REQUIRE(v == 0 || v == 1, "flat_gemm8_epi: 0 (scalar arithmetic, carried stage) or 1 (packed arithmetic, one drain per unit)");
     g_gemm8_epi = v;
 }
-template <int KC, int MODE, bool XNT, bool BURST, bool RES, int EPI>
+static std::atomic<int> g_gemm8_prep_fused{1};
+void gemm8_set_prep_fused(int v) {
+    VDB_REQUIRE(v == 0 || v == 1, "flat_i8_prep_fused: 0 (the threshold sample prepares the queries) or 1 (a launch of its own)");
+    g_gemm8_prep_fused = v;
+}
+int gemm8_prep_fused() { return g_gemm8_prep_fused; }
+template <int KC, int MODE, bool XNT, bool BURST, bool RES, int EPI, int PREP = 0>
 static void flat_gemm8_launch2(const Gemm8Args &a0, int num_cu, hipStream_t s) {
     Gemm8Args a = a0;
     const uint64_t n_tiles = (a.n + 15) / 16;
@@ -518,12 +650,27 @@
     const size_t lds = RES ? gemm8_res_lds(a.KB)
                            : size_t(2) * KC * G8_NH * 64 * sizeof(uint4) + size_t(G8_WGBUF) * 12 + (4 + 4 * G8_BQ + 2 * 8 * 64) * 4 +
                                  size_t(8) * G8_STAGE * 24 + 16;
-    func_max_lds(reinterpret_cast<const void *>(&k_flat_gemm8<KC, MODE, XNT, BURST, RES, EPI>), int(160 * 1024));
-    hipLaunchKernelGGL((k_flat_gemm8<KC, MODE, XNT, BURST, RES, EPI>), dim3(grid, MODE == G8_SAMPLE ? a.ngroups : 1), dim3(512), lds, s, a);
+    if (PREP) grid += G8_FOLD_WG;
+    func_max_lds(reinterpret_cast<const void *>(&k_flat_gemm8<KC, MODE, XNT, BURST, RES, EPI, PREP>), int(160 * 1024));
+    hipLaunchKernelGGL((k_flat_gemm8<KC, MODE, XNT, BURST, RES, EPI, PREP>), dim3(grid, MODE == G8_SAMPLE ? a.ngroups : 1), dim3(512), lds, s, a);
     VDB_HIP(hipGetLastError());
 }
 template <int KC, int MODE, bool XNT, bool BURST, bool RES>
 static void flat_gemm8_launch1(const Gemm8Args &a, int num_cu, hipStream_t s) {
+    if constexpr (MODE == G8_SAMPLE && RES && !XNT) {
+        if (a.Q) {
+            const bool cos = a.cosine != 0;
+            if (g_gemm8_epi == 1) {
+                if (cos) flat_gemm8_launch2<KC, MODE, XNT, BURST, RES, 1, 2>(a, num_cu, s);
+                else flat_gemm8_launch2<KC, MODE, XNT, BURST, RES, 1, 1>(a, num_cu, s);
+            } else {
+                if (cos) flat_gemm8_launch2<KC, MODE, XNT, BURST, RES, 0, 2>(a, num_cu, s);
+                else flat_gemm8_launch2<KC, MODE, XNT, BURST, RES, 0, 1>(a, num_cu, s);
+            }
+            return;
+        }
+    }
+    VDB_REQUIRE(a.Q == nullptr, "flat_gemm8: the fused sample needs the resident form");
     if (g_gemm8_epi == 1)
         flat_gemm8_launch2<KC, MODE, XNT, BURST, RES, 1>(a, num_cu, s);
     else
@@ -655,6 +802,38 @@
     const uint64_t units = ((n + 15) / 16 + G8_TW - 1) / G8_TW;
     return (units + unit_step - 1) / unit_step;
 }
+bool gemm8_sample_fused_applies(uint32_t dim) {
+    if ((dim & 3) != 0 || !gemm8_supported(dim)) return false;
+    const uint32_t KB = mfma_dim_pad(dim) / 64;
+    return g_gemm8_res != 1 && g_gemm8_sample_res != 1 && gemm8_res_lds(KB) <= size_t(160) * 1024 && KB * 4 <= 64;
+}
+void launch_flat_gemm8_sample_fused(const void *XT, uint64_t n, uint32_t dim, const float *Q, uint32_t nq, const float *mu, float l1, float l2,
+                                    int cosine, float *qsq, float *qscale, float *qoff, uint32_t *hits, void *qfrag, uint32_t ngroups,
+                                    const float *rowc, uint32_t unit_step, float *out, uint64_t ld, int num_cu, hipStream_t s, int unit_min) {
+    if (n == 0 || ngroups == 0) return;
+    VDB_REQUIRE(gemm8_sample_fused_applies(dim), "flat_gemm8: no fused sample form for this dimension");
+    VDB_REQUIRE(unit_step >= 1 && (ld & 3) == 0 && ld >= (unit_min ? gemm8_sample_units(n, unit_step) : gemm8_sample_rows(n, unit_step)),
+                "flat_gemm8: ld must cover the sample");
+    VDB_REQUIRE(ngroups <= 65535 && nq >= 1 && nq <= ngroups * G8_BQ && nq > (ngroups - 1) * G8_BQ, "flat_gemm8: query groups do not match the queries");
+    Gemm8Args a = gemm8_args(XT, n, dim, qfrag, qscale, ngroups, rowc);
+    a.unit_step = unit_step;
+    a.out = out;
+    a.ld = ld;
+    a.unit_min = unit_min ? 1u : 0u;
+    a.Q = Q;
+    a.mu = mu;
+    a.nq = nq;
+    a.dim = dim;
+    a.cosine = cosine ? 1u : 0u;
+    a.l1 = l1;
+    a.l2 = l2;
+    a.qsq_w = qsq;
+    a.qscale_w = qscale;
+    a.qoff_w = qoff;
+    a.qfrag_w = reinterpret_cast<uint4 *>(qfrag);
+    a.hits_w = hits;
+    flat_gemm8_dispatch<G8_SAMPLE>(a, num_cu, s);
+}
 void launch_flat_gemm8_sample(const void *XT, uint64_t n, uint32_t dim, const void *qfrag, const float *qscale, uint32_t ngroups,
                               const float *rowc, uint32_t unit_step, float *out, uint64_t ld, int num_cu, hipStream_t s, int unit_min) {
     if (n == 0 || ngroups == 0) return;
diff --git a/lab_1806_vec_db_amd/csrc/k_i8.hip b/lab_1806_vec_db_amd/csrc/k_i8.hip
--- a/lab_1806_vec_db_amd/csrc/k_i8.hip
+++ b/lab_1806_vec_db_amd/csrc/k_i8.hip
@@ -1,9 +1,9 @@
 #include "common.hpp"
 #include "kernels.hpp"
+#include "i8_quant.hpp"
 
 namespace vdb {
 
-constexpr float I8_U = 5.9604645e-8f;
 
 __global__ __launch_bounds__(256) void k_col_sum(const float *__restrict__ X, uint64_t n, uint32_t dim, uint64_t stride,
                                                  uint64_t n_s, float *__restrict__ part, const float *__restrict__ xsq) {
@@ -37,81 +37,6 @@
     hipLaunchKernelGGL(k_col_sum, dim3((dim + 63) / 64, I8_MEAN_CHUNKS), dim3(256), 0, s, X, n, dim, stride, n_s, part, xsq_cos);
     hipLaunchKernelGGL(k_col_mean, dim3((dim + 63) / 64), dim3(64), 0, s, part, I8_MEAN_CHUNKS, dim, 1.0f / float(n_s), mu);
 }
-
-struct I8Row {
-    float s;
-    float xs;
-    float e2;
-    float i2;
-    bool bad;
-};
-template <bool COS>
-__device__ __forceinline__ float i8_centre(float a, float m, double inv) {
-    if constexpr (COS)
-        return float(double(a) * inv - double(m));
-    else
-        return a - m;
-}
-__device__ __forceinline__ double i8_sumsq64(const float *__restrict__ v, uint32_t dim, uint32_t sub) {
-    double acc = 0.0;
-    const float4 *v4 = reinterpret_cast<const float4 *>(v);
-    for (uint32_t j = sub; j < dim / 4; j += 16) {
-        const float4 a = v4[j];
-        acc += double(a.x) * double(a.x) + double(a.y) * double(a.y);
-        acc += double(a.z) * double(a.z) + double(a.w) * double(a.w);
-    }
-#pragma unroll
-    for (int o = 8; o > 0; o >>= 1) acc += __shfl_xor(acc, o);
-    return acc;
-}
-template <bool COS>
-__device__ __forceinline__ void i8_pass1(const float *__restrict__ v, const float *__restrict__ mu, uint32_t dim, uint32_t sub, double inv,
-                                         float &mx, float &xs, bool &bad) {
-    mx = 0.0f;
-    xs = 0.0f;
-    bad = false;
-    const float4 *v4 = reinterpret_cast<const float4 *>(v), *m4 = reinterpret_cast<const float4 *>(mu);
-    for (uint32_t j = sub; j < dim / 4; j += 16) {
-        const float4 a = v4[j], m = m4[j];
-        const float c[4] = {i8_centre<COS>(a.x, m.x, inv), i8_centre<COS>(a.y, m.y, inv), i8_centre<COS>(a.z, m.z, inv), i8_centre<COS>(a.w, m.w, inv)};
-#pragma unroll
-        for (int e = 0; e < 4; e++) {
-            mx = fmaxf(mx, fabsf(c[e]));
-            xs += c[e] * c[e];
-            bad |= !(c[e] - c[e] == 0.0f);
-        }
-    }
-#pragma unroll
-    for (int o = 8; o > 0; o >>= 1) {
-        mx = fmaxf(mx, __shfl_xor(mx, o));
-        xs += __shfl_xor(xs, o);
-        bad |= __shfl_xor((int)bad, o) != 0;
-    }
-}
-template <bool COS>
-__device__ __forceinline__ uint4 i8_piece(const float *__restrict__ v, const float *__restrict__ mu, uint32_t dim, uint32_t c0, float s,
-                                          float inv, double inv_n, bool zero, float &e2, float &i2) {
-    uint32_t w[4] = {0u, 0u, 0u, 0u};
-    if (zero || c0 >= dim) return make_uint4(0u, 0u, 0u, 0u);
-#pragma unroll
-    for (int k = 0; k < 4; k++) {
-        if (c0 + 4 * k >= dim) break;
-        const float4 a = *reinterpret_cast<const float4 *>(v + c0 + 4 * k), m = *reinterpret_cast<const float4 *>(mu + c0 + 4 * k);
-        const float c[4] = {i8_centre<COS>(a.x, m.x, inv_n), i8_centre<COS>(a.y, m.y, inv_n), i8_centre<COS>(a.z, m.z, inv_n),
-                            i8_centre<COS>(a.w, m.w, inv_n)};
-#pragma unroll
-        for (int e = 0; e < 4; e++) {
-            float q = rintf(c[e] * inv);
-            q = fminf(fmaxf(q, -127.0f), 127.0f);
-            const float d = c[e] - q * s;
-            e2 += d * d;
-            i2 += q * q;
-            w[k] |= (uint32_t(int(q)) & 0xffu) << (8 * e);
-        }
-    }
-    return make_uint4(w[0], w[1], w[2], w[3]);
-}
-__device__ __forceinline__ float i8_scale(float mx, bool bad) { return (mx >= 1e-30f && mx <= 1e30f && !bad) ? mx / 127.0f : 1.0f; }
 
 template <bool COS>
 __global__ __launch_bounds__(256) void k_tile_rows_i8(const float *__restrict__ X, uint64_t n, uint32_t dim, uint64_t tile0,
@@ -232,59 +157,18 @@
     float *sq = qp8_smem + size_t(wave) * dim;
     for (uint32_t j = lane; j < dim; j += 64) sq[j] = qv[j];
     if (wave >= 4) {
-        if (lane != 0) return;
-        float qs = 0.0f;
-        const float4 *s4 = reinterpret_cast<const float4 *>(sq);
-        const uint32_t nv = dim / 4;
-        uint32_t i = 0;
-        for (; i + 8 <= nv; i += 8) {
-            float4 t[8];
-#pragma unroll
-            for (int u = 0; u < 8; u++) t[u] = s4[i + u];
-#pragma unroll
-            for (int u = 0; u < 8; u++) {
-                const float p0 = t[u].x * t[u].x, p1 = t[u].y * t[u].y, p2 = t[u].z * t[u].z, p3 = t[u].w * t[u].w;
-                qs = qs + p0;
-                qs = qs + p1;
-                qs = qs + p2;
-                qs = qs + p3;
-            }
-        }
-        for (uint32_t j = i * 4; j < dim; j++) qs = qs + sq[j] * sq[j];
-        qsq[q] = qs;
+        if (lane == 0) qsq[q] = i8_fold_sq(sq, dim);
         return;
     }
-    float mx, xs;
-    bool bad;
-    double inv_n = 0.0;
-    bool odd = false;
-    if constexpr (COS) {
-        const double s64 = i8_sumsq64(sq, dim, lane & 15);
-        odd = !(s64 >= 1e-29 && s64 <= 1e29);
-        inv_n = odd ? 0.0 : 1.0 / sqrt(s64);
-    }
-    i8_pass1<COS>(sq, mu, dim, lane & 15, inv_n, mx, xs, bad);
-    bad |= odd;
-    const float s = i8_scale(mx, bad), inv = 1.0f / s;
-    const bool zero = bad || !(mx >= 1e-30f && mx <= 1e30f);
+    const I8QueryHead hd = i8_query_head<COS, false>(sq, mu, dim, lane & 15);
     float e2 = 0.0f, i2 = 0.0f;
     for (uint32_t pp = lane; pp < KB * 4; pp += 64)
-        dst[((pp >> 2) * NH + h) * 64 + 16 * (pp & 3) + r] = i8_piece<COS>(sq, mu, dim, pp * 16, s, inv, inv_n, zero, e2, i2);
+        dst[((pp >> 2) * NH + h) * 64 + 16 * (pp & 3) + r] = i8_piece<COS>(sq, mu, dim, pp * 16, hd.s, hd.inv, hd.inv_n, hd.zero, e2, i2);
 #pragma unroll
     for (int o = 32; o > 0; o >>= 1) e2 += __shfl_xor(e2, o);
-    if (zero && !bad) e2 = xs;
+    const float off = i8_query_off<COS>(hd.xs, e2, hd.zero, hd.bad, dim, l1, l2);
     if (lane == 0) {
-        float off;
-        if (bad) {
-            off = __uint_as_float(0x7fc00000u);
-        } else {
-            const float du = 2.0f * float(dim + 8) * I8_U;
-            const float dqn = sqrtf(e2) * 1.001f + 4.0f * I8_U * sqrtf(xs) + (COS ? 1e-12f : 0.0f);
-            const float w1 = 1.0f - l1;
-            off = (w1 >= 0.0f ? xs * (1.0f - du) : xs * (1.0f + du)) * w1 - l2 * dqn * dqn;
-            off -= 8.0f * I8_U * (xs * fabsf(w1) + l2 * dqn * dqn);
-        }
-        qscale[q] = (zero || bad) ? 0.0f : s;
+        qscale[q] = i8_query_scale(hd.s, hd.zero, hd.bad);
         qoff[q] = off;
         hits[q] = 0;
     }
diff --git a/lab_1806_vec_db_amd/csrc/kernels.hpp b/lab_1806_vec_db_amd/csrc/kernels.hpp
--- a/lab_1806_vec_db_amd/csrc/kernels.hpp
+++ b/lab_1806_vec_db_amd/csrc/kernels.hpp
@@ -193,6 +193,12 @@
 void launch_flat_gemm8_sample(const void *XT, uint64_t n, uint32_t dim, const void *qfrag, const float *qscale, uint32_t ngroups,
                               const float *rowc, uint32_t unit_step, float *out, uint64_t ld, int num_cu, hipStream_t s, int unit_min = 0);
 uint64_t gemm8_sample_units(uint64_t n, uint32_t unit_step);
+bool gemm8_sample_fused_applies(uint32_t dim);
+void gemm8_set_prep_fused(int v);
+int gemm8_prep_fused();
+void launch_flat_gemm8_sample_fused(const void *XT, uint64_t n, uint32_t dim, const float *Q, uint32_t nq, const float *mu, float l1, float l2,
+                                    int cosine, float *qsq, float *qscale, float *qoff, uint32_t *hits, void *qfrag, uint32_t ngroups,
+                                    const float *rowc, uint32_t unit_step, float *out, uint64_t ld, int num_cu, hipStream_t s, int unit_min);
 void launch_i8_col_mean(const float *X, uint64_t n, uint32_t dim, float *part , float *mu, hipStream_t s,
                         const float *xsq_cos = nullptr);
 void launch_i8_row_stats(const float *X, uint64_t n, uint32_t dim, const float *mu, uint64_t n_s, uint64_t stride,
```
